# krea-ai/realtime-video

Hardware: AMD Instinct MI355X
Metric: frames/sec at 832x480, 4-step 14B T2V (per-step DiT latency in config) (higher is better)
Workload: dtype bf16

## Files before the change

include/rtv_hip.h:

```cpp
#ifndef RTV_HIP_H
#define RTV_HIP_H

#include <stddef.h>
#include <stdint.h>

#ifdef __cplusplus
extern "C" {
#endif

#define RTV_DTYPE_BF16 0
#define RTV_DTYPE_F16 1

#define RTV_ACT_NONE 0
#define RTV_ACT_GELU_TANH 1
#define RTV_ACT_SILU 2

typedef void* rtv_stream_t;

#define RTV_ABI_VERSION 103
int rtv_version(void);
const char* rtv_last_error(void);

int rtv_prof_enable(int class_mask);
int rtv_prof_read(int cls, double* total_ms, int64_t* launches, double* total_work);
int rtv_prof_reset(void);
int rtv_prof_set_stride(int cls, int stride);
int rtv_prof_read_seen(int cls, int64_t* launches, double* work);
int rtv_prof_bracket_overhead(int n, rtv_stream_t stream, double* avg_ms);

int rtv_dispatch_counts(int64_t* counts, int n);
const char* rtv_dispatch_name(int id);
int rtv_dispatch_reset(void);

int rtv_attn_fwd(const void* q, const void* k, const void* v, void* o,
                 int B, int Lq, int Lkv, int H, int D,
                 int64_t q_batch_stride, int64_t q_row_stride,
                 int64_t k_batch_stride, int64_t k_row_stride,
                 int64_t v_batch_stride, int64_t v_row_stride,
                 int64_t o_batch_stride, int64_t o_row_stride,
                 float scale, int causal_block, int q_offset, int dtype, rtv_stream_t stream);

int rtv_attn_fwd_win(const void* q, const void* k, const void* v, void* o,
                     int B, int Lq, int Lkv0, int Lkv1, int seg1_row, int H, int D,
                     int64_t q_batch_stride, int64_t q_row_stride,
                     int64_t k_batch_stride, int64_t k_row_stride,
                     int64_t v_batch_stride, int64_t v_row_stride,
                     int64_t o_batch_stride, int64_t o_row_stride,
                     float scale, int causal_block, int q_offset, int dtype, rtv_stream_t stream);
int rtv_attn_fwd_dup(const void* q, const void* k, const void* v, void* o,
                     int B, int Lq, int Lkv, int H, int D,
                     int64_t q_batch_stride, int64_t q_row_stride,
                     int64_t k_batch_stride, int64_t k_row_stride,
                     int64_t v_batch_stride, int64_t v_row_stride,
                     int64_t o_batch_stride, int64_t o_row_stride,
                     float scale, int dup_key, int dup_count, int dtype, rtv_stream_t stream);
size_t rtv_attn_split_workspace_bytes(int B, int Lq, int H, int kv_splits);
int rtv_attn_fwd_split(const void* q, const void* k, const void* v, void* o,
                       int B, int Lq, int Lkv0, int Lkv1, int seg1_row, int H, int D,
                       int64_t q_batch_stride, int64_t q_row_stride,
                       int64_t k_batch_stride, int64_t k_row_stride,
                       int64_t v_batch_stride, int64_t v_row_stride,
                       int64_t o_batch_stride, int64_t o_row_stride,
                       float scale, int causal_block, int q_offset,
                       int kv_splits, void* workspace, size_t workspace_bytes, int dtype, rtv_stream_t stream);

int rtv_gemm(const void* A, int lda, const void* W, int ldw, void* C, int ldc,
             int M, int N, int K,
             const void* bias, int act,
             const void* gate, int gate_stride, int rows_per_frame, int row_offset,
             const void* residual, int ldr,
             int dtype, int tile_cfg, rtv_stream_t stream);

size_t rtv_gemm_workspace_bytes(void);
int rtv_gemm_set_workspace(void* ptr, size_t bytes);
int rtv_gemm_set_stream_workspace(rtv_stream_t stream, void* ptr, size_t bytes);

int rtv_layernorm_modulate(const void* x, void* out, int M, int d, float eps,
                           const void* shift, const void* scale, int frame_stride, int rows_per_frame,
                           int row_offset, const void* weight, const void* bias, rtv_stream_t stream);

int rtv_rmsnorm(const void* x, int ldx, void* out, int ldo, int M, int d, float eps,
                const void* weight, rtv_stream_t stream);

int rtv_qk_norm_rope_cache(const void* qkv, void* q_out, void* k_cache, void* v_cache,
                           int64_t cache_row_stride, int cache_row0,
                           int M, int d, int num_heads, float eps,
                           const void* wq, const void* wk, const void* rope_cs,
                           int F, int gh, int gw, int start_frame, int row_offset, rtv_stream_t stream);
int rtv_qk_norm_rope_cache_ring(const void* qkv, void* q_out, void* k_cache, void* v_cache,
                                int64_t cache_row_stride, int cache_row0,
                                int M, int d, int num_heads, float eps,
                                const void* wq, const void* wk, const void* rope_cs,
                                int F, int gh, int gw, int start_frame, int row_offset,
                                int ring_lo, int ring_size, int ring_shift, rtv_stream_t stream);

int rtv_modulation_table(const void* modulation, const void* e0, void* emod,
                         int L, int F, int J, int J0, int d, rtv_stream_t stream);

int rtv_sinusoidal_embedding(const void* t, void* out, int F, int dim, rtv_stream_t stream);

int rtv_patchify(const void* x, void* rows, int C, int F, int gh, int gw, rtv_stream_t stream);
int rtv_unpatchify(const void* rows, void* x, int C, int F, int gh, int gw, rtv_stream_t stream);

int rtv_scheduler_step(const void* flow, int64_t flow_frame_stride, int64_t flow_channel_stride,
                       const void* xt, int64_t xt_frame_stride, int64_t xt_channel_stride,
                       const void* t, const void* t_next, int t_kind,
                       const void* timesteps, const void* sigmas, int n_table,
                       void* x0, const void* noise, void* noisy,
                       int F, int C, int hw, rtv_stream_t stream);

int rtv_silu(const void* x, void* out, int64_t n, rtv_stream_t stream);

typedef struct rtv_dit_config {
  int dim, ffn_dim, num_heads, num_layers;
  int freq_dim, text_dim, text_len;
  int in_dim, out_dim;
  float eps;
  int use_fp8;
  int max_attn_kv_splits;
} rtv_dit_config;

typedef struct rtv_dit_layer_weights {
  const void *qkv_w, *qkv_b;
  const void *norm_q_w, *norm_k_w;
  const void *o_w, *o_b;
  const void *norm3_w, *norm3_b;
  const void *cq_w, *cq_b, *ck_w, *ck_b, *cv_w, *cv_b, *co_w, *co_b;
  const void *cnorm_q_w, *cnorm_k_w;
  const void *ffn0_w, *ffn0_b, *ffn2_w, *ffn2_b;
} rtv_dit_layer_weights;

typedef struct rtv_dit_weights {
  const void *patch_w, *patch_b;
  const void *text0_w, *text0_b, *text2_w, *text2_b;
  const void *time0_w, *time0_b, *time2_w, *time2_b;
  const void *tproj_w, *tproj_b;
  const void *head_w, *head_b;
  const void *modulation;
  const void *head_modulation;
  const void *rope_cs;
  const rtv_dit_layer_weights* layers;
  const float* fp8_scales;
} rtv_dit_weights;

typedef struct rtv_dit_step {
  const void* x;
  const void* t;
  const void* context;
  void* out;
  int F, gh, gw;
  void* const* kv_k;
  void* const* kv_v;
  int64_t kv_row_stride;
  void* const* ca_k;
  void* const* ca_v;
  int compute_cross_kv;
  int cache_row0;
  int kv_lo, kv_hi;
  int start_frame;
  int causal_block;
  int gemm_tile_cfg;
  int row_begin, row_count;
  int ring_lo, ring_size, ring_shift;
  int text_rows;
  int kv_only;
  int attn_kv_splits;
} rtv_dit_step;

size_t rtv_dit_workspace_bytes(const rtv_dit_config* cfg, int F, int gh, int gw);
int rtv_dit_forward(const rtv_dit_config* cfg, const rtv_dit_weights* w, const rtv_dit_step* step,
                    void* workspace, size_t workspace_bytes, rtv_stream_t stream);

int rtv_dit_begin(const rtv_dit_config* cfg, const rtv_dit_weights* w, const rtv_dit_step* step,
                  void* workspace, size_t workspace_bytes, rtv_stream_t stream);
int rtv_dit_layer_qkv(const rtv_dit_config* cfg, const rtv_dit_weights* w, const rtv_dit_step* step, int layer,
                      void* workspace, size_t workspace_bytes, rtv_stream_t stream);
int rtv_dit_layer_rest(const rtv_dit_config* cfg, const rtv_dit_weights* w, const rtv_dit_step* step, int layer,
                       void* workspace, size_t workspace_bytes, rtv_stream_t stream);
enum { RTV_PROJ_LN = 1, RTV_PROJ_Q = 2, RTV_PROJ_KV = 4 };
int rtv_dit_layer_proj(const rtv_dit_config* cfg, const rtv_dit_weights* w, const rtv_dit_step* step, int layer,
                       int parts, int world, void* q_send, void* kv_send,
                       void* workspace, size_t workspace_bytes, rtv_stream_t stream);
int rtv_dit_head(const rtv_dit_config* cfg, const rtv_dit_weights* w, const rtv_dit_step* step, void* head_rows,
                 void* workspace, size_t workspace_bytes, rtv_stream_t stream);
int rtv_dit_finish(const rtv_dit_config* cfg, const rtv_dit_step* step, const void* head_rows, rtv_stream_t stream);

int rtv_dit_layer_qkv_hp(const rtv_dit_config* cfg, const rtv_dit_weights* w, const rtv_dit_step* step, int layer, int world,
                         void* q_send, void* kv_send, void* workspace, size_t workspace_bytes, rtv_stream_t stream);
int rtv_dit_layer_attn_hp(const rtv_dit_config* cfg, const rtv_dit_weights* w, const rtv_dit_step* step, int layer, int world,
                          const void* q_all, void* o_all, void* workspace, size_t workspace_bytes, rtv_stream_t stream);
int rtv_dit_layer_rest_hp(const rtv_dit_config* cfg, const rtv_dit_weights* w, const rtv_dit_step* step, int layer, int world,
                          const void* o_recv, void* workspace, size_t workspace_bytes, rtv_stream_t stream);

int rtv_quantize_fp8(const void* x, int64_t ld, int M, int d, void* q, int64_t ldq, float* scale_out, void* amax_scratch,
                     rtv_stream_t stream);
int rtv_gemm_fp8(const void* A, int lda, const void* W, int ldw, const float* a_scale, float w_scale, void* C, int ldc,
                 int M, int N, int K, const void* bias, int act, const void* gate, int gate_stride, int rows_per_frame,
                 int row_offset, const void* residual, int ldr, rtv_stream_t stream);

enum { RTV_CONV_NONE = 0, RTV_CONV_UPSAMPLE2X = 1, RTV_CONV_DOWN2X = 2, RTV_CONV_TIME_DOWN2X = 3 };
enum { RTV_CONV_GATHER = 16 };
int rtv_conv_cl(const void* in, const void* w, const void* bias, const void* residual, int res_ld,
                void* out, int out_ld, int T, int H, int W, int Cin, int Cout, int kt, int kh, int kw,
                int resample, int n_split, const void* zeros, rtv_stream_t stream);
int rtv_conv_cl_win(const void* in, const void* w, const void* bias, const void* residual, int res_ld,
                    void* out, int out_ld, int T, int H, int W, int Cin, int Cout, int kt, int kh, int kw,
                    int resample, int n_split, const void* zeros, int y_out0, int y_in0, int in_rows, int img_rows,
                    rtv_stream_t stream);
int rtv_conv3_norm_silu_cl(const void* in, const void* w, const void* bias, const void* gamma, void* out, int out_ld,
                           int T, int H, int W, int Cin, int Cout, int flags, const void* zeros, rtv_stream_t stream);
int rtv_rmsnorm_silu_cl(const void* x, void* out, const void* gamma, int C, int64_t npix, int apply_silu,
                        rtv_stream_t stream);
int rtv_softmax_rows(const void* s, int lds, void* p, int ldp, int rows, int n, rtv_stream_t stream);

typedef struct rtv_vae_conv { const void* w; const void* b; } rtv_vae_conv;
typedef struct rtv_vae_res {
  const void* gamma0; rtv_vae_conv conv_a; const void* gamma3; rtv_vae_conv conv_b; rtv_vae_conv shortcut;
} rtv_vae_res;
typedef struct rtv_vae_attn {
  const void* gamma; const void *wq, *bq, *wk, *bk, *wv, *bv, *wproj, *bproj;
} rtv_vae_attn;
typedef struct rtv_vae_weights {
  const void *conv2_w, *conv2_b, *mean, *std;
  rtv_vae_conv conv1;
  rtv_vae_res mid0, mid2, up[12];
  rtv_vae_attn attn;
  rtv_vae_conv time_conv[2], resample[3];
  const void* head_gamma;
  rtv_vae_conv head;
} rtv_vae_weights;

size_t rtv_vae_arena_bytes(int h, int w);
int rtv_vae_cache_slot(int h, int w, int slot, size_t* offset, int* C, int* H, int* W);
int rtv_vae_decode(const rtv_vae_weights* w, const void* z, int T, int h, int wd, int first,
                   void* arena, size_t arena_bytes, void* pixels, rtv_stream_t stream);
int rtv_vae_decode_single(const rtv_vae_weights* w, const void* z, int h, int wd, int is_first_frame,
                          void* arena, size_t arena_bytes, void* pixels, rtv_stream_t stream);
int rtv_pixels_to_rgb8(const void* pixels, void* rgb8, int T, int H, int W, rtv_stream_t stream);
size_t rtv_vae_arena_bytes_rows(int h, int w, int row0, int row1);
int rtv_vae_cache_slot_rows(int h, int w, int row0, int row1, int slot, size_t* offset, int* C, int* H, int* W,
                            int* first_row);
int rtv_vae_decode_rows(const rtv_vae_weights* w, const void* z, int T, int h, int wd, int first, int row0, int row1,
                        void* arena, size_t arena_bytes, void* pixels, rtv_stream_t stream);

typedef struct rtv_vae_enc_weights {
  rtv_vae_conv conv1;
  rtv_vae_res down[8];
  rtv_vae_conv resample[3];
  rtv_vae_conv time_conv[2];
  rtv_vae_res mid0, mid2;
  rtv_vae_attn attn;
  const void* head_gamma;
  rtv_vae_conv head;
  const void *conv1x1_w, *conv1x1_b;
  const void *mean, *std;
} rtv_vae_enc_weights;

size_t rtv_vae_enc_arena_bytes(int H, int W);
int rtv_vae_enc_cache_slot(int H, int W, int slot, size_t* offset, int* C, int* h, int* w, int* nslices);
int rtv_vae_encode(const rtv_vae_enc_weights* w, const void* frames, int Ttot, int t0, int tn, int H, int W, int first,
                   void* arena, size_t arena_bytes, void* mu, int Tout_tot, int tout, rtv_stream_t stream);

size_t rtv_vae_attn_arena_bytes(int h, int w);
int rtv_vae_mid_attention(const rtv_vae_attn* a, const void* x, void* y, int h, int w, void* arena, size_t arena_bytes,
                          rtv_stream_t stream);
int rtv_vae_prep(const void* z, int T, int t, int hw, const void* mean, const void* std, const void* conv2_w,
                 const void* conv2_b, void* out, rtv_stream_t stream);
int rtv_vae_final(const void* in, void* pixels, int T, int64_t hw, int64_t in_hw, int64_t skip_px, rtv_stream_t stream);
int rtv_vae_upsample_cache_t1(void* buf, int64_t slice, rtv_stream_t stream);
int rtv_vae_enc_prep(const void* frames, int Ttot, int t0, int T, int64_t hw, void* out, rtv_stream_t stream);
int rtv_vae_enc_final(const void* in, int T, int64_t hw, const void* conv1x1_w, const void* conv1x1_b, const void* mean,
                      const void* std, void* mu, int Tout_tot, int tout, rtv_stream_t stream);

typedef struct rtv_taehv_weights {
  rtv_vae_conv conv_in;
  rtv_vae_conv mem[9][3];
  const void* up[3];
  rtv_vae_conv head;
} rtv_taehv_weights;

size_t rtv_taehv_arena_bytes(int h, int w, int t_max);
int rtv_taehv_state_slot(int h, int w, int slot, size_t* offset, int* C, int* H, int* W);
int rtv_taehv_decode(const rtv_taehv_weights* w, const void* z, int T, int h, int wd, int first, void* arena,
                     size_t arena_bytes, void* pixels, rtv_stream_t stream);
int rtv_taehv_conv(const void* in, const void* w, const void* bias, const void* residual, void* out, int T, int H, int W,
                   int Cin, int Cout, int kt, int ups, int n_split, int relu, int head, const void* zeros,
                   rtv_stream_t stream);

int rtv_taehv_prep(const void* z, int T, int hw, void* out, rtv_stream_t stream);

typedef struct rtv_taehv_enc_weights {
  rtv_vae_conv conv_in;
  const void* down[3];
  rtv_vae_conv mem[9][3];
  rtv_vae_conv head;
} rtv_taehv_enc_weights;

size_t rtv_taehv_enc_arena_bytes(int H, int W, int t_max);
int rtv_taehv_enc_state_slot(int H, int W, int slot, size_t* offset, int* C, int* h, int* w);
int rtv_taehv_encode(const rtv_taehv_enc_weights* w, const void* frames, int T_total, int t0, int tn, int H, int W, int first,
                     void* arena, size_t arena_bytes, void* latents, int T_out, int j, rtv_stream_t stream);
int rtv_taehv_enc_conv(const void* in, const void* w, const void* bias, void* out, int form, int T, int H, int W, int kt,
                       int n_total, int n0, const void* zeros, rtv_stream_t stream);

int rtv_probe_mfma(const void* A , const void* B , void* D ,
                   rtv_stream_t stream);
int rtv_probe_tr(const void* V , void* out , int kbk, int s,
                 rtv_stream_t stream);

typedef struct {
  int vocab, dim, dim_attn, dim_ffn, num_heads, num_layers;
  float eps;
} rtv_t5_config;
typedef struct {
  const void* norm1_w;
  const void* qk_w;
  const void* v_w;
  const void* o_w;
  const void* norm2_w;
  const void* gate_fc1_w;
  const void* fc2_w;
  const void* pos_bias;
} rtv_t5_layer_weights;
typedef struct {
  const void* token_embedding;
  const void* final_norm_w;
  const rtv_t5_layer_weights* layers;
  int max_len;
} rtv_t5_weights;
size_t rtv_t5_workspace_bytes(const rtv_t5_config* cfg, int seq_len);
int rtv_t5_encode(const rtv_t5_config* cfg, const rtv_t5_weights* w, const int* ids, int seq_len, int out_rows,
                  void* workspace, size_t workspace_bytes, void* out, rtv_stream_t stream);

#ifdef __cplusplus
}
#endif
#endif
```

realtime_video_amd/_lib.py:

```python
import ctypes
import os
import re
import subprocess

_HERE = os.path.dirname(os.path.abspath(__file__))
LIB_PATH = os.environ.get("RTV_LIB_PATH") or os.path.join(_HERE, "librtv_hip.so")
CSRC = os.path.join(_HERE, "csrc")

_INCLUDE = os.path.join(os.path.dirname(_HERE), "include")
HEADERS = ("rtv_hip.h", "rtv_hip_lab.h")

_lib = None

_SCALARS = {"int": ctypes.c_int, "int64_t": ctypes.c_int64, "float": ctypes.c_float, "double": ctypes.c_double,
            "size_t": ctypes.c_size_t}
_RETURNS = {"int": ctypes.c_int, "size_t": ctypes.c_size_t, "const char*": ctypes.c_char_p}
_STARS = r"(\*(?:\s*const\s*\*)?)?"


def _field_type(base, stars, structs):
    value = _SCALARS.get(base) or structs.get(base)
    if not stars:
        return value
    if base == "void":
        return ctypes.c_void_p if stars == "*" else ctypes.POINTER(ctypes.c_void_p)
    return ctypes.POINTER(value) if value and stars == "*" else None


def _param_type(base, stars, structs):
    if not stars:
        return ctypes.c_void_p if base == "rtv_stream_t" else _SCALARS.get(base)
    if base in structs:
        return ctypes.POINTER(structs[base]) if stars == "*" else None
    return ctypes.c_void_p if base == "void" or base in _SCALARS else None


def parse_header(text, structs):
    text = re.sub(r"/\*.*?\*/", "", text, flags=re.S)
    text = re.sub(r"#ifdef __cplusplus.*?#endif", "", text, flags=re.S)
    text = re.sub(r"^[ \t]*#.*$", "", text, flags=re.M)
    text = re.sub(r"\benum\s*\{[^}]*\}\s*;|\btypedef\s+void\s*\*\s*rtv_stream_t\s*;", "", text)

    def struct(m):
        name, fields = m.group(2), []
        for decl in filter(None, (d.strip() for d in m.group(1).split(";"))):
            head = re.match(r"(?:const\s+)?(\w+)\s*", decl)
            for item in decl[head.end():].split(","):
                d = re.fullmatch(_STARS + r"\s*(\w+)((?:\s*\[\d+\])*)", item.strip())
                t = d and _field_type(head.group(1), re.sub(r"\s", "", d.group(1) or ""), structs)
                if not t:
                    raise ValueError(f"{name}: cannot bind field declaration `{decl}`")
                for n in reversed(re.findall(r"\d+", d.group(3))):
                    t = t * int(n)
                fields.append((d.group(2), t))
        structs[name] = type(name, (ctypes.Structure,), {"_fields_": fields})
        return ""

    text = re.sub(r"\btypedef\s+struct\s*\w*\s*\{([^}]*)\}\s*(\w+)\s*;", struct, text)
    protos = {}
    for stmt in filter(None, (" ".join(s.split()) for s in text.split(";"))):
        m = re.fullmatch(r"(.*?)\s*\b(\w+)\s*\((.*)\)", stmt)
        if not m:
            raise ValueError(f"cannot bind declaration `{stmt}`")
        ret, name, params = m.group(1).replace(" *", "*"), m.group(2), m.group(3).strip()
        if ret not in _RETURNS:
            raise ValueError(f"{name}: cannot bind return type `{ret}`")
        argtypes = []
        for param in ([] if params == "void" else params.split(",")):
            d = re.fullmatch(r"(?:const\s+)?(\w+)\s*" + _STARS + r"\s*(\w+)?", param.strip())
            t = d and _param_type(d.group(1), re.sub(r"\s", "", d.group(2) or ""), structs)
            if not t:
                raise ValueError(f"{name}: cannot bind parameter `{param.strip()}`")
            argtypes.append(t)
        protos[name] = (_RETURNS[ret], argtypes)
    return protos


def _read(name):
    with open(os.path.join(_INCLUDE, name)) as f:
        return f.read()


STRUCTS, PROTOTYPES = {}, {}
for _name in HEADERS:
    PROTOTYPES.update(parse_header(_read(_name), STRUCTS))
IO_HEADER = "rtv_hip_io.h"
IO_STRUCTS = dict(STRUCTS)
IO_PROTOTYPES = parse_header(_read(IO_HEADER), IO_STRUCTS)
IO_STRUCTS = {k: v for k, v in IO_STRUCTS.items() if k not in STRUCTS}
JPEG_HEADER = "rtv_hip_jpeg.h"
JPEG_STRUCTS = dict(STRUCTS)
JPEG_PROTOTYPES = parse_header(_read(JPEG_HEADER), JPEG_STRUCTS)
JPEG_STRUCTS = {k: v for k, v in JPEG_STRUCTS.items() if k not in STRUCTS}
JPEGDEC_HEADER = "rtv_hip_jpeg_decode.h"
JPEGDEC_STRUCTS = dict(STRUCTS)
JPEGDEC_PROTOTYPES = parse_header(_read(JPEGDEC_HEADER), JPEGDEC_STRUCTS)
JPEGDEC_STRUCTS = {k: v for k, v in JPEGDEC_STRUCTS.items() if k not in STRUCTS}
LORA_HEADER = "rtv_hip_lora.h"
LORA_STRUCTS = dict(STRUCTS)
LORA_PROTOTYPES = parse_header(_read(LORA_HEADER), LORA_STRUCTS)
LORA_STRUCTS = {k: v for k, v in LORA_STRUCTS.items() if k not in STRUCTS}
LORA_MAX_ADAPTERS, LORA_MAX_RANK = (int(re.search(rf"^#define\s+RTV_LORA_MAX_{n}\s+(\d+)", _read(LORA_HEADER), flags=re.M).group(1))
                                    for n in ("ADAPTERS", "RANK"))
FRAMES_MAX = int(re.search(r"^#define\s+RTV_FRAMES_MAX\s+(\d+)", _read(IO_HEADER), flags=re.M).group(1))
ABI_VERSION = int(re.search(r"^#define\s+RTV_ABI_VERSION\s+(\d+)", _read(HEADERS[0]), flags=re.M).group(1))


def build(verbose=False):
    jobs = os.environ.get("MAX_JOBS") or str(min(16, len(os.sched_getaffinity(0)) if hasattr(os, "sched_getaffinity") else os.cpu_count() or 4))
    cmd = ["make", "-C", CSRC, "-j", jobs]
    res = subprocess.run(cmd, capture_output=True, text=True)
    if verbose or res.returncode != 0:
        print(res.stdout[-4000:])
        print(res.stderr[-4000:])
    if res.returncode != 0:
        raise RuntimeError("building librtv_hip.so failed")
    return LIB_PATH


def declared_symbols(lab=True):
    out = set()
    for name in HEADERS if lab else HEADERS[:1]:
        text = re.sub(r"/\*.*?\*/", "", _read(name), flags=re.S)
        out.update(re.findall(r"\b(rtv_[a-z0-9_]+)\s*\(", text))
    return sorted(out)


def load():
    global _lib
    if _lib is not None:
        return _lib
    if not os.path.exists(LIB_PATH):
        raise RuntimeError(
            f"{LIB_PATH} is missing: run `python -c 'import __graft_entry__ as g; g.build()'` "
            "(or `make -C realtime_video_amd/csrc`). There is no CPU fallback for the HIP path.")
    lib = ctypes.CDLL(LIB_PATH)
    for name, (restype, argtypes) in list(PROTOTYPES.items()) + list(IO_PROTOTYPES.items()) + list(JPEG_PROTOTYPES.items()) + list(JPEGDEC_PROTOTYPES.items()) + list(LORA_PROTOTYPES.items()):
        fn = getattr(lib, name, None)
        if fn is None:
            if os.environ.get("RTV_LIB_PATH"):
                continue
            raise RuntimeError(f"librtv_hip.so does not export {name}")
        fn.restype, fn.argtypes = restype, argtypes
    have = lib.rtv_version()
    if have != ABI_VERSION:
        raise RuntimeError(f"{LIB_PATH} reports ABI revision {have}, include/rtv_hip.h declares RTV_ABI_VERSION {ABI_VERSION}: "
                           "rebuild the library (`make -C realtime_video_amd/csrc`)")
    _lib = lib
    return lib


def check(status, what):
    if status != 0:
        msg = load().rtv_last_error().decode("utf-8", "replace")
        raise RuntimeError(f"{what} failed (status {status}): {msg}")


def call(name, *args):
    check(getattr(load(), name)(*args), name)
```

realtime_video_amd/causal_model.py:

```python
import collections
import ctypes
import types

import torch

from . import _lib, lora, ops
from .rope import rope_cos_sin_table

c_vp = ctypes.c_void_p
_IncompatibleKeys = collections.namedtuple("_IncompatibleKeys", ["missing_keys", "unexpected_keys"])


_Cfg = _lib.STRUCTS["rtv_dit_config"]
_LayerW = _lib.STRUCTS["rtv_dit_layer_weights"]
_Weights = _lib.STRUCTS["rtv_dit_weights"]
_Step = _lib.STRUCTS["rtv_dit_step"]
_LAYER_FIELDS = tuple(n for n, _ in _LayerW._fields_)
_TOP_FIELDS = tuple(n for n, t in _Weights._fields_ if t is c_vp)

_FP8_TOP = ("text0_w", "text2_w", "time0_w", "time2_w", "tproj_w", "head_w")
_FP8_LAYER = ("qkv_w", "o_w", "cq_w", "ck_w", "cv_w", "co_w", "ffn0_w", "ffn2_w")

PROJ_LN, PROJ_Q, PROJ_KV = 1, 2, 4


class BlockCausalMask:

    def __init__(self, num_frames, frame_seqlen, num_frame_per_block, local_attn_size=-1):
        if local_attn_size != -1:
            raise NotImplementedError("local-window block masks are not used by the inference path")
        self.num_frames, self.frame_seqlen = num_frames, frame_seqlen
        self.num_frame_per_block = num_frame_per_block
        self.block_tokens = frame_seqlen * num_frame_per_block

    def __repr__(self):
        return f"BlockCausalMask(frames={self.num_frames}, block_tokens={self.block_tokens})"


class _SelfAttnHandle:

    def __init__(self, local_attn_size, sink_size):
        self.local_attn_size = local_attn_size
        self.sink_size = sink_size
        self.num_frame_per_block = 1
        self.fused_projections = True
        self.max_attention_size = 32760 if local_attn_size == -1 else local_attn_size * 1560

    def fuse_projections(self):
        self.fused_projections = True


def cache_row_map(cache, sink_tokens=None):
    n = int(cache["local_end_index"])
    r = torch.arange(n)
    lo, size, start = (int(cache.get(k, 0)) for k in ("ring_lo", "ring_size", "ring_start"))
    if size > 0:
        r = torch.where(r >= lo, lo + (r - lo + start) % size, r)
    return r


class CausalWanModel:
    def __init__(self, model_type="t2v", patch_size=(1, 2, 2), text_len=512, in_dim=16, dim=2048, ffn_dim=8192,
                 freq_dim=256, text_dim=4096, out_dim=16, num_heads=16, num_layers=32, local_attn_size=-1,
                 sink_size=0, qk_norm=True, cross_attn_norm=True, eps=1e-6, device="cuda"):
        if model_type != "t2v" or tuple(patch_size) != (1, 2, 2) or not qk_norm or not cross_attn_norm:
            raise NotImplementedError("the MI355X hot path implements the t2v causal model (patch 1x2x2, qk_norm, cross_attn_norm)")
        if dim % num_heads or dim // num_heads != 128:
            raise ValueError("head_dim must be 128")
        self.model_type, self.patch_size = model_type, tuple(patch_size)
        self.text_len, self.in_dim, self.dim, self.ffn_dim = text_len, in_dim, dim, ffn_dim
        self.freq_dim, self.text_dim, self.out_dim = freq_dim, text_dim, out_dim
        self.num_heads, self.num_layers, self.eps = num_heads, num_layers, eps
        self.local_attn_size, self.sink_size = local_attn_size, sink_size
        self.device = torch.device(device)
        self.config = types.SimpleNamespace(num_heads=num_heads, dim=dim, num_layers=num_layers, ffn_dim=ffn_dim)
        self.blocks = [types.SimpleNamespace(self_attn=_SelfAttnHandle(local_attn_size, sink_size))
                       for _ in range(num_layers)]
        self.block_mask = None
        self.num_frame_per_block = 1
        self.independent_first_frame = False
        self.gemm_tile_cfg = 0
        self.context_parallel = None
        self._tensors = {}
        self._w = None
        self._ws = {}
        self.fold_text_padding = True
        self.use_hip_graphs = False
        self._graphs = {}
        self._weights_version = 0
        self._cfg = _Cfg(dim, ffn_dim, num_heads, num_layers, freq_dim, text_dim, text_len, in_dim, out_dim, eps, 0, 0)
        self._lora = {}
        self._lora_base = {}
        self.lora_version = 0

    def eval(self):
        return self

    def to(self, *args, **kwargs):
        for a in list(args) + list(kwargs.values()):
            if isinstance(a, torch.dtype) and a != torch.bfloat16:
                raise NotImplementedError(f"the MI355X DiT computes in bf16 (asked for {a})")
            if isinstance(a, (str, torch.device, int)) and not isinstance(a, bool):
                dev = torch.device("cuda", a) if isinstance(a, int) else torch.device(a)
                if dev.type != self.device.type or (dev.index is not None and self.device.index is not None
                                                    and dev.index != self.device.index):
                    raise NotImplementedError(f"weights live on {self.device}; construct the model with device={dev!s} instead")
        return self

    def requires_grad_(self, flag=False):
        return self

    def parameters(self):
        return iter(self._tensors.values())

    def state_dict_shapes(self, fused=False):
        d, f = self.dim, self.ffn_dim
        sh = {"patch_embedding.weight": (d, self.in_dim) + self.patch_size, "patch_embedding.bias": (d,),
              "text_embedding.0.weight": (d, self.text_dim), "text_embedding.0.bias": (d,),
              "text_embedding.2.weight": (d, d), "text_embedding.2.bias": (d,),
              "time_embedding.0.weight": (d, self.freq_dim), "time_embedding.0.bias": (d,),
              "time_embedding.2.weight": (d, d), "time_embedding.2.bias": (d,),
              "time_projection.1.weight": (6 * d, d), "time_projection.1.bias": (6 * d,),
              "head.head.weight": (self.out_dim * 4, d), "head.head.bias": (self.out_dim * 4,), "head.modulation": (1, 2, d)}
        for i in range(self.num_layers):
            p = f"blocks.{i}"
            for a in ("self_attn", "cross_attn"):
                for m in ("q", "k", "v", "o"):
                    sh[f"{p}.{a}.{m}.weight"], sh[f"{p}.{a}.{m}.bias"] = (d, d), (d,)
                sh[f"{p}.{a}.norm_q.weight"], sh[f"{p}.{a}.norm_k.weight"] = (d,), (d,)
            if fused:
                sh[f"{p}.self_attn.to_qkv.weight"], sh[f"{p}.self_attn.to_qkv.bias"] = (3 * d, d), (3 * d,)
            sh[f"{p}.norm3.weight"], sh[f"{p}.norm3.bias"] = (d,), (d,)
            sh[f"{p}.ffn.0.weight"], sh[f"{p}.ffn.0.bias"] = (f, d), (f,)
            sh[f"{p}.ffn.2.weight"], sh[f"{p}.ffn.2.bias"] = (d, f), (d,)
            sh[f"{p}.modulation"] = (1, 6, d)
        return sh

    def load_state_dict(self, sd, strict=True, assign=False):
        dev, bf = self.device, torch.bfloat16
        sd = {(k[len("model."):] if k.startswith("model.") else k): v for k, v in sd.items()}
        want = self.state_dict_shapes(fused=True)
        problems, missing, unexpected = [], [], sorted(k for k in sd if k not in want)
        fused_layers = set()
        for i in range(self.num_layers):
            sa = f"blocks.{i}.self_attn"
            if sa + ".to_qkv.weight" in sd and sa + ".to_qkv.bias" in sd:
                fused_layers.add(i)
        for k, shp in want.items():
            layer_fused = ".self_attn." in k and int(k.split(".")[1]) in fused_layers
            is_qkv = ".self_attn." in k and k.split(".")[3] in ("q", "k", "v")
            is_fused_key = ".to_qkv." in k
            if k not in sd:
                if (is_fused_key and not layer_fused) or (is_qkv and layer_fused):
                    continue
                missing.append(k)
            elif tuple(sd[k].shape) != tuple(shp):
                problems.append(f"size mismatch for {k}: copying a param with shape {tuple(sd[k].shape)} from checkpoint, "
                                f"the shape in current model is {tuple(shp)}.")
        if missing:
            problems.insert(0, "Missing key(s) in state_dict: " + ", ".join(repr(k) for k in missing[:12])
                            + (f" ... ({len(missing)} in total)" if len(missing) > 12 else "") + ".")
        if unexpected and strict:
            problems.insert(1 if missing else 0, "Unexpected key(s) in state_dict: " + ", ".join(repr(k) for k in unexpected[:12])
                            + (f" ... ({len(unexpected)} in total)" if len(unexpected) > 12 else "") + ".")
        if problems and (strict or missing or any(p.startswith("size") for p in problems)):
            raise RuntimeError("Error(s) in loading state_dict for CausalWanModel:\n\t" + "\n\t".join(problems))
        t = {}

        def get(name):
            return sd[name].detach().to(device=dev, dtype=bf).contiguous()

        t["patch_w"] = get("patch_embedding.weight").reshape(self.dim, -1).contiguous()
        t["patch_b"] = get("patch_embedding.bias")
        for dst, src in (("text0", "text_embedding.0"), ("text2", "text_embedding.2"), ("time0", "time_embedding.0"),
                         ("time2", "time_embedding.2"), ("tproj", "time_projection.1"), ("head", "head.head")):
            t[dst + "_w"], t[dst + "_b"] = get(src + ".weight"), get(src + ".bias")
        t["head_modulation"] = get("head.modulation").reshape(2, self.dim).contiguous()
        t["modulation"] = torch.empty((self.num_layers, 6, self.dim), dtype=bf, device=dev)
        for i in range(self.num_layers):
            t["modulation"][i].copy_(sd[f"blocks.{i}.modulation"].detach().reshape(6, self.dim))
        t["rope_cs"] = rope_cos_sin_table(self.dim // self.num_heads).to(dev)
        layers = (_LayerW * self.num_layers)()
        d = self.dim
        for i in range(self.num_layers):
            p, sa, ca = f"blocks.{i}", f"blocks.{i}.self_attn", f"blocks.{i}.cross_attn"
            lt = {}
            if i in fused_layers:
                lt["qkv_w"], lt["qkv_b"] = get(sa + ".to_qkv.weight"), get(sa + ".to_qkv.bias")
            else:
                lt["qkv_w"] = torch.empty((3 * d, d), dtype=bf, device=dev)
                lt["qkv_b"] = torch.empty((3 * d,), dtype=bf, device=dev)
                for j, m in enumerate(("q", "k", "v")):
                    lt["qkv_w"][j * d:(j + 1) * d].copy_(sd[f"{sa}.{m}.weight"].detach())
                    lt["qkv_b"][j * d:(j + 1) * d].copy_(sd[f"{sa}.{m}.bias"].detach())
            lt["norm_q_w"], lt["norm_k_w"] = get(sa + ".norm_q.weight"), get(sa + ".norm_k.weight")
            lt["o_w"], lt["o_b"] = get(sa + ".o.weight"), get(sa + ".o.bias")
            lt["norm3_w"], lt["norm3_b"] = get(p + ".norm3.weight"), get(p + ".norm3.bias")
            for m in ("q", "k", "v", "o"):
                lt[f"c{m}_w"], lt[f"c{m}_b"] = get(f"{ca}.{m}.weight"), get(f"{ca}.{m}.bias")
            lt["cnorm_q_w"], lt["cnorm_k_w"] = get(ca + ".norm_q.weight"), get(ca + ".norm_k.weight")
            lt["ffn0_w"], lt["ffn0_b"] = get(p + ".ffn.0.weight"), get(p + ".ffn.0.bias")
            lt["ffn2_w"], lt["ffn2_b"] = get(p + ".ffn.2.weight"), get(p + ".ffn.2.bias")
            for name in _LAYER_FIELDS:
                setattr(layers[i], name, lt[name].data_ptr())
                t[f"L{i}.{name}"] = lt[name]
        w = _Weights()
        for name in _TOP_FIELDS:
            setattr(w, name, t[name].data_ptr())
        w.layers = ctypes.cast(layers, ctypes.POINTER(_LayerW))
        self._layers_arr = layers
        self._tensors, self._w = t, w
        self._cfg.use_fp8 = 0
        if self._lora or self._lora_base:
            self._lora, self._lora_base = {}, {}
            self.lora_version += 1
        self._graphs.clear()
        self._weights_version += 1
        return _IncompatibleKeys([], [] if strict else unexpected)

    def enable_fp8(self):
        if self._w is None:
            raise RuntimeError("load weights before enable_fp8()")
        if self._cfg.use_fp8:
            return self
        for k in (self.dim, self.ffn_dim, self.text_dim, self.freq_dim):
            if k % 128:
                raise ValueError("enable_fp8: every Linear input width must be a multiple of 128")
        scales = (ctypes.c_float * (len(_FP8_TOP) + len(_FP8_LAYER) * self.num_layers))()

        def quant(key):
            q, s = self._quantize_fp8(self._tensors[key])
            self._tensors[key] = q
            return q, s

        for i, name in enumerate(_FP8_TOP):
            q, scales[i] = quant(name)
            setattr(self._w, name, q.data_ptr())
        for l in range(self.num_layers):
            for j, name in enumerate(_FP8_LAYER):
                q, scales[len(_FP8_TOP) + len(_FP8_LAYER) * l + j] = quant(f"L{l}.{name}")
                setattr(self._layers_arr[l], name, q.data_ptr())
        self._fp8_scales = scales
        self._w.fp8_scales = ctypes.cast(scales, ctypes.POINTER(ctypes.c_float))
        self._cfg.use_fp8 = 1
        self._graphs.clear()
        self._weights_version += 1
        self._ws.clear()
        ops.ensure_gemm_workspace(self.device)
        return self

    @staticmethod
    def _quantize_fp8(w):
        s = w.float().abs().max().clamp(min=1e-12) / 448.0
        q = (w.float() / s).clamp(-448.0, 448.0).to(torch.float8_e4m3fn).contiguous()
        return q, float(s)

    def lora_adapters(self):
        return {name: ad["scale"] for name, ad in self._lora.items()}

    def load_lora(self, sd, scale=1.0, name=None, strict=True):
        targets, _ = lora.parse_lora_state_dict(sd, self.state_dict_shapes(), strict=strict)
        scale = float(scale)
        if scale != scale or scale in (float("inf"), float("-inf")):
            raise ValueError("load_lora: scale must be finite")
        if name is None:
            n = len(self._lora)
            while f"lora{n}" in self._lora:
                n += 1
            name = f"lora{n}"
        if name in self._lora:
            raise ValueError(f"load_lora: an adapter named {name!r} is loaded already")
        if len(self._lora) >= lora.MAX_ADAPTERS:
            raise RuntimeError(f"load_lora: at most {lora.MAX_ADAPTERS} adapters are loaded at once (RTV_LORA_MAX_ADAPTERS)")
        if self.device.type != "cuda":
            raise RuntimeError("load_lora: the merge is a HIP kernel and this model lives on the CPU (no CPU fallback)")
        if self._w is None:
            raise RuntimeError("load weights before load_lora()")
        if self._cfg.use_fp8:
            raise RuntimeError("load_lora after enable_fp8(): the bf16 weights are gone - load adapters first, then enable_fp8()")
        dev, bf = self.device, torch.bfloat16
        on_dev = {t: tg._replace(A=tg.A.detach().to(device=dev, dtype=bf).contiguous(),
                                 B=tg.B.detach().to(device=dev, dtype=bf).contiguous()) for t, tg in targets.items()}
        for tg in on_dev.values():
            if tg.tensor not in self._lora_base:
                self._lora_base[tg.tensor] = self._tensors[tg.tensor].clone()
        self._lora[name] = {"scale": scale, "targets": on_dev}
        self._remerge({tg.tensor for tg in on_dev.values()})
        return name

    def set_lora_scale(self, name, scale):
        if name not in self._lora:
            raise KeyError(f"no LoRA adapter named {name!r} (loaded: {list(self._lora)})")
        scale = float(scale)
        if scale != scale or scale in (float("inf"), float("-inf")):
            raise ValueError("set_lora_scale: scale must be finite")
        self._lora[name]["scale"] = scale
        self._remerge({tg.tensor for tg in self._lora[name]["targets"].values()})

    def unload_lora(self, name=None):
        if name is not None and name not in self._lora:
            raise KeyError(f"no LoRA adapter named {name!r} (loaded: {list(self._lora)})")
        touched = set()
        for n in [name] if name is not None else list(self._lora):
            touched |= {tg.tensor for tg in self._lora.pop(n)["targets"].values()}
        self._remerge(touched)

    def _remerge(self, keys):
        fp8, cross = bool(self._cfg.use_fp8), False
        for key in sorted(keys):
            base = self._lora_base[key]
            live = [(ad["scale"], tg) for ad in self._lora.values() for tg in ad["targets"].values() if tg.tensor == key]
            out = torch.empty_like(base) if fp8 else self._tensors[key]
            blocks = ((0, base.shape[0]),) if not key.endswith(".qkv_w") else tuple((j * self.dim, self.dim) for j in range(3))
            for row0, rows in blocks:
                lora.merge(base[row0:row0 + rows], out[row0:row0 + rows],
                           [(tg.A, tg.B, s * tg.factor) for s, tg in live if (tg.row0, tg.rows) == (row0, rows)])
            if fp8:
                q, s = self._quantize_fp8(out)
                self._tensors[key].copy_(q)
                layer, field = key[1:].split(".")
                self._fp8_scales[len(_FP8_TOP) + len(_FP8_LAYER) * int(layer) + _FP8_LAYER.index(field)] = s
            if not live:
                del self._lora_base[key]
            cross = cross or key.endswith((".ck_w", ".cv_w"))
        if fp8 and keys:
            self._graphs.clear()
            self._weights_version += 1
        if cross:
            self.lora_version += 1

    def init_random_weights(self, seed=0, std=0.02):
        g = torch.Generator(device=self.device).manual_seed(seed)
        d, ffn, bf = self.dim, self.ffn_dim, torch.bfloat16

        def rnd(*shape, s=std):
            return (torch.randn(*shape, generator=g, device=self.device, dtype=torch.float32) * s).to(bf)

        def xav(o, i):
            return rnd(o, i, s=(2.0 / (i + o)) ** 0.5)

        sd = {"patch_embedding.weight": xav(d, self.in_dim * 4).view(d, self.in_dim, 1, 2, 2), "patch_embedding.bias": rnd(d),
              "text_embedding.0.weight": rnd(d, self.text_dim), "text_embedding.0.bias": rnd(d),
              "text_embedding.2.weight": rnd(d, d), "text_embedding.2.bias": rnd(d),
              "time_embedding.0.weight": rnd(d, self.freq_dim), "time_embedding.0.bias": rnd(d),
              "time_embedding.2.weight": rnd(d, d), "time_embedding.2.bias": rnd(d),
              "time_projection.1.weight": xav(6 * d, d), "time_projection.1.bias": rnd(6 * d),
              "head.head.weight": rnd(self.out_dim * 4, d), "head.head.bias": rnd(self.out_dim * 4),
              "head.modulation": rnd(1, 2, d, s=d ** -0.5)}
        for i in range(self.num_layers):
            p = f"blocks.{i}"
            sd[f"{p}.self_attn.to_qkv.weight"], sd[f"{p}.self_attn.to_qkv.bias"] = xav(3 * d, d), rnd(3 * d)
            sd[f"{p}.self_attn.o.weight"], sd[f"{p}.self_attn.o.bias"] = xav(d, d), rnd(d)
            for a in ("self_attn", "cross_attn"):
                sd[f"{p}.{a}.norm_q.weight"] = 1 + rnd(d, s=0.1)
                sd[f"{p}.{a}.norm_k.weight"] = 1 + rnd(d, s=0.1)
            for m in ("q", "k", "v", "o"):
                sd[f"{p}.cross_attn.{m}.weight"], sd[f"{p}.cross_attn.{m}.bias"] = xav(d, d), rnd(d)
            sd[f"{p}.norm3.weight"], sd[f"{p}.norm3.bias"] = 1 + rnd(d, s=0.1), rnd(d, s=0.05)
            sd[f"{p}.ffn.0.weight"], sd[f"{p}.ffn.0.bias"] = xav(ffn, d), rnd(ffn)
            sd[f"{p}.ffn.2.weight"], sd[f"{p}.ffn.2.bias"] = xav(d, ffn), rnd(d)
            sd[f"{p}.modulation"] = rnd(1, 6, d, s=d ** -0.5)
        self.load_state_dict(sd)
        return self

    @staticmethod
    def _prepare_blockwise_causal_attn_mask(device=None, num_frames=21, frame_seqlen=1560, num_frame_per_block=1,
                                            local_attn_size=-1):
        return BlockCausalMask(num_frames, frame_seqlen, num_frame_per_block, local_attn_size)

    def _workspace(self, F, gh, gw, slot=0):
        key = (F, gh, gw, slot)
        ws = self._ws.get(key)
        if ws is None:
            n = _lib.load().rtv_dit_workspace_bytes(ctypes.byref(self._cfg), F, gh, gw)
            ws = torch.empty(n + 256, dtype=torch.uint8, device=self.device)
            self._ws[key] = ws
        return ws

    def kv_cache_heads(self):
        cp = self.context_parallel
        if cp is not None and getattr(cp, "world", 1) > 1 and len(cp.local_ranks()) == 1 and cp.head_exchange(self.num_heads):
            return self.num_heads // cp.world
        return self.num_heads

    def _exchange_buffers(self, M, world, slot, device):
        key = (M, world, slot)
        if not hasattr(self, "_xbufs"):
            self._xbufs = {}
        b = self._xbufs.get(key)
        if b is None:
            rl, hn = M // world, self.num_heads // world
            gc = hn * 128
            e = lambda *shape: torch.empty(shape, dtype=torch.bfloat16, device=device)
            b = {"hn": hn, "q_send": e(world, rl, gc), "kv_send": e(world, rl, 2, gc), "q_all": e(M, gc), "o_all": e(M, gc),
                 "o_recv": e(world, rl, gc)}
            self._xbufs[key] = b
        return b

    def _cache_window(self, kv_cache, num_new, current_start, frame_seqlen, ring=True):
        c0 = kv_cache[0]
        kv_size = c0["k"].shape[1]
        if self.block_mask is not None:
            if num_new > kv_size:
                raise RuntimeError(f"KV cache window [0, {num_new}) outside cache of {kv_size} rows")

            def commit_rc():
                for c in kv_cache:
                    c["global_end_index"] = num_new
                    c["local_end_index"] = num_new
                    c["ring_lo"], c["ring_size"], c["ring_start"] = 0, 0, 0
            return 0, 0, num_new, 0, self.block_mask.block_tokens, (0, 0, 0), commit_rc
        sa = self.blocks[0].self_attn
        g_end, l_end = int(c0["global_end_index"]), int(c0["local_end_index"])
        current_end = current_start + num_new
        sink_tokens = sa.sink_size * frame_seqlen
        ring_lo, ring_size = int(c0.get("ring_lo", 0)), int(c0.get("ring_size", 0))
        ring_start = int(c0.get("ring_start", 0)) if l_end > 0 else 0
        shift_copy = None
        if sa.local_attn_size != -1 and current_end > g_end and num_new + l_end > kv_size:
            evicted = num_new + l_end - kv_size
            rolled = l_end - evicted - sink_tokens
            if ring and rolled <= 0:
                ring_start = 0
            elif ring:
                if ring_size == 0 or ring_start == 0:
                    ring_lo, ring_size = sink_tokens, kv_size - sink_tokens
                elif (ring_lo, ring_size) != (sink_tokens, kv_size - sink_tokens):
                    raise RuntimeError("the attention sink changed under a rotated rolling cache")
                ring_start = (ring_start + evicted) % ring_size
            else:
                shift_copy = (sink_tokens, evicted, rolled)
            local_end = l_end + current_end - g_end - evicted
        else:
            local_end = l_end + current_end - g_end
        if not ring and ring_start:
            raise RuntimeError("this KV cache is rotated (ring_start != 0): reset it before using it under context parallelism")
        local_start = local_end - num_new
        if local_start < 0 or local_end > kv_size:
            raise RuntimeError(f"KV cache window [{local_start}, {local_end}) outside cache of {kv_size} rows")
        lo = max(0, local_end - sa.max_attention_size)
        if ring_start == 0:
            ring_lo = ring_size = 0

        def commit():
            if shift_copy is not None:
                s0, ev, ro = shift_copy
                for c in kv_cache:
                    for n in ("k", "v"):
                        c[n][:, s0:s0 + ro] = c[n][:, s0 + ev:s0 + ev + ro].clone()
            for c in kv_cache:
                c["global_end_index"] = current_end
                c["local_end_index"] = local_end
                c["ring_lo"], c["ring_size"], c["ring_start"] = ring_lo, ring_size, ring_start
        return local_start, lo, local_end, current_start // frame_seqlen, 0, (ring_lo, ring_size, ring_start), commit

    def _forward_inference(self, x, t, context, seq_len=None, clip_fea=None, y=None, kv_cache=None,
                           crossattn_cache=None, current_start=0, cache_start=0, kv_cache_only=False):
        if self._w is None:
            raise RuntimeError("weights not loaded")
        if kv_cache is None or crossattn_cache is None:
            raise NotImplementedError("the hot path is the KV-cached inference forward (causal_model.py:825-954)")
        if clip_fea is not None or y is not None:
            raise NotImplementedError("i2v conditioning is out of scope")
        xs = list(x) if not torch.is_tensor(x) else [x[i] for i in range(x.shape[0])]
        B = len(xs)
        if B != 1:
            raise NotImplementedError("batch size 1 (the streaming server path); run sessions as replicas")
        u = xs[0]
        if not u.is_cuda:
            raise RuntimeError("realtime_video_amd.CausalWanModel needs GPU tensors (no CPU fallback)")
        C, F, Hh, Ww = u.shape
        gh, gw = Hh // 2, Ww // 2
        fs = gh * gw
        M = F * fs
        if seq_len is not None and M > seq_len:
            raise AssertionError("sequence longer than seq_len")
        u = u.to(torch.bfloat16).contiguous()
        tt = t.reshape(-1).to(device=u.device, dtype=torch.float32).contiguous()
        if tt.numel() != F:
            raise ValueError("t must hold one timestep per latent frame")
        need_cross = not all(bool(c["is_init"]) and int(c.get("lora_version", 0)) == self.lora_version for c in crossattn_cache)
        ctx = None
        if need_cross:
            cu = context[0] if not torch.is_tensor(context) else context[0]
            ctx = torch.zeros(self.text_len, self.text_dim, dtype=torch.bfloat16, device=u.device)
            ctx[:cu.shape[0]] = cu.to(torch.bfloat16)
            nz = torch.nonzero(ctx.abs().amax(dim=1) > 0)
            n_real = int(nz[-1]) + 1 if nz.numel() else 0
            for c in crossattn_cache:
                c["text_rows"] = n_real
        cp = self.context_parallel
        use_cp = cp is not None and (cp.world > 1 or getattr(cp, "force_single_rank", False))
        kv_only = bool(kv_cache_only) and not need_cross
        text_rows = int(crossattn_cache[0].get("text_rows", 0)) if getattr(self, "fold_text_padding", True) else 0
        if text_rows <= 0 or any(int(c.get("text_rows", 0)) != text_rows for c in crossattn_cache):
            text_rows = 0
        row0, lo, hi, start_frame, causal_block, (ring_lo, ring_size, ring_shift), commit = \
            self._cache_window(kv_cache, M, current_start, fs, ring=not use_cp)
        L = self.num_layers
        rs = kv_cache[0]["k"].stride(1)
        for c in kv_cache:
            for n in ("k", "v"):
                if c[n].stride(3) != 1 or c[n].stride(2) != c[n].shape[3] or c[n].stride(1) != rs:
                    raise ValueError("KV cache tensors must be [B, kv_size, H, 128] views with dense [H, 128] rows "
                                     "and one common row stride")

        def ptr_array(tensors):
            arr = (c_vp * L)(*[t_.data_ptr() for t_ in tensors])
            return arr, ctypes.cast(arr, ctypes.POINTER(c_vp))

        kk_keep, kk = ptr_array([c["k"] for c in kv_cache])
        kv_keep, kv = ptr_array([c["v"] for c in kv_cache])
        ck_keep, ck = ptr_array([c["k"] for c in crossattn_cache])
        cv_keep, cv = ptr_array([c["v"] for c in crossattn_cache])
        out = (torch.zeros if kv_only else torch.empty)((self.out_dim, F, Hh, Ww), dtype=torch.bfloat16, device=u.device)
        stream = c_vp(torch.cuda.current_stream().cuda_stream)
        cfg_p, w_p = ctypes.byref(self._cfg), ctypes.byref(self._w)

        def make(rank_rows, slot, kk=kk, kv=kv):
            ws = self._workspace(F, gh, gw, slot)
            ws_ptr = (ws.data_ptr() + 255) & ~255
            st = _Step(u.data_ptr(), tt.data_ptr(), ctx.data_ptr() if ctx is not None else None, out.data_ptr(),
                       F, gh, gw, kk, kv, rs, ck, cv, int(need_cross), row0, lo, hi,
                       start_frame, causal_block, int(self.gemm_tile_cfg), rank_rows[0], rank_rows[1],
                       ring_lo, ring_size, ring_shift, int(text_rows), int(kv_only),
                       int(getattr(cp, "attn_kv_splits", 1)) if use_cp else 1)
            return st, (c_vp(ws_ptr), ctypes.c_size_t(ws.numel() - (ws_ptr - ws.data_ptr())), stream)

        splits = int(getattr(cp, "attn_kv_splits", 1)) if use_cp else 1
        if splits > self._cfg.max_attn_kv_splits:
            self._cfg.max_attn_kv_splits = splits
            self._ws.clear()
            self._graphs.clear()
            self._weights_version += 1
        if self.gemm_tile_cfg in (0, 5):
            ops.ensure_gemm_workspace(u.device)
        if use_cp:
            commit()
        if not use_cp:
            graph_key = None
            if self.use_hip_graphs and not need_cross:
                graph_key = (F, gh, gw, row0, lo, hi, start_frame, causal_block, ring_lo, ring_size, ring_shift, kv_only, text_rows,
                             int(self.gemm_tile_cfg), rs, self._weights_version,
                             kv_cache[0]["k"].data_ptr(), kv_cache[-1]["v"].data_ptr(), crossattn_cache[0]["k"].data_ptr())
                ent = self._graphs.get(graph_key)
                if isinstance(ent, dict):
                    ent["u"].copy_(u)
                    ent["t"].copy_(tt)
                    ent["graph"].replay()
                    commit()
                    return ent["out"].clone().unsqueeze(0)
            if graph_key is not None and self._graphs.get(graph_key) == "seen":
                ent = {"u": u.clone(), "t": tt.clone(), "out": out, "keep": (kk_keep, kv_keep, ck_keep, cv_keep)}
                u, tt = ent["u"], ent["t"]
                g = torch.cuda.CUDAGraph()
                if not hasattr(self, "_capture_stream"):
                    self._capture_stream = torch.cuda.Stream(device=u.device)
                ops.ensure_gemm_workspace(u.device, self._capture_stream.cuda_stream)
                with torch.cuda.graph(g, stream=self._capture_stream):
                    stream = c_vp(torch.cuda.current_stream().cuda_stream)
                    st, wsa = make((0, 0), 0)
                    _lib.call("rtv_dit_forward", cfg_p, w_p, ctypes.byref(st), *wsa)
                ent["graph"], ent["step"] = g, st
                self._graphs[graph_key] = ent
                g.replay()
                commit()
                return out.clone().unsqueeze(0)
            if graph_key is not None:
                self._graphs[graph_key] = "seen"
            st, wsa = make((0, 0), 0)
            _lib.call("rtv_dit_forward", cfg_p, w_p, ctypes.byref(st), *wsa)
            commit()
        else:
            graph_key = None
            if self.use_hip_graphs and not need_cross and not getattr(cp, "_gloo", False):
                graph_key = ("cp", id(cp), bool(getattr(cp, "overlap", True)), cp.world, cp.head_exchange(self.num_heads), F, gh, gw, row0, lo, hi, start_frame, causal_block, kv_only,
                             text_rows, int(self.gemm_tile_cfg), rs, self._weights_version, splits,
                             kv_cache[0]["k"].data_ptr(), kv_cache[-1]["v"].data_ptr(), crossattn_cache[0]["k"].data_ptr())
                ent = self._graphs.get(graph_key)
                if isinstance(ent, dict):
                    ent["u"].copy_(u)
                    ent["t"].copy_(tt)
                    ent["graph"].replay()
                    return ent["out"].clone().unsqueeze(0)

            def run_cp():
                self.cp_forwards_issued = getattr(self, "cp_forwards_issued", 0) + 1
                from .parallel import shard_rows, wait_in_order
                W, H = cp.world, self.num_heads
                heads = cp.head_exchange(H)
                keep = []
                if heads:
                    hn = H // W
                    if kv_cache[0]["k"].shape[2] not in (hn, H):
                        raise ValueError(f"KV cache must hold {hn} (this rank's) or {H} heads, not {kv_cache[0]['k'].shape[2]}")
                    parts = []
                    for i, r in enumerate(cp.local_ranks()):
                        h0 = 0 if kv_cache[0]["k"].shape[2] == hn else r * hn
                        ka, kp = ptr_array([c["k"][0, :, h0:h0 + hn] for c in kv_cache])
                        va, vp = ptr_array([c["v"][0, :, h0:h0 + hn] for c in kv_cache])
                        keep.append((ka, va))
                        parts.append(make(shard_rows(M, W, r), i, kp, vp))
                    bufs = [(r, self._exchange_buffers(M, W, i, u.device)) for i, r in enumerate(cp.local_ranks())]
                else:
                    parts = [make(shard_rows(M, W, r), i) for i, r in enumerate(cp.local_ranks())]
                for st, wsa in parts:
                    _lib.call("rtv_dit_begin", cfg_p, w_p, ctypes.byref(st), *wsa)
                null = c_vp(0)
                for l in range(L):
                    last_kv_only = kv_only and l == L - 1
                    if not heads:
                        for st, wsa in parts:
                            _lib.call("rtv_dit_layer_proj", cfg_p, w_p, ctypes.byref(st), l, PROJ_LN | PROJ_KV, 0, null, null, *wsa)
                        pend = cp.gather_kv(kv_cache[l]["k"][0], kv_cache[l]["v"][0], row0, M, async_op=True)
                        if last_kv_only:
                            pend.wait()
                            break
                        for st, wsa in parts:
                            _lib.call("rtv_dit_layer_proj", cfg_p, w_p, ctypes.byref(st), l, PROJ_Q, 0, null, null, *wsa)
                        pend.wait()
                        for st, wsa in parts:
                            _lib.call("rtv_dit_layer_rest", cfg_p, w_p, ctypes.byref(st), l, *wsa)
                        continue
                    if last_kv_only:
                        for (st, wsa), (_, b) in zip(parts, bufs):
                            _lib.call("rtv_dit_layer_proj", cfg_p, w_p, ctypes.byref(st), l, PROJ_LN | PROJ_KV, W, null,
                                      c_vp(b["kv_send"].data_ptr()), *wsa)
                        cp.exchange_kv(bufs, kv_cache[l]["k"][0], kv_cache[l]["v"][0], row0, M)
                        break
                    for (st, wsa), (_, b) in zip(parts, bufs):
                        _lib.call("rtv_dit_layer_proj", cfg_p, w_p, ctypes.byref(st), l, PROJ_LN | PROJ_Q, W,
                                  c_vp(b["q_send"].data_ptr()), null, *wsa)
                    pend_q = cp.exchange_q(bufs, async_op=True)
                    for (st, wsa), (_, b) in zip(parts, bufs):
                        _lib.call("rtv_dit_layer_proj", cfg_p, w_p, ctypes.byref(st), l, PROJ_KV, W, null,
                                  c_vp(b["kv_send"].data_ptr()), *wsa)
                    pend_kv = cp.exchange_kv(bufs, kv_cache[l]["k"][0], kv_cache[l]["v"][0], row0, M, async_op=True)
                    wait_in_order(pend_q, pend_kv)
                    for (st, wsa), (_, b) in zip(parts, bufs):
                        _lib.call("rtv_dit_layer_attn_hp", cfg_p, w_p, ctypes.byref(st), l, W, c_vp(b["q_all"].data_ptr()),
                                  c_vp(b["o_all"].data_ptr()), *wsa)
                    cp.exchange_o(bufs)
                    for (st, wsa), (_, b) in zip(parts, bufs):
                        _lib.call("rtv_dit_layer_rest_hp", cfg_p, w_p, ctypes.byref(st), l, W, c_vp(b["o_recv"].data_ptr()), *wsa)
                if not kv_only:
                    hrow = torch.empty((M, self.out_dim * 4), dtype=torch.bfloat16, device=u.device)
                    for st, wsa in parts:
                        _lib.call("rtv_dit_head", cfg_p, w_p, ctypes.byref(st), c_vp(hrow.data_ptr()), *wsa)
                    cp.all_gather_rows_(hrow, kind="head_rows")
                    _lib.call("rtv_dit_finish", cfg_p, ctypes.byref(parts[0][0]), c_vp(hrow.data_ptr()), stream)

            if graph_key is not None and self._graphs.get(graph_key) == "seen":
                ent = {"u": u.clone(), "t": tt.clone(), "out": out, "keep": (kk_keep, kv_keep, ck_keep, cv_keep)}
                u, tt = ent["u"], ent["t"]
                g = torch.cuda.CUDAGraph()
                if not hasattr(self, "_capture_stream"):
                    self._capture_stream = torch.cuda.Stream(device=u.device)
                ops.ensure_gemm_workspace(u.device, self._capture_stream.cuda_stream)
                with torch.cuda.graph(g, stream=self._capture_stream, capture_error_mode="thread_local"):
                    stream = c_vp(torch.cuda.current_stream().cuda_stream)
                    run_cp()
                ent["graph"] = g
                self._graphs[graph_key] = ent
                g.replay()
                return out.clone().unsqueeze(0)
            if graph_key is not None:
                self._graphs[graph_key] = "seen"
            run_cp()
        if need_cross:
            for c in crossattn_cache:
                c["is_init"] = True
                c["lora_version"] = self.lora_version
        return out.unsqueeze(0)

    def forward(self, *args, **kwargs):
        return self._forward_inference(*args, **kwargs)

    __call__ = forward
```

realtime_video_amd/csrc/attn_fwd.hip:

```cpp
#include "attn_common.h"

namespace rtv {

#ifdef RTV_ATTN_TRACE
__device__ unsigned* g_attn_trace = nullptr;
#define ATT_STAMP(i)                                                                    \
  do {                                                                                  \
    if (tr_on && j >= 20 && j < 24) {                                                   \
      __builtin_amdgcn_sched_barrier(0);                                                \
      const unsigned t_ = (unsigned)__builtin_readcyclecounter();                       \
      if (lane == 0) tr_dst[(j - 20) * 6 + (i)] = t_;                                   \
      __builtin_amdgcn_sched_barrier(0);                                                \
    }                                                                                   \
  } while (0)
#else
#define ATT_STAMP(i)
#endif

template <bool F16>
__global__ __launch_bounds__(256) void attn_combine_kernel(const float* __restrict__ part_o, const float* __restrict__ part_ml,
                                                           uint16_t* __restrict__ o, int S, int B, int H, int Lq, int64_t o_bs,
                                                           int64_t o_rs) {
  const int64_t nrows = (int64_t)B * H * Lq;
  const int64_t row = (int64_t)blockIdx.x * 16 + (threadIdx.x >> 4);
  if (row >= nrows) return;
  const int c8 = (threadIdx.x & 15) * 8;
  float m = -INFINITY;
  for (int s = 0; s < S; ++s) m = fmaxf(m, part_ml[((int64_t)s * nrows + row) * 2]);
  float acc[8] = {0.f, 0.f, 0.f, 0.f, 0.f, 0.f, 0.f, 0.f};
  float l = 0.f;
  for (int s = 0; s < S; ++s) {
    const f32x2 ml = *(const f32x2*)(part_ml + ((int64_t)s * nrows + row) * 2);
    const float w = __builtin_amdgcn_exp2f(ml[0] - m);
    l += w * ml[1];
    const float* po = part_o + ((int64_t)s * nrows + row) * ATT_D + c8;
    const f32x4 a = *(const f32x4*)po, b2 = *(const f32x4*)(po + 4);
#pragma unroll
    for (int i = 0; i < 4; ++i) {
      acc[i] += w * a[i];
      acc[4 + i] += w * b2[i];
    }
  }
  const float inv = 1.0f / l;
  const int bh = (int)(row / Lq), q = (int)(row - (int64_t)bh * Lq);
  const int b = bh / H, h = bh - b * H;
  u32x4 out;
#pragma unroll
  for (int i = 0; i < 4; ++i) out[i] = pack2<F16>(acc[2 * i] * inv, acc[2 * i + 1] * inv);
  *(u32x4*)(o + (size_t)b * o_bs + (size_t)q * o_rs + (size_t)h * ATT_D + c8) = out;
}

template <bool F16, int NW>
__global__ __launch_bounds__(NW * 64, 2) void attn_fwd_kernel(AttnParams p) {
  constexpr int ATT_QT = ATT_QW * NW;
  constexpr int ATT_THREADS = NW * 64;
  constexpr int ATT_LD_PER_THREAD = ATT_KT * 16 / ATT_THREADS;
  constexpr int ATT_RSTEP = ATT_THREADS / 16;
  extern __shared__ __attribute__((aligned(16))) char smem[];
  char* const sK = smem;
  char* const sV = smem + 2 * ATT_TILE_BYTES;

  const int tid = threadIdx.x;
  const int lane = tid & 63;
  const int wave = __builtin_amdgcn_readfirstlane(tid >> 6);
  const int l31 = lane & 31, g = lane >> 5;

  int bh, qt;
  {
    const int nbh = p.B * p.H;
    const int bid = blockIdx.x;
    if (nbh % 8 == 0) {
      int xcd = bid & 7, slot = bid >> 3;
      bh = xcd + 8 * (slot / p.n_qtiles);
      qt = slot % p.n_qtiles;
    } else {
      bh = bid / p.n_qtiles;
      qt = bid % p.n_qtiles;
    }
  }
  const int b = bh / p.H, h = bh % p.H;
  const int q0 = qt * ATT_QT;

  const uint16_t* qb = p.q + (size_t)b * p.q_bs + (size_t)h * ATT_D;
  const uint16_t* kb = p.k + (size_t)b * p.k_bs + (size_t)h * ATT_D;
  const uint16_t* vb = p.v + (size_t)b * p.v_bs + (size_t)h * ATT_D;
  uint16_t* ob = p.o + (size_t)b * p.o_bs + (size_t)h * ATT_D;

  const int q_row = q0 + wave * ATT_QW + l31;
  const int q_row_c = min(q_row, p.Lq - 1);
  u32x4 qf[8];
  {
    const uint16_t* qp = qb + (size_t)q_row_c * p.q_rs + g * 8;
#pragma unroll
    for (int dc = 0; dc < 8; ++dc) qf[dc] = *(const u32x4*)(qp + dc * 16);
  }

  int kv_lim = p.Lkv;
  int wave_min_lim = p.Lkv;
  int wg_max_lim = p.Lkv;
  if (p.causal_block > 0) {
    const int cb = p.causal_block;
    kv_lim = min(p.Lkv, ((p.q_offset + q_row_c) / cb + 1) * cb);
    int first = min(q0 + wave * ATT_QW, p.Lq - 1);
    wave_min_lim = min(p.Lkv, ((p.q_offset + first) / cb + 1) * cb);
    int last = min(q0 + ATT_QT - 1, p.Lq - 1);
    wg_max_lim = min(p.Lkv, ((p.q_offset + last) / cb + 1) * cb);
  }
  const int ntiles = (wg_max_lim + ATT_KT - 1) / ATT_KT;
  int t_lo, t_hi;
  split_tile_range(p, ntiles, &t_lo, &t_hi);

  u32x4 kreg[ATT_LD_PER_THREAD], vreg[ATT_LD_PER_THREAD];
  const int st_r = tid >> 4, st_c = tid & 15;
  const uint32_t k_goff = (uint32_t)(st_r * (int)p.k_rs + st_c * 8) * 2u;
  const uint32_t v_goff = (uint32_t)(st_r * (int)p.v_rs + st_c * 8) * 2u;
  auto load_tile = [&](int j) {
    const int row0 = j * ATT_KT;
    const bool in0 = row0 + ATT_KT <= p.n0;
    if (in0 || (row0 >= p.n0 && row0 + ATT_KT <= p.Lkv)) {
      const int64_t prow = in0 ? row0 : row0 + p.delta;
      const char* kj = (const char*)(kb + prow * p.k_rs);
      const char* vj = (const char*)(vb + prow * p.v_rs);
#pragma unroll
      for (int i = 0; i < ATT_LD_PER_THREAD; ++i) {
        kreg[i] = *(const u32x4*)(kj + (size_t)(i * ATT_RSTEP) * p.k_rs * 2 + k_goff);
        vreg[i] = *(const u32x4*)(vj + (size_t)(i * ATT_RSTEP) * p.v_rs * 2 + v_goff);
      }
    } else {
#pragma unroll
      for (int i = 0; i < ATT_LD_PER_THREAD; ++i) {
        int kv = min(row0 + st_r + i * ATT_RSTEP, p.Lkv - 1);
        if (kv >= p.n0) kv += p.delta;
        kreg[i] = *(const u32x4*)(kb + (int64_t)kv * p.k_rs + st_c * 8);
        vreg[i] = *(const u32x4*)(vb + (int64_t)kv * p.v_rs + st_c * 8);
      }
    }
  };
  char* const k_wr = sK + st_r * 256 + ((st_c ^ (st_r & 15)) << 4);
  char* const v_wr = sV + st_r * 256 + ((st_c << 4) ^ ((st_r & 3) << 6));
  auto write_tile = [&](int buf) {
#pragma unroll
    for (int i = 0; i < ATT_LD_PER_THREAD; ++i) {
      *(u32x4*)(k_wr + buf * ATT_TILE_BYTES + i * ATT_RSTEP * 256) = kreg[i];
      *(u32x4*)(v_wr + buf * ATT_TILE_BYTES + i * ATT_RSTEP * 256) = vreg[i];
    }
  };

  const char* k_rd[8];
#pragma unroll
  for (int dc = 0; dc < 8; ++dc) k_rd[dc] = sK + l31 * 256 + (((dc * 2 + g) ^ (l31 & 15)) << 4);
  const int i16 = lane & 15, h16 = (lane >> 4) & 1;
  const char* v_rd[4];
#pragma unroll
  for (int db = 0; db < 4; ++db)
    v_rd[db] = sV + (4 * g + (i16 >> 2)) * 256 + h16 * 32 + (i16 & 3) * 8 + ((db ^ (i16 >> 2)) << 6);

  f32x16 oacc[4];
#pragma unroll
  for (int db = 0; db < 4; ++db)
#pragma unroll
    for (int r = 0; r < 16; ++r) oacc[db][r] = 0.f;
  float m_run = -1e30f;
  float l_run = 0.f;
  const float c = p.scale_log2e;
  const f32x2 c2 = {c, c};
  constexpr float RESCALE_SLACK = 8.f;

#ifdef RTV_ATTN_TRACE
  const bool tr_on = g_attn_trace != nullptr && (wave == 0 || wave == NW - 1) && blockIdx.x < 512;
  unsigned* const tr_dst = g_attn_trace + ((size_t)(blockIdx.x & 511) * 2 + (wave == 0 ? 0 : 1)) * 24;
#endif
  auto tile = [&](const int j, auto bufc) {
    constexpr int buf = decltype(bufc)::value;
    const bool has_next = (j + 1 < t_hi);
    ATT_STAMP(0);
    if (has_next) load_tile(j + 1);

    f32x16 sacc[2];
#pragma unroll
    for (int kbk = 0; kbk < 2; ++kbk)
#pragma unroll
      for (int r = 0; r < 16; ++r) sacc[kbk][r] = 0.f;
#pragma unroll
    for (int dc = 0; dc < 8; ++dc)
#pragma unroll
      for (int kbk = 0; kbk < 2; ++kbk) {
        u32x4 kf = *(const u32x4*)(k_rd[dc] + buf * ATT_TILE_BYTES + kbk * 32 * 256);
        sacc[kbk] = mfma32<F16>(kf, qf[dc], sacc[kbk]);
      }

    ATT_STAMP(1);
    if (p.dup_key >= 0 && (unsigned)(p.dup_key - j * ATT_KT) < (unsigned)ATT_KT) {
      const int local = p.dup_key - j * ATT_KT;
#pragma unroll
      for (int kbk = 0; kbk < 2; ++kbk)
#pragma unroll
        for (int r = 0; r < 16; ++r)
          if (kbk * 32 + (r & 3) + 8 * (r >> 2) + 4 * g == local) sacc[kbk][r] += p.dup_bias;
    }
    if ((j + 1) * ATT_KT > wave_min_lim) {
#pragma unroll
      for (int kbk = 0; kbk < 2; ++kbk)
#pragma unroll
        for (int r = 0; r < 16; ++r) {
          int kv = j * ATT_KT + kbk * 32 + (r & 3) + 8 * (r >> 2) + 4 * g;
          if (kv >= kv_lim) sacc[kbk][r] = -INFINITY;
        }
    }

    float mx = sacc[0][0];
#pragma unroll
    for (int r = 1; r < 16; ++r) mx = fmaxf(mx, sacc[0][r]);
#pragma unroll
    for (int r = 0; r < 16; ++r) mx = fmaxf(mx, sacc[1][r]);
    mx = fmaxf(mx, __shfl_xor(mx, 32, 64));
    const float m_cand = fmaxf(m_run, mx * c);
    const bool need = m_cand - m_run > RESCALE_SLACK;
    if (__builtin_amdgcn_ballot_w64(need) != 0) {
      const float m_new = need ? m_cand : m_run;
      const float alpha = __builtin_amdgcn_exp2f(m_run - m_new);
      m_run = m_new;
      l_run *= alpha;
#pragma unroll
      for (int db = 0; db < 4; ++db)
#pragma unroll
        for (int r = 0; r < 16; ++r) oacc[db][r] *= alpha;
    }
    const f32x2 nm2 = {-m_run, -m_run};
    f32x2 ps2 = {0.f, 0.f};
    u32x4 pf[2][2];
#pragma unroll
    for (int kbk = 0; kbk < 2; ++kbk)
#pragma unroll
      for (int t = 0; t < 8; ++t) {
        f32x2 x = {sacc[kbk][2 * t], sacc[kbk][2 * t + 1]};
        x = __builtin_elementwise_fma(x, c2, nm2);
        f32x2 e = {__builtin_amdgcn_exp2f(x[0]), __builtin_amdgcn_exp2f(x[1])};
        ps2 += e;
        pf[kbk][t >> 2][t & 3] = pack2<F16>(e[0], e[1]);
      }
    l_run += ps2[0] + ps2[1];

    ATT_STAMP(2);
#pragma unroll
    for (int kbk = 0; kbk < 2; ++kbk)
#pragma unroll
      for (int s = 0; s < 2; ++s) {
#pragma unroll
        for (int db = 0; db < 4; ++db) {
          const char* vp = v_rd[db] + buf * ATT_TILE_BYTES + (kbk * 32 + s * 16) * 256;
          u32x2 lo = lds_tr_read(vp);
          u32x2 hi = lds_tr_read(vp + 8 * 256);
          u32x4 vf = {lo[0], lo[1], hi[0], hi[1]};
          oacc[db] = mfma32<F16>(vf, pf[kbk][s], oacc[db]);
        }
      }

    ATT_STAMP(3);
    if (has_next) write_tile(buf ^ 1);
    ATT_STAMP(4);
    __syncthreads();
    ATT_STAMP(5);
  };

  load_tile(t_lo);
  write_tile(0);
  __syncthreads();
  for (int j = t_lo; j < t_hi; j += 2) {
    tile(j, IntC<0>{});
    if (j + 1 < t_hi) tile(j + 1, IntC<1>{});
  }

  const float l_tot = l_run + __shfl_xor(l_run, 32, 64);
  if (p.kv_splits > 1) {
    store_partial(p, bh, q_row, g, oacc, m_run, l_tot);
    return;
  }
  const float inv = 1.0f / l_tot;
  if (q_row < p.Lq) {
    uint16_t* op = ob + (size_t)q_row * p.o_rs + 4 * g;
#pragma unroll
    for (int db = 0; db < 4; ++db)
#pragma unroll
      for (int i = 0; i < 4; ++i) {
        u32x2 w;
        w[0] = pack2<F16>(oacc[db][4 * i + 0] * inv, oacc[db][4 * i + 1] * inv);
        w[1] = pack2<F16>(oacc[db][4 * i + 2] * inv, oacc[db][4 * i + 3] * inv);
        *(u32x2*)(op + db * 32 + i * 8) = w;
      }
  }
}


constexpr int ATT_NB = 3;

#ifdef RTV_ATTN_TRACE
#define ATT_STAMP8(i)                                                                   \
  do {                                                                                  \
    if (tr_on && j >= 20 && j < 24) {                                                   \
      __builtin_amdgcn_sched_barrier(0);                                                \
      const unsigned t_ = (unsigned)__builtin_readcyclecounter();                       \
      if (lane == 0) tr_lds[(j - 20) * 8 + (i)] = t_;    \
      __builtin_amdgcn_sched_barrier(0);                                                \
    }                                                                                   \
  } while (0)
#else
#define ATT_STAMP8(i)
#endif

template <bool F16>
__global__ __launch_bounds__(512, 2) void attn_fwd_pp_kernel(AttnParams p) {
  constexpr int ATT_QT = 256;
  extern __shared__ __attribute__((aligned(16))) char smem[];
  char* const sK = smem;
  char* const sV = smem + ATT_NB * ATT_TILE_BYTES;

  const int tid = threadIdx.x;
  const int lane = tid & 63;
  const int wave = __builtin_amdgcn_readfirstlane(tid >> 6);
  const int grp = wave >> 2;
  const int l31 = lane & 31, g = lane >> 5;

  int bh, qt;
  {
    const int nbh = p.B * p.H;
    const int bid = blockIdx.x;
    if (nbh % 8 == 0) {
      int xcd = bid & 7, slot = bid >> 3;
      bh = xcd + 8 * (slot / p.n_qtiles);
      qt = slot % p.n_qtiles;
    } else {
      bh = bid / p.n_qtiles;
      qt = bid % p.n_qtiles;
    }
  }
  const int b = bh / p.H, h = bh % p.H;
  const int q0 = qt * ATT_QT;
  const uint16_t* qb = p.q + (size_t)b * p.q_bs + (size_t)h * ATT_D;
  const uint16_t* kb = p.k + (size_t)b * p.k_bs + (size_t)h * ATT_D;
  const uint16_t* vb = p.v + (size_t)b * p.v_bs + (size_t)h * ATT_D;
  uint16_t* ob = p.o + (size_t)b * p.o_bs + (size_t)h * ATT_D;

  const int q_row = q0 + wave * ATT_QW + l31;
  const int q_row_c = min(q_row, p.Lq - 1);
  int kv_lim = p.Lkv, wave_min_lim = p.Lkv, wg_max_lim = p.Lkv;
  if (p.causal_block > 0) {
    const int cb = p.causal_block;
    kv_lim = min(p.Lkv, ((p.q_offset + q_row_c) / cb + 1) * cb);
    int first = min(q0 + wave * ATT_QW, p.Lq - 1);
    wave_min_lim = min(p.Lkv, ((p.q_offset + first) / cb + 1) * cb);
    int last = min(q0 + ATT_QT - 1, p.Lq - 1);
    wg_max_lim = min(p.Lkv, ((p.q_offset + last) / cb + 1) * cb);
  }
  const int ntiles = (wg_max_lim + ATT_KT - 1) / ATT_KT;
  int t_lo, t_hi;
  split_tile_range(p, ntiles, &t_lo, &t_hi);

  const __amdgpu_buffer_rsrc_t rsrcK = __builtin_amdgcn_make_buffer_rsrc((void*)kb, 0, 0x7fffffff, 0x00020000);
  const __amdgpu_buffer_rsrc_t rsrcV = __builtin_amdgcn_make_buffer_rsrc((void*)vb, 0, 0x7fffffff, 0x00020000);
  const int st_row = wave * 8 + (lane >> 4);
  const int st_cp = lane & 15;
  const int k_rs = (int)p.k_rs, v_rs = (int)p.v_rs;
  const int w_off0 = __builtin_amdgcn_readfirstlane(p.off0), w_delta = __builtin_amdgcn_readfirstlane(p.delta);
  const int w_n0 = __builtin_amdgcn_readfirstlane(p.n0), w_lkv = __builtin_amdgcn_readfirstlane(p.Lkv);
  int k_ch[2], v_ch[2];
  uint32_t k_fast[2], v_fast[2];
#pragma unroll
  for (int i = 0; i < 2; ++i) {
    const int r = st_row + 4 * i;
    k_ch[i] = (st_cp ^ (r & 15)) * 8;
    v_ch[i] = (st_cp ^ ((r & 3) << 2)) * 8;
    k_fast[i] = (uint32_t)(r * k_rs + k_ch[i]) * 2u;
    v_fast[i] = (uint32_t)(r * v_rs + v_ch[i]) * 2u;
  }
  auto stage = [&](const __amdgpu_buffer_rsrc_t& rsrc, char* ring, int j, int rs, const uint32_t (&fast)[2],
                   const int (&ch)[2]) {
    const int row0 = j * ATT_KT;
    char* const dst = ring + (j % ATT_NB) * ATT_TILE_BYTES + wave * (8 * 256);
    const bool in0 = row0 + ATT_KT <= w_n0;
    if (in0 || (row0 >= w_n0 && row0 + ATT_KT <= w_lkv)) {
      const uint32_t so = (uint32_t)((row0 + (in0 ? w_off0 : w_delta)) * rs) * 2u;
#pragma unroll
      for (int i = 0; i < 2; ++i)
        __builtin_amdgcn_raw_ptr_buffer_load_lds(rsrc, (RTV_LDS void*)(dst + i * 1024), 16, fast[i], so, 0, 0);
    } else {
#pragma unroll
      for (int i = 0; i < 2; ++i) {
        int kv = min(row0 + st_row + 4 * i, w_lkv - 1);
        kv += kv >= w_n0 ? w_delta : w_off0;
        __builtin_amdgcn_raw_ptr_buffer_load_lds(rsrc, (RTV_LDS void*)(dst + i * 1024), 16,
                                                 (uint32_t)(kv * rs + ch[i]) * 2u, 0, 0, 0);
      }
    }
  };
  auto stage_k = [&](int j) { stage(rsrcK, sK, j, k_rs, k_fast, k_ch); };
  auto stage_v = [&](int j) { stage(rsrcV, sV, j, v_rs, v_fast, v_ch); };

  stage_k(t_lo);
  stage_v(t_lo);
  stage_k(t_lo + 1);
  stage_v(t_lo + 1);
  u32x4 qf[8];
  {
    const uint16_t* qp = qb + (size_t)q_row_c * p.q_rs + g * 8;
#pragma unroll
    for (int dc = 0; dc < 8; ++dc) qf[dc] = *(const u32x4*)(qp + dc * 16);
  }

  uint32_t k_rd32[8];
#pragma unroll
  for (int dc = 0; dc < 8; ++dc)
    k_rd32[dc] = (uint32_t)(uintptr_t)(RTV_LDS const char*)(sK + l31 * 256 + (((dc * 2 + g) ^ (l31 & 15)) << 4));
  const int i16 = lane & 15, h16 = (lane >> 4) & 1;
  uint32_t v_rd32[4];
#pragma unroll
  for (int db = 0; db < 4; ++db)
    v_rd32[db] = (uint32_t)(uintptr_t)(RTV_LDS const char*)(sV + (4 * g + (i16 >> 2)) * 256 + h16 * 32 + (i16 & 3) * 8 +
                                                            ((db ^ (i16 >> 2)) << 6));

  f32x16 oacc[4];
#pragma unroll
  for (int db = 0; db < 4; ++db)
#pragma unroll
    for (int r = 0; r < 16; ++r) oacc[db][r] = 0.f;
  float m_run = -1e30f;
  float l_run = 0.f;
  const float c = p.scale_log2e;
  const f32x2 c2 = {c, c};
  constexpr float RESCALE_SLACK = 8.f;

  f32x16 sacc[2];
  u32x4 pf[2][2];
  u32x4 frag[16];
  f32x2 ps2 = {0.f, 0.f};
  auto exp_step = [&](auto kc, auto tc) {
    constexpr int kbk = decltype(kc)::value, t = decltype(tc)::value;
    const f32x2 nm2 = {-m_run, -m_run};
    f32x2 x = {sacc[kbk][2 * t], sacc[kbk][2 * t + 1]};
    x = __builtin_elementwise_fma(x, c2, nm2);
#ifdef ATT_LAB_T3
    f32x2 e = x;
#else
    f32x2 e = {__builtin_amdgcn_exp2f(x[0]), __builtin_amdgcn_exp2f(x[1])};
#endif
    ps2 += e;
    pf[kbk][t >> 2][t & 3] = pack2<F16>(e[0], e[1]);
  };

#ifdef RTV_ATTN_TRACE
  const bool tr_on = g_attn_trace != nullptr && (wave == 0 || wave == 7) && blockIdx.x < 512;
  unsigned* const tr_dst = g_attn_trace + ((size_t)(blockIdx.x & 511) * 2 + (wave == 0 ? 0 : 1)) * 32;
  unsigned* const tr_lds = (unsigned*)(smem + 2 * ATT_NB * ATT_TILE_BYTES) + (wave == 0 ? 0 : 32);
#endif
#define PP_BARRIER()                        \
  do {                                      \
    __builtin_amdgcn_sched_barrier(0);      \
    __builtin_amdgcn_s_barrier();           \
    __builtin_amdgcn_sched_barrier(0);      \
  } while (0)

  asm volatile("s_waitcnt vmcnt(0)" ::: "memory");
  __syncthreads();
  if (grp) PP_BARRIER();

  const bool idle_rows = p.skip_idle && q0 + wave * ATT_QW >= p.Lq;
  if (idle_rows) {
    for (int j = t_lo; j < t_hi; ++j) {
      stage_k(j + 2);
      asm volatile("s_waitcnt vmcnt(4)" ::: "memory");
      PP_BARRIER();
      PP_BARRIER();
      stage_v(j + 2);
      asm volatile("s_waitcnt vmcnt(4)" ::: "memory");
      PP_BARRIER();
      PP_BARRIER();
    }
    if (!grp) PP_BARRIER();
    return;
  }
  for (int j = t_lo; j < t_hi; ++j) {
    const int slot_off = (j % ATT_NB) * ATT_TILE_BYTES;
    ATT_STAMP8(0);
#ifndef ATT_LAB_T6
    stage_k(j + 2);
#endif
    static_for<0, 16>([&](auto ic) {
      constexpr int n = decltype(ic)::value;
      frag[n] = lds_read128_at<(n & 1) * 32 * 256>(k_rd32[n >> 1] + (uint32_t)slot_off);
    });
    asm volatile("s_waitcnt vmcnt(4)" ::: "memory");
    ATT_STAMP8(1);
    PP_BARRIER();
    ATT_STAMP8(2);
    lds_wait_frags(frag);
    uint32_t va[4];
#pragma unroll
    for (int db = 0; db < 4; ++db) va[db] = v_rd32[db] + (uint32_t)slot_off;
    auto rd_v = [&](auto ic) {
#ifndef ATT_LAB_T4
      constexpr int idx = decltype(ic)::value;
      constexpr int off = ((idx >> 3) * 32 + ((idx >> 2) & 1) * 16) * 256;
      const u32x2 lo = lds_tr_read_at<off>(va[idx & 3]);
      const u32x2 hi = lds_tr_read_at<off + 8 * 256>(va[idx & 3]);
      frag[idx] = u32x4{lo[0], lo[1], hi[0], hi[1]};
#endif
    };
    static_for<0, 8>([&](auto ic) {
      constexpr int dc = decltype(ic)::value;
      if constexpr (dc == 0) {
        f32x16 z;
#pragma unroll
        for (int r = 0; r < 16; ++r) z[r] = 0.f;
        sacc[0] = mfma32<F16>(frag[0], qf[0], z);
        sacc[1] = mfma32<F16>(frag[1], qf[0], z);
      } else {
        sacc[0] = mfma32<F16>(frag[2 * dc], qf[dc], sacc[0]);
        sacc[1] = mfma32<F16>(frag[2 * dc + 1], qf[dc], sacc[1]);
      }
      __builtin_amdgcn_sched_barrier(0);
      rd_v(IntC<2 * dc>{});
      rd_v(IntC<2 * dc + 1>{});
      __builtin_amdgcn_sched_barrier(0);
    });
    ATT_STAMP8(3);
    PP_BARRIER();
    ATT_STAMP8(4);
#ifndef ATT_LAB_T6
    stage_v(j + 2);
#endif
    if ((j + 1) * ATT_KT > wave_min_lim) {
#pragma unroll
      for (int kbk = 0; kbk < 2; ++kbk)
#pragma unroll
        for (int r = 0; r < 16; ++r) {
          int kv = j * ATT_KT + kbk * 32 + (r & 3) + 8 * (r >> 2) + 4 * g;
          if (kv >= kv_lim) sacc[kbk][r] = -INFINITY;
        }
    }
    {
      float mx = sacc[0][0];
#pragma unroll
      for (int r = 1; r < 16; ++r) mx = fmaxf(mx, sacc[0][r]);
#pragma unroll
      for (int r = 0; r < 16; ++r) mx = fmaxf(mx, sacc[1][r]);
      mx = xor32_max(mx);
      const float m_cand = fmaxf(m_run, mx * c);
      const bool need = m_cand - m_run > RESCALE_SLACK;
      if (__builtin_amdgcn_ballot_w64(need) != 0) {
        const float m_new = need ? m_cand : m_run;
        const float alpha = __builtin_amdgcn_exp2f(m_run - m_new);
        m_run = m_new;
        l_run *= alpha;
#pragma unroll
        for (int db = 0; db < 4; ++db)
#pragma unroll
          for (int r = 0; r < 16; ++r) oacc[db][r] *= alpha;
      }
      static_for<0, 4>([&](auto ic) { exp_step(IntC<0>{}, ic); });
    }
    asm volatile("" : "+v"(pf[0][0]), "+v"(ps2));
    asm volatile("s_waitcnt vmcnt(4)" ::: "memory");
    ATT_STAMP8(5);
    PP_BARRIER();
    ATT_STAMP8(6);
    lds_wait_frags(frag);
    static_for<0, 16>([&](auto ic) {
      constexpr int i = decltype(ic)::value, kbk = i >> 3, s_ = (i >> 2) & 1, db = i & 3;
      oacc[db] = mfma32<F16>(frag[(kbk * 2 + s_) * 4 + db], pf[kbk][s_], oacc[db]);
      if constexpr (i < 12) {
        constexpr int f = i + 4;
        exp_step(IntC<(f >> 3)>{}, IntC<(f & 7)>{});
      }
      __builtin_amdgcn_sched_barrier(0);
    });
    l_run += ps2[0] + ps2[1];
    ps2 = f32x2{0.f, 0.f};
    asm volatile("" : "+v"(l_run));
    ATT_STAMP8(7);
    PP_BARRIER();
  }
  if (!grp) PP_BARRIER();
#undef PP_BARRIER

#ifdef RTV_ATTN_TRACE
  if (tr_on && lane < 32 && ntiles >= 24) tr_dst[lane] = tr_lds[lane];
#endif
  const float l_tot = l_run + __shfl_xor(l_run, 32, 64);
  if (p.kv_splits > 1) {
    store_partial(p, bh, q_row, g, oacc, m_run, l_tot);
    return;
  }
  const float inv = 1.0f / l_tot;
  if (q_row < p.Lq) {
    uint16_t* op = ob + (size_t)q_row * p.o_rs + 4 * g;
#pragma unroll
    for (int db = 0; db < 4; ++db)
#pragma unroll
      for (int i = 0; i < 4; ++i) {
        u32x2 w;
        w[0] = pack2<F16>(oacc[db][4 * i + 0] * inv, oacc[db][4 * i + 1] * inv);
        w[1] = pack2<F16>(oacc[db][4 * i + 2] * inv, oacc[db][4 * i + 3] * inv);
        *(u32x2*)(op + db * 32 + i * 8) = w;
      }
  }
}

}

using namespace rtv;

#ifdef RTV_ATTN_TRACE
extern "C" int rtv_attn_debug_trace(unsigned* buf) {
  return hipMemcpyToSymbol(HIP_SYMBOL(rtv::g_attn_trace), &buf, sizeof(buf)) == hipSuccess ? 0 : -1;
}
#endif

static std::atomic<int> g_attn_waves{0};
static std::atomic<bool> g_attn_lockstep{false};
static std::atomic<bool> g_attn_force_pp{false};
static std::atomic<bool> g_attn_skip_idle{true};
static std::atomic<int> g_attn_w4{-2};
constexpr int W4_DEFAULT = 600;
namespace rtv {
int launch_attn_w4(const AttnParams& p, bool f16, int variant, dim3 grid, hipStream_t stream);
}

extern "C" int rtv_attn_set_skip_idle(int on) {
  g_attn_skip_idle = on != 0;
  return 0;
}

extern "C" int rtv_attn_set_waves(int waves) {
  if (waves != 0 && waves != 4 && waves != 8 && waves != 81 && waves != 82 && !(waves >= 840 && waves <= 1639))
    return set_error(-1, "attn_set_waves: 0 (auto), 4, 8, 81 (256 rows, lockstep schedule), 82 (256 rows, four-phase schedule) or "
                         "840 + v (256 rows, one wave per SIMD, kernel variant v: attn_w4.hip)");
  g_attn_lockstep = waves == 81;
  g_attn_force_pp = waves == 82;
  g_attn_w4 = waves >= 840 ? waves - 840 : (waves == 81 || waves == 82 ? -1 : -2);
  g_attn_waves = waves > 8 ? 8 : waves;
  return 0;
}

extern "C" int rtv_attn_fwd(const void* q, const void* k, const void* v, void* o, int B, int Lq, int Lkv,
                            int H, int D, int64_t q_batch_stride, int64_t q_row_stride,
                            int64_t k_batch_stride, int64_t k_row_stride, int64_t v_batch_stride,
                            int64_t v_row_stride, int64_t o_batch_stride, int64_t o_row_stride, float scale,
                            int causal_block, int q_offset, int dtype, rtv_stream_t stream) {
  return rtv_attn_fwd_win(q, k, v, o, B, Lq, Lkv, 0, 0, H, D, q_batch_stride, q_row_stride, k_batch_stride, k_row_stride,
                          v_batch_stride, v_row_stride, o_batch_stride, o_row_stride, scale, causal_block, q_offset, dtype,
                          stream);
}

static int attn_fwd_impl(const void* q, const void* k, const void* v, void* o, int B, int Lq, int Lkv0, int Lkv1,
                         int seg1_row, int H, int D, int64_t q_batch_stride, int64_t q_row_stride,
                         int64_t k_batch_stride, int64_t k_row_stride, int64_t v_batch_stride,
                         int64_t v_row_stride, int64_t o_batch_stride, int64_t o_row_stride, float scale,
                         int causal_block, int q_offset, int dtype, rtv_stream_t stream, int dup_key, int dup_count,
                         int kv_splits = 1, void* split_ws = nullptr, size_t split_ws_bytes = 0);

extern "C" int rtv_attn_fwd_win(const void* q, const void* k, const void* v, void* o, int B, int Lq, int Lkv0, int Lkv1,
                                int seg1_row, int H, int D, int64_t q_batch_stride, int64_t q_row_stride,
                                int64_t k_batch_stride, int64_t k_row_stride, int64_t v_batch_stride,
                                int64_t v_row_stride, int64_t o_batch_stride, int64_t o_row_stride, float scale,
                                int causal_block, int q_offset, int dtype, rtv_stream_t stream) {
  return attn_fwd_impl(q, k, v, o, B, Lq, Lkv0, Lkv1, seg1_row, H, D, q_batch_stride, q_row_stride, k_batch_stride, k_row_stride,
                       v_batch_stride, v_row_stride, o_batch_stride, o_row_stride, scale, causal_block, q_offset, dtype, stream,
                       -1, 0);
}

extern "C" int rtv_attn_fwd_dup(const void* q, const void* k, const void* v, void* o, int B, int Lq, int Lkv, int H, int D,
                                int64_t q_batch_stride, int64_t q_row_stride, int64_t k_batch_stride, int64_t k_row_stride,
                                int64_t v_batch_stride, int64_t v_row_stride, int64_t o_batch_stride, int64_t o_row_stride,
                                float scale, int dup_key, int dup_count, int dtype, rtv_stream_t stream) {
  if (dup_key < 0 || dup_key >= Lkv || dup_count < 1) return set_error(-1, "attn_fwd_dup: dup_key must be a key of the window, dup_count >= 1");
  return attn_fwd_impl(q, k, v, o, B, Lq, Lkv, 0, 0, H, D, q_batch_stride, q_row_stride, k_batch_stride, k_row_stride,
                       v_batch_stride, v_row_stride, o_batch_stride, o_row_stride, scale, 0, 0, dtype, stream,
                       dup_count > 1 ? dup_key : -1, dup_count);
}

extern "C" size_t rtv_attn_split_workspace_bytes(int B, int Lq, int H, int kv_splits) {
  if (B <= 0 || Lq <= 0 || H <= 0 || kv_splits < 2) return 0;
  return (size_t)kv_splits * B * H * Lq * (ATT_D + 2) * sizeof(float);
}

extern "C" int rtv_attn_fwd_split(const void* q, const void* k, const void* v, void* o, int B, int Lq, int Lkv0, int Lkv1,
                                  int seg1_row, int H, int D, int64_t q_batch_stride, int64_t q_row_stride,
                                  int64_t k_batch_stride, int64_t k_row_stride, int64_t v_batch_stride,
                                  int64_t v_row_stride, int64_t o_batch_stride, int64_t o_row_stride, float scale,
                                  int causal_block, int q_offset, int kv_splits, void* workspace, size_t workspace_bytes,
                                  int dtype, rtv_stream_t stream) {
  if (kv_splits < 1 || kv_splits > 16) return set_error(-1, "attn_fwd_split: kv_splits must be 1..16");
  return attn_fwd_impl(q, k, v, o, B, Lq, Lkv0, Lkv1, seg1_row, H, D, q_batch_stride, q_row_stride, k_batch_stride, k_row_stride,
                       v_batch_stride, v_row_stride, o_batch_stride, o_row_stride, scale, causal_block, q_offset, dtype, stream, -1,
                       0, kv_splits, workspace, workspace_bytes);
}

static int attn_fwd_impl(const void* q, const void* k, const void* v, void* o, int B, int Lq, int Lkv0, int Lkv1,
                         int seg1_row, int H, int D, int64_t q_batch_stride, int64_t q_row_stride,
                         int64_t k_batch_stride, int64_t k_row_stride, int64_t v_batch_stride,
                         int64_t v_row_stride, int64_t o_batch_stride, int64_t o_row_stride, float scale,
                         int causal_block, int q_offset, int dtype, rtv_stream_t stream, int dup_key, int dup_count,
                         int kv_splits, void* split_ws, size_t split_ws_bytes) {
  if (Lkv0 < 0 || Lkv1 < 0) return set_error(-1, "attn_fwd: negative segment length");
  if (Lkv1 > 0 && causal_block > 0) return set_error(-1, "attn_fwd: the block-causal mask needs a one-segment window");
  const int Lkv = Lkv0 + Lkv1;
  if (D != ATT_D) return set_error(-1, "attn_fwd: head_dim must be 128");
  if (B <= 0 || H <= 0 || Lq <= 0) return 0;
  if (Lkv <= 0) return set_error(-1, "attn_fwd: Lkv must be positive");
  if ((q_row_stride | k_row_stride | v_row_stride | o_row_stride | q_batch_stride | k_batch_stride |
       v_batch_stride | o_batch_stride) & 7)
    return set_error(-1, "attn_fwd: strides must be multiples of 8 elements (16-byte rows)");
  if (((uintptr_t)q | (uintptr_t)k | (uintptr_t)v | (uintptr_t)o) & 15)
    return set_error(-1, "attn_fwd: base pointers must be 16-byte aligned");
  if (causal_block < 0 || q_offset < 0) return set_error(-1, "attn_fwd: negative mask parameters");
  if (dtype != RTV_DTYPE_BF16 && dtype != RTV_DTYPE_F16) return set_error(-1, "attn_fwd: dtype");
  AttnParams p;
  p.q = (const uint16_t*)q;
  p.k = (const uint16_t*)k;
  p.v = (const uint16_t*)v;
  p.o = (uint16_t*)o;
  p.B = B;
  p.Lq = Lq;
  p.Lkv = Lkv;
  p.H = H;
  p.q_bs = q_batch_stride;
  p.q_rs = q_row_stride;
  p.k_bs = k_batch_stride;
  p.k_rs = k_row_stride;
  p.v_bs = v_batch_stride;
  p.v_rs = v_row_stride;
  p.o_bs = o_batch_stride;
  p.o_rs = o_row_stride;
  p.scale_log2e = scale * 1.4426950408889634f;
  p.dup_key = dup_key;
  p.dup_bias = dup_key >= 0 ? log2f((float)dup_count) / p.scale_log2e : 0.f;
  if (kv_splits > (Lkv + ATT_KT - 1) / ATT_KT) kv_splits = (Lkv + ATT_KT - 1) / ATT_KT;
  if (kv_splits < 1) kv_splits = 1;
  p.kv_splits = kv_splits;
  p.part_o = nullptr;
  p.part_ml = nullptr;
  if (kv_splits > 1) {
    if (dup_key >= 0) return set_error(-1, "attn_fwd: no KV split of a window with a counted key");
    const size_t rows = (size_t)kv_splits * B * H * Lq;
    if (!split_ws || ((uintptr_t)split_ws & 15) || split_ws_bytes < rows * (ATT_D + 2) * sizeof(float))
      return set_error(-1, "attn_fwd: split workspace missing, misaligned or too small (rtv_attn_split_workspace_bytes)");
    p.part_o = (float*)split_ws;
    p.part_ml = p.part_o + rows * ATT_D;
  }
  p.causal_block = causal_block;
  p.q_offset = q_offset;
  p.n0 = Lkv1 > 0 ? Lkv0 : Lkv;
  p.delta = Lkv1 > 0 ? seg1_row - Lkv0 : 0;
  int waves = g_attn_waves;
  const int cus = device_num_cus() > 0 ? device_num_cus() : 256;
  if (waves == 0) waves = ((int64_t)B * H * ((Lq + 255) / 256) * kv_splits < (int64_t)cus * 5 / 8 || Lkv <= 512) ? 4 : 8;
  const int qt_rows = ATT_QW * waves;
  p.n_qtiles = (Lq + qt_rows - 1) / qt_rows;
  const int lds = 4 * ATT_TILE_BYTES;
  const bool f16 = dtype == RTV_DTYPE_F16;
  const void* kerns[4] = {(const void*)attn_fwd_kernel<false, 8>, (const void*)attn_fwd_kernel<true, 8>,
                          (const void*)attn_fwd_kernel<false, 4>, (const void*)attn_fwd_kernel<true, 4>};
  static LdsAttr lds_attr[4];
  const int ki = (waves == 4 ? 2 : 0) + (f16 ? 1 : 0);
  if (int st = ensure_dynamic_lds(kerns[ki], lds, &lds_attr[ki], "attn_fwd")) return st;
  const int grid = B * H * p.n_qtiles;
  double kv_avg = Lkv;
  if (causal_block > 0 && Lq > 0) {
    double keys = 0;
    for (int64_t r0 = 0; r0 < Lq;) {
      const int64_t blk = (r0 + q_offset) / causal_block;
      int64_t r1 = (blk + 1) * (int64_t)causal_block - q_offset;
      if (r1 > Lq) r1 = Lq;
      const int64_t lim = (blk + 1) * (int64_t)causal_block;
      keys += (double)(r1 - r0) * (double)(lim < Lkv ? lim : Lkv);
      r0 = r1;
    }
    kv_avg = keys / Lq;
  }
  ProfScope prof(PROF_ATTN, (hipStream_t)stream, 4.0 * B * H * (double)Lq * kv_avg * ATT_D);
  const dim3 g(grid, kv_splits), t(waves * 64);
  auto combine = [&]() -> int {
    if (int st = check_launch("attn_fwd")) return st;
    const int64_t nrows = (int64_t)B * H * Lq;
    const dim3 cg((unsigned)((nrows + 15) / 16)), ct(256);
    note_kernel(DK_ATTN_SPLIT_COMBINE);
    if (f16) hipLaunchKernelGGL((attn_combine_kernel<true>), cg, ct, 0, (hipStream_t)stream, p.part_o, p.part_ml, p.o, kv_splits, B, H, Lq, p.o_bs, p.o_rs);
    else hipLaunchKernelGGL((attn_combine_kernel<false>), cg, ct, 0, (hipStream_t)stream, p.part_o, p.part_ml, p.o, kv_splits, B, H, Lq, p.o_bs, p.o_rs);
    return check_launch("attn_combine");
  };
  p.off0 = 0;
  p.skip_idle = g_attn_skip_idle ? 1 : 0;
  const int base_shift = (Lkv1 > 0 && seg1_row < 0) ? seg1_row : 0;
  const int64_t top0 = (int64_t)p.n0 - base_shift, top1 = (int64_t)Lkv + p.delta - base_shift;
  const int64_t rs_max = k_row_stride > v_row_stride ? k_row_stride : v_row_stride;
  const bool offsets_fit = k_row_stride > 0 && v_row_stride > 0 &&
                           ((top0 > top1 ? top0 : top1) + ATT_KT) * rs_max * 2 < 0x7fffffffLL;
  int w4v = g_attn_w4;
  if (w4v == -2) w4v = Lkv >= 1024 ? W4_DEFAULT : -1;
  if (waves == 8 && w4v >= 0 && !f16 && Lkv1 == 0 && dup_key < 0 && offsets_fit) {
    if (int st = launch_attn_w4(p, f16, w4v, g, (hipStream_t)stream)) return st;
    note_kernel(DK_ATTN_W4);
    if (kv_splits > 1) return combine();
    return check_launch("attn_w4");
  }
  if (waves == 8 && !g_attn_lockstep && offsets_fit && dup_key < 0 && (Lkv >= 1024 || g_attn_force_pp)) {
    p.k += (int64_t)base_shift * k_row_stride;
    p.v += (int64_t)base_shift * v_row_stride;
    p.off0 = -base_shift;
    p.delta -= base_shift;
#ifdef RTV_ATTN_TRACE
    const int lds_pp = 2 * ATT_NB * ATT_TILE_BYTES + 256;
#else
    const int lds_pp = 2 * ATT_NB * ATT_TILE_BYTES;
#endif
    static LdsAttr pp_attr[2];
    const void* kp = f16 ? (const void*)attn_fwd_pp_kernel<true> : (const void*)attn_fwd_pp_kernel<false>;
    if (int st = ensure_dynamic_lds(kp, lds_pp, &pp_attr[f16], "attn_fwd")) return st;
    note_kernel(DK_ATTN_FOUR_PHASE);
    if (f16) hipLaunchKernelGGL((attn_fwd_pp_kernel<true>), g, t, lds_pp, (hipStream_t)stream, p);
    else hipLaunchKernelGGL((attn_fwd_pp_kernel<false>), g, t, lds_pp, (hipStream_t)stream, p);
    if (kv_splits > 1) return combine();
    return check_launch("attn_fwd");
  }
  note_kernel(waves == 4 ? DK_ATTN_LOCKSTEP_128ROW : DK_ATTN_LOCKSTEP_256ROW);
  if (waves == 4) {
    if (f16) hipLaunchKernelGGL((attn_fwd_kernel<true, 4>), g, t, lds, (hipStream_t)stream, p);
    else hipLaunchKernelGGL((attn_fwd_kernel<false, 4>), g, t, lds, (hipStream_t)stream, p);
  } else {
    if (f16) hipLaunchKernelGGL((attn_fwd_kernel<true, 8>), g, t, lds, (hipStream_t)stream, p);
    else hipLaunchKernelGGL((attn_fwd_kernel<false, 8>), g, t, lds, (hipStream_t)stream, p);
  }
  if (kv_splits > 1) return combine();
  return check_launch("attn_fwd");
}
```

realtime_video_amd/csrc/dit_forward.hip:

```cpp
#include <atomic>

#include "rtv_common.h"
#include "rtv_internal.h"

namespace rtv {

__global__ void silu_kernel(const bf16_t* __restrict__ x, bf16_t* __restrict__ out, int64_t n) {
  for (int64_t i = (int64_t)blockIdx.x * blockDim.x + threadIdx.x; i < n; i += (int64_t)gridDim.x * blockDim.x)
    out[i] = f32_to_bf16(silu(bf16_to_f32(x[i])));
}

struct Workspace {
  char* base;
  size_t off, cap;
  bool ok;
  void* take(size_t bytes) {
    size_t a = (off + 255) & ~(size_t)255;
    if (base && a + bytes > cap) ok = false;
    off = a + bytes;
    return base ? base + a : nullptr;
  }
};

struct DitBuffers {
  uint16_t *x, *xn, *qkv, *q, *ao, *h, *prow, *hrow;
  uint16_t *sinus, *te1, *e, *se, *e0, *emod, *ehead, *ctx1, *ctx, *ktmp;
  uint8_t* q8;
  float* fscale;
  float* attn_part;
  size_t attn_part_bytes;
};

static size_t carve(const rtv_dit_config* c, int F, int gh, int gw, char* base, size_t cap, DitBuffers* b,
                    bool* ok) {
  Workspace ws{base, 0, cap, true};
  const size_t M = (size_t)F * gh * gw, d = c->dim, e = 2;
  DitBuffers t;
  t.x = (uint16_t*)ws.take(M * d * e);
  t.xn = (uint16_t*)ws.take(M * d * e);
  t.qkv = (uint16_t*)ws.take(M * 3 * d * e);
  t.q = (uint16_t*)ws.take(M * d * e);
  t.ao = (uint16_t*)ws.take(M * d * e);
  t.h = (uint16_t*)ws.take(M * (size_t)c->ffn_dim * e);
  t.prow = (uint16_t*)ws.take(M * (size_t)c->in_dim * 4 * e);
  t.hrow = (uint16_t*)ws.take(M * (size_t)c->out_dim * 4 * e);
  t.sinus = (uint16_t*)ws.take((size_t)F * c->freq_dim * e);
  t.te1 = (uint16_t*)ws.take((size_t)F * d * e);
  t.e = (uint16_t*)ws.take((size_t)F * d * e);
  t.se = (uint16_t*)ws.take((size_t)F * d * e);
  t.e0 = (uint16_t*)ws.take((size_t)F * 6 * d * e);
  t.emod = (uint16_t*)ws.take((size_t)c->num_layers * F * 6 * d * e);
  t.ehead = (uint16_t*)ws.take((size_t)F * 2 * d * e);
  t.ctx1 = (uint16_t*)ws.take((size_t)c->text_len * d * e);
  t.ctx = (uint16_t*)ws.take((size_t)c->text_len * d * e);
  t.ktmp = (uint16_t*)ws.take((size_t)c->text_len * d * e);
  {
    size_t rows = M > (size_t)c->text_len ? M : (size_t)c->text_len, k = d;
    if ((size_t)c->ffn_dim > k) k = c->ffn_dim;
    if ((size_t)c->text_dim > k) k = c->text_dim;
    if ((size_t)c->freq_dim > k) k = c->freq_dim;
    t.q8 = (uint8_t*)ws.take(c->use_fp8 ? rows * k : 0);
    t.fscale = (float*)ws.take(256);
  }
  t.attn_part_bytes = c->max_attn_kv_splits > 1 ? M * (size_t)c->num_heads * (128 + 2) * sizeof(float) : 0;
  t.attn_part = (float*)ws.take(t.attn_part_bytes);
  if (b) *b = t;
  if (ok) *ok = ws.ok;
  return ws.off;
}

struct Ctx {
  const rtv_dit_config* cfg;
  const rtv_dit_weights* w;
  const rtv_dit_step* st;
  DitBuffers b;
  rtv_stream_t stream;
  int d, H, L, ffn, hd, F, gh, gw, fs, M, r0, rc, tc;
};

static int make_ctx(const rtv_dit_config* cfg, const rtv_dit_weights* w, const rtv_dit_step* st, void* workspace,
                    size_t workspace_bytes, rtv_stream_t stream, Ctx* c) {
  if (!cfg || !w || !st || !workspace) return set_error(-1, "dit: null argument");
  c->cfg = cfg;
  c->w = w;
  c->st = st;
  c->stream = stream;
  c->d = cfg->dim;
  c->H = cfg->num_heads;
  c->L = cfg->num_layers;
  c->ffn = cfg->ffn_dim;
  if (c->H <= 0 || c->d % c->H || c->d / c->H != 128) return set_error(-1, "dit: head_dim must be 128");
  c->hd = 128;
  c->F = st->F;
  c->gh = st->gh;
  c->gw = st->gw;
  c->fs = st->gh * st->gw;
  c->M = st->F * c->fs;
  if (c->M <= 0) return set_error(-1, "dit: empty token grid");
  c->r0 = st->row_begin;
  c->rc = st->row_count > 0 ? st->row_count : c->M - st->row_begin;
  if (c->r0 < 0 || c->rc <= 0 || c->r0 + c->rc > c->M) return set_error(-1, "dit: local row range outside the token grid");
  if (st->kv_lo < 0 || st->kv_hi <= st->kv_lo) return set_error(-1, "dit: empty attention window");
  if (st->cache_row0 < 0 || st->cache_row0 + c->M > st->kv_hi)
    return set_error(-1, "dit: the rows written by this call must lie inside the attention window");
  if (st->ring_size < 0 || st->ring_lo < 0 || st->ring_shift < 0 || (st->ring_size > 0 && st->ring_shift >= st->ring_size) ||
      (st->ring_size > 0 && st->kv_hi > st->ring_lo + st->ring_size))
    return set_error(-1, "dit: bad ring window (0 <= ring_shift < ring_size, kv_hi <= ring_lo + ring_size)");
  if (st->ring_size > 0 && st->ring_shift > 0 && st->causal_block > 0)
    return set_error(-1, "dit: the block-causal recompute pass writes an unrotated cache (ring_shift must be 0)");
  if (((uintptr_t)workspace) & 255) return set_error(-1, "dit: workspace must be 256-byte aligned");
  bool ok = true;
  carve(cfg, c->F, c->gh, c->gw, (char*)workspace, workspace_bytes, &c->b, &ok);
  if (!ok) return set_error(-1, "dit: workspace too small (see rtv_dit_workspace_bytes)");
  c->tc = st->gemm_tile_cfg;
  return 0;
}

}

using namespace rtv;

#define RTV_TRY(expr)        \
  do {                       \
    int _s = (expr);         \
    if (_s != 0) return _s;  \
  } while (0)

extern "C" int rtv_silu(const void* x, void* out, int64_t n, rtv_stream_t stream) {
  if (n <= 0) return 0;
  int blocks = (int)((n + 255) / 256);
  if (blocks > 2048) blocks = 2048;
  hipLaunchKernelGGL(silu_kernel, dim3(blocks), dim3(256), 0, (hipStream_t)stream, (const bf16_t*)x,
                     (bf16_t*)out, n);
  return check_launch("silu");
}

extern "C" size_t rtv_dit_workspace_bytes(const rtv_dit_config* cfg, int F, int gh, int gw) {
  if (!cfg || F <= 0 || gh <= 0 || gw <= 0) return 0;
  return carve(cfg, F, gh, gw, nullptr, 0, nullptr, nullptr) + 256;
}

enum { S_TEXT0 = 0, S_TEXT2, S_TIME0, S_TIME2, S_TPROJ, S_HEAD, S_LAYER0 };
enum { S_QKV = 0, S_O, S_CQ, S_CK, S_CV, S_CO, S_FFN0, S_FFN2, S_PER_LAYER };
static int linear(Ctx& c, int sidx, const void* a, int K, const void* w, const void* bias, void* out, int M, int N, int act,
                  const void* gate, int gate_stride, int rpf, int row_off, const void* res, int cfg, rtv_stream_t s) {
  if (!c.cfg->use_fp8 || sidx < 0)
    return rtv_gemm(a, K, w, K, out, N, M, N, K, bias, act, gate, gate_stride, rpf, row_off, res, N, RTV_DTYPE_BF16, cfg, s);
  if (!c.w->fp8_scales) return set_error(-1, "dit: use_fp8 needs rtv_dit_weights.fp8_scales");
  if (rtv_quantize_fp8(a, K, M, K, c.b.q8, K, c.b.fscale, c.b.fscale + 1, s)) return -1;
  return rtv_gemm_fp8(c.b.q8, K, w, K, c.b.fscale, c.w->fp8_scales[sidx], out, N, M, N, K, bias, act, gate, gate_stride, rpf,
                      row_off, res, N, s);
}

static int dit_begin(Ctx& c) {
  const rtv_dit_config* cfg = c.cfg;
  const rtv_dit_weights* w = c.w;
  const rtv_dit_step* st = c.st;
  DitBuffers& b = c.b;
  const int d = c.d, F = c.F, L = c.L, tc = c.tc;
  rtv_stream_t stream = c.stream;
  const int pk = cfg->in_dim * 4;
  RTV_TRY(rtv_patchify(st->x, b.prow, cfg->in_dim, F, c.gh, c.gw, stream));
  RTV_TRY(linear(c, -1, b.prow + (size_t)c.r0 * pk, pk, w->patch_w, w->patch_b, b.x, c.rc, d, 0, nullptr, 0, 0, 0, nullptr, tc, stream));
  RTV_TRY(rtv_sinusoidal_embedding(st->t, b.sinus, F, cfg->freq_dim, stream));
  RTV_TRY(linear(c, S_TIME0, b.sinus, cfg->freq_dim, w->time0_w, w->time0_b, b.te1, F, d, RTV_ACT_SILU, nullptr, 0, 0, 0, nullptr, tc, stream));
  RTV_TRY(linear(c, S_TIME2, b.te1, d, w->time2_w, w->time2_b, b.e, F, d, 0, nullptr, 0, 0, 0, nullptr, tc, stream));
  RTV_TRY(rtv_silu(b.e, b.se, (int64_t)F * d, stream));
  RTV_TRY(linear(c, S_TPROJ, b.se, d, w->tproj_w, w->tproj_b, b.e0, F, 6 * d, 0, nullptr, 0, 0, 0, nullptr, tc, stream));
  RTV_TRY(rtv_modulation_table(w->modulation, b.e0, b.emod, L, F, 6, 6, d, stream));
  RTV_TRY(rtv_modulation_table(w->head_modulation, b.e, b.ehead, 1, F, 2, 1, d, stream));
  if (st->compute_cross_kv) {
    if (!st->context) return set_error(-1, "dit: context required to initialise the cross-attention cache");
    const int T = cfg->text_len;
    RTV_TRY(linear(c, S_TEXT0, st->context, cfg->text_dim, w->text0_w, w->text0_b, b.ctx1, T, d, RTV_ACT_GELU_TANH, nullptr, 0, 0, 0, nullptr, tc, stream));
    RTV_TRY(linear(c, S_TEXT2, b.ctx1, d, w->text2_w, w->text2_b, b.ctx, T, d, 0, nullptr, 0, 0, 0, nullptr, tc, stream));
    for (int l = 0; l < L; ++l) {
      const rtv_dit_layer_weights& lw = w->layers[l];
      RTV_TRY(linear(c, S_LAYER0 + S_PER_LAYER * l + S_CK, b.ctx, d, lw.ck_w, lw.ck_b, b.ktmp, T, d, 0, nullptr, 0, 0, 0, nullptr, tc, stream));
      RTV_TRY(rtv_rmsnorm(b.ktmp, d, st->ca_k[l], d, T, d, cfg->eps, lw.cnorm_k_w, stream));
      RTV_TRY(linear(c, S_LAYER0 + S_PER_LAYER * l + S_CV, b.ctx, d, lw.cv_w, lw.cv_b, st->ca_v[l], T, d, 0, nullptr, 0, 0, 0, nullptr, tc, stream));
    }
  }
  return 0;
}

static int hp_check(Ctx& c, int world);

static std::atomic<int> g_direct_v{1};
static int dit_layer_proj(Ctx& c, int l, int parts, int world, void* q_send, void* kv_send) {
  const rtv_dit_layer_weights& lw = c.w->layers[l];
  const rtv_dit_step* st = c.st;
  DitBuffers& b = c.b;
  const int d = c.d;
  if (!(parts & (RTV_PROJ_LN | RTV_PROJ_Q | RTV_PROJ_KV))) return set_error(-1, "dit: empty projection phase");
  const uint16_t* em = b.emod + (size_t)l * c.F * 6 * d;
  if (parts & RTV_PROJ_LN)
    RTV_TRY(rtv_layernorm_modulate(b.x, b.xn, c.rc, d, c.cfg->eps, em + 0 * d, em + 1 * d, 6 * d, c.fs, c.r0, nullptr, nullptr, c.stream));
  const bool q = parts & RTV_PROJ_Q, kv = parts & RTV_PROJ_KV;
  if (!q && !kv) return 0;
  const int n0 = q ? 0 : d, nn = (q ? d : 0) + (kv ? 2 * d : 0);
  const uint16_t* wq = (const uint16_t*)lw.qkv_w;
  const uint16_t* bq = (const uint16_t*)lw.qkv_b;
  const size_t welt = c.cfg->use_fp8 ? 1 : 2;
  bool v_in_place = false;
  {
    const void* wp = (const char*)lw.qkv_w + (size_t)n0 * d * welt;
    (void)wq;
    void* v_dst = nullptr;
    if (kv && !kv_send && g_direct_v.load(std::memory_order_relaxed) && st->kv_v[l] && !(st->kv_row_stride & 7)) {
      int r0 = st->cache_row0 + c.r0;
      const int S = st->ring_lo, R = st->ring_size;
      bool one_range = true;
      if (R > 0 && r0 + c.rc > S) {
        if (r0 < S) one_range = false;
        else {
          r0 = S + (r0 - S + st->ring_shift) % R;
          one_range = r0 + c.rc <= S + R;
        }
      }
      uint16_t* dst = (uint16_t*)st->kv_v[l] + (size_t)r0 * st->kv_row_stride;
      if (one_range && !((uintptr_t)dst & 15)) v_dst = dst;
    }
    const void* wv = (const char*)lw.qkv_w + (size_t)2 * d * d * welt;
    {
      const int rp = (q ? 1 : 0) | (kv ? 2 : 0) | (v_dst ? 4 : 0);
      if (q_send || kv_send) {
        RTV_TRY(hp_check(c, world));
        const int gc = d / world;
        if ((q && !q_send) || (kv && !kv_send)) return set_error(-1, "dit: exchange buffers required");
        RTV_TRY(qk_norm_rope_check(2 * gc, 0, c.rc, d, c.H, c.F, c.gh, c.gw, st->start_frame, c.r0, gc, (int64_t)c.rc * gc,
                                   (int64_t)c.rc * 2 * gc, 0, 0, 0, rp));
      } else {
        RTV_TRY(qk_norm_rope_check(st->kv_row_stride, st->cache_row0, c.rc, d, c.H, c.F, c.gh, c.gw, st->start_frame, c.r0, 0, 0, 0,
                                   st->ring_lo, st->ring_size, st->ring_shift, rp));
      }
    }
    if (!c.cfg->use_fp8) {
      if (v_dst) {
        if (2 * d > n0)
          RTV_TRY(rtv_gemm(b.xn, d, wp, d, b.qkv + n0, 3 * d, c.rc, 2 * d - n0, d, bq + n0, 0, nullptr, 0, 0, 0, nullptr, 0, RTV_DTYPE_BF16,
                           c.tc, c.stream));
        RTV_TRY(rtv_gemm(b.xn, d, wv, d, v_dst, (int)st->kv_row_stride, c.rc, d, d, bq + 2 * d, 0, nullptr, 0, 0, 0, nullptr, 0,
                         RTV_DTYPE_BF16, c.tc, c.stream));
        v_in_place = true;
      } else {
        RTV_TRY(rtv_gemm(b.xn, d, wp, d, b.qkv + n0, 3 * d, c.rc, nn, d, bq + n0, 0, nullptr, 0, 0, 0, nullptr, 0, RTV_DTYPE_BF16, c.tc,
                         c.stream));
      }
    } else {
      if (!c.w->fp8_scales) return set_error(-1, "dit: use_fp8 needs rtv_dit_weights.fp8_scales");
      if (rtv_quantize_fp8(b.xn, d, c.rc, d, b.q8, d, b.fscale, b.fscale + 1, c.stream)) return -1;
      const float ws = c.w->fp8_scales[S_LAYER0 + S_PER_LAYER * l + S_QKV];
      if (v_dst) {
        if (2 * d > n0)
          RTV_TRY(rtv_gemm_fp8(b.q8, d, wp, d, b.fscale, ws, b.qkv + n0, 3 * d, c.rc, 2 * d - n0, d, bq + n0, 0, nullptr, 0, 0, 0, nullptr, 0,
                               c.stream));
        RTV_TRY(rtv_gemm_fp8(b.q8, d, wv, d, b.fscale, ws, v_dst, (int)st->kv_row_stride, c.rc, d, d, bq + 2 * d, 0, nullptr, 0, 0, 0, nullptr,
                             0, c.stream));
        v_in_place = true;
      } else {
        RTV_TRY(rtv_gemm_fp8(b.q8, d, wp, d, b.fscale, ws, b.qkv + n0, 3 * d, c.rc, nn, d, bq + n0, 0, nullptr, 0, 0, 0, nullptr, 0, c.stream));
      }
    }
  }
  const int rope_parts = (q ? 1 : 0) | (kv ? 2 : 0) | (v_in_place ? 4 : 0);
  if (q_send || kv_send) {
    RTV_TRY(hp_check(c, world));
    const int gc = d / world;
    if ((q && !q_send) || (kv && !kv_send)) return set_error(-1, "dit: exchange buffers required");
    return qk_norm_rope_launch(b.qkv, q_send, kv_send, kv_send ? (void*)((uint16_t*)kv_send + gc) : nullptr, 2 * gc, 0, c.rc, d, c.H,
                               c.cfg->eps, lw.norm_q_w, lw.norm_k_w, c.w->rope_cs, c.F, c.gh, c.gw, st->start_frame, c.r0, gc,
                               (int64_t)c.rc * gc, (int64_t)c.rc * 2 * gc, 0, 0, 0, rope_parts, c.stream);
  }
  return qk_norm_rope_launch(b.qkv, b.q, st->kv_k[l], st->kv_v[l], st->kv_row_stride, st->cache_row0, c.rc, d, c.H, c.cfg->eps,
                             lw.norm_q_w, lw.norm_k_w, c.w->rope_cs, c.F, c.gh, c.gw, st->start_frame, c.r0, 0, 0, 0, st->ring_lo,
                             st->ring_size, st->ring_shift, rope_parts, c.stream);
}

static int dit_layer_qkv(Ctx& c, int l) { return dit_layer_proj(c, l, RTV_PROJ_LN | RTV_PROJ_Q | RTV_PROJ_KV, 0, nullptr, nullptr); }

static int dit_after_attn(Ctx& c, int l);

struct KeyWindow {
  int row0, n0, row1, n1;
};
static KeyWindow key_window(const rtv_dit_step* st) {
  const int lo = st->kv_lo, hi = st->kv_hi, S = st->ring_lo, R = st->ring_size;
  if (R <= 0 || hi <= S) return KeyWindow{lo, hi - lo, 0, 0};
  const int rl = lo > S ? lo : S;
  const int n = hi - rl;
  const int p0 = S + (rl - S + st->ring_shift) % R;
  const int first = (p0 + n <= S + R) ? n : S + R - p0;
  const int sink = lo < S ? S - lo : 0;
  if (first == n) {
    if (sink == 0) return KeyWindow{p0, n, 0, 0};
    if (p0 == S) return KeyWindow{lo, sink + n, 0, 0};
    return KeyWindow{lo, sink, p0, n};
  }
  return KeyWindow{sink ? lo : S, sink + n - first, p0, first};
}

static int sharded_self_attn(Ctx& c, const void* q, const void* k, const void* v, void* o, int rows, int n0, int n1, int seg1_row,
                             int heads, int64_t q_rs, int64_t kv_rs, int64_t o_rs, int q_offset) {
  const rtv_dit_step* st = c.st;
  const float scale = 1.0f / sqrtf((float)c.hd);
  const int S = st->attn_kv_splits;
  const int qo = st->causal_block > 0 ? q_offset : 0;
  if (S > 1 && (S > c.cfg->max_attn_kv_splits || rtv_attn_split_workspace_bytes(1, rows, heads, S) > c.b.attn_part_bytes))
    return set_error(-1, "dit: attn_kv_splits exceeds rtv_dit_config.max_attn_kv_splits / the partials do not fit the workspace "
                         "(splits <= number of shards)");
  if (S > 1)
    return rtv_attn_fwd_split(q, k, v, o, 1, rows, n0, n1, seg1_row, heads, c.hd, 0, q_rs, 0, kv_rs, 0, kv_rs, 0, o_rs, scale,
                              st->causal_block, qo, S, c.b.attn_part, c.b.attn_part_bytes, RTV_DTYPE_BF16, c.stream);
  return rtv_attn_fwd_win(q, k, v, o, 1, rows, n0, n1, seg1_row, heads, c.hd, 0, q_rs, 0, kv_rs, 0, kv_rs, 0, o_rs, scale,
                          st->causal_block, qo, RTV_DTYPE_BF16, c.stream);
}

static int dit_layer_rest(Ctx& c, int l) {
  const rtv_dit_step* st = c.st;
  DitBuffers& b = c.b;
  const int d = c.d, H = c.H, hd = c.hd, rc = c.rc, r0 = c.r0;
  rtv_stream_t stream = c.stream;
  const float scale = 1.0f / sqrtf((float)hd);
  const int64_t rs = st->kv_row_stride;
  const int Lkv = st->kv_hi - st->kv_lo;
  const int q_offset = st->cache_row0 - st->kv_lo + r0;
  uint16_t* kc = (uint16_t*)st->kv_k[l];
  uint16_t* vc = (uint16_t*)st->kv_v[l];
  KeyWindow kw = key_window(st);
  if (rc < c.M) {
    RTV_TRY(sharded_self_attn(c, b.q, kc + (size_t)kw.row0 * rs, vc + (size_t)kw.row0 * rs, b.ao, rc, kw.n0, kw.n1,
                              kw.row1 - kw.row0, H, d, rs, d, q_offset));
  } else {
    RTV_TRY(rtv_attn_fwd_win(b.q, kc + (size_t)kw.row0 * rs, vc + (size_t)kw.row0 * rs, b.ao, 1, rc, kw.n0, kw.n1,
                             kw.row1 - kw.row0, H, hd, 0, d, 0, rs, 0, rs, 0, d, scale, st->causal_block,
                             st->causal_block > 0 ? q_offset : 0, RTV_DTYPE_BF16, stream));
  }
  (void)Lkv;
  return dit_after_attn(c, l);
}

static int dit_after_attn(Ctx& c, int l) {
  const rtv_dit_layer_weights& lw = c.w->layers[l];
  const rtv_dit_step* st = c.st;
  DitBuffers& b = c.b;
  const int d = c.d, H = c.H, hd = c.hd, fs = c.fs, tc = c.tc, rc = c.rc, r0 = c.r0;
  rtv_stream_t stream = c.stream;
  const float eps = c.cfg->eps;
  const uint16_t* em = b.emod + (size_t)l * c.F * 6 * d;
  const float scale = 1.0f / sqrtf((float)hd);
  RTV_TRY(linear(c, S_LAYER0 + S_PER_LAYER * l + S_O, b.ao, d, lw.o_w, lw.o_b, b.x, rc, d, 0, em + 2 * d, 6 * d, fs, r0, b.x, tc, stream));
  RTV_TRY(rtv_layernorm_modulate(b.x, b.xn, rc, d, eps, nullptr, nullptr, 0, 0, 0, lw.norm3_w, lw.norm3_b, stream));
  RTV_TRY(linear(c, S_LAYER0 + S_PER_LAYER * l + S_CQ, b.xn, d, lw.cq_w, lw.cq_b, b.qkv, rc, d, 0, nullptr, 0, 0, 0, nullptr, tc, stream));
  RTV_TRY(rtv_rmsnorm(b.qkv, d, b.q, d, rc, d, eps, lw.cnorm_q_w, stream));
  if (st->text_rows > 0 && st->text_rows + 1 < c.cfg->text_len)
    RTV_TRY(rtv_attn_fwd_dup(b.q, st->ca_k[l], st->ca_v[l], b.ao, 1, rc, st->text_rows + 1, H, hd, 0, d, 0, d, 0, d, 0, d, scale,
                             st->text_rows, c.cfg->text_len - st->text_rows, RTV_DTYPE_BF16, stream));
  else
    RTV_TRY(rtv_attn_fwd(b.q, st->ca_k[l], st->ca_v[l], b.ao, 1, rc, c.cfg->text_len, H, hd, 0, d, 0, d, 0, d, 0, d,
                         scale, 0, 0, RTV_DTYPE_BF16, stream));
  RTV_TRY(linear(c, S_LAYER0 + S_PER_LAYER * l + S_CO, b.ao, d, lw.co_w, lw.co_b, b.x, rc, d, 0, nullptr, 0, 0, 0, b.x, tc, stream));
  RTV_TRY(rtv_layernorm_modulate(b.x, b.xn, rc, d, eps, em + 3 * d, em + 4 * d, 6 * d, fs, r0, nullptr, nullptr, stream));
  RTV_TRY(linear(c, S_LAYER0 + S_PER_LAYER * l + S_FFN0, b.xn, d, lw.ffn0_w, lw.ffn0_b, b.h, rc, c.ffn, RTV_ACT_GELU_TANH, nullptr, 0, 0, 0, nullptr, tc, stream));
  RTV_TRY(linear(c, S_LAYER0 + S_PER_LAYER * l + S_FFN2, b.h, c.ffn, lw.ffn2_w, lw.ffn2_b, b.x, rc, d, 0, em + 5 * d, 6 * d, fs, r0, b.x, tc, stream));
  return 0;
}

static int hp_check(Ctx& c, int world) {
  if (world < 1 || c.H % world) return set_error(-1, "dit: head-parallel exchange needs num_heads % world == 0");
  if (c.M % world || c.rc != c.M / world || c.r0 % c.rc)
    return set_error(-1, "dit: head-parallel exchange needs equal token shards (M % world == 0)");
  return 0;
}

static int dit_layer_qkv_hp(Ctx& c, int l, int world, void* q_send, void* kv_send) {
  return dit_layer_proj(c, l, RTV_PROJ_LN | RTV_PROJ_Q | RTV_PROJ_KV, world, q_send, kv_send);
}

static int dit_layer_attn_hp(Ctx& c, int l, int world, const void* q_all, void* o_all) {
  RTV_TRY(hp_check(c, world));
  const rtv_dit_step* st = c.st;
  const int gc = c.d / world, hn = c.H / world;
  const int64_t rs = st->kv_row_stride;
  const int Lkv = st->kv_hi - st->kv_lo;
  const int q_offset = st->cache_row0 - st->kv_lo;
  const uint16_t* kc = (const uint16_t*)st->kv_k[l];
  const uint16_t* vc = (const uint16_t*)st->kv_v[l];
  KeyWindow kw = key_window(st);
  (void)Lkv;
  return sharded_self_attn(c, q_all, kc + (size_t)kw.row0 * rs, vc + (size_t)kw.row0 * rs, o_all, c.M, kw.n0, kw.n1,
                           kw.row1 - kw.row0, hn, gc, rs, gc, q_offset);
}

static int dit_layer_rest_hp(Ctx& c, int l, int world, const void* o_recv) {
  RTV_TRY(hp_check(c, world));
  RTV_TRY(regroup_heads(o_recv, c.b.ao, c.rc, world, c.d / world, c.stream));
  return dit_after_attn(c, l);
}

static int dit_head(Ctx& c, void* head_rows) {
  DitBuffers& b = c.b;
  const int d = c.d, n = c.cfg->out_dim * 4;
  RTV_TRY(rtv_layernorm_modulate(b.x, b.xn, c.rc, d, c.cfg->eps, b.ehead + 0 * d, b.ehead + 1 * d, 2 * d, c.fs, c.r0, nullptr, nullptr, c.stream));
  RTV_TRY(linear(c, S_HEAD, b.xn, d, c.w->head_w, c.w->head_b, (uint16_t*)head_rows + (size_t)c.r0 * n, c.rc, n, 0, nullptr, 0, 0, 0, nullptr, c.tc, c.stream));
  return 0;
}

extern "C" int rtv_dit_begin(const rtv_dit_config* cfg, const rtv_dit_weights* w, const rtv_dit_step* st, void* ws,
                             size_t ws_bytes, rtv_stream_t stream) {
  Ctx c;
  RTV_TRY(make_ctx(cfg, w, st, ws, ws_bytes, stream, &c));
  return dit_begin(c);
}

extern "C" int rtv_dit_layer_qkv(const rtv_dit_config* cfg, const rtv_dit_weights* w, const rtv_dit_step* st, int layer,
                                 void* ws, size_t ws_bytes, rtv_stream_t stream) {
  Ctx c;
  RTV_TRY(make_ctx(cfg, w, st, ws, ws_bytes, stream, &c));
  if (layer < 0 || layer >= c.L) return set_error(-1, "dit: layer out of range");
  return dit_layer_qkv(c, layer);
}

extern "C" int rtv_dit_layer_proj(const rtv_dit_config* cfg, const rtv_dit_weights* w, const rtv_dit_step* st, int layer,
                                  int parts, int world, void* q_send, void* kv_send, void* ws, size_t ws_bytes,
                                  rtv_stream_t stream) {
  Ctx c;
  RTV_TRY(make_ctx(cfg, w, st, ws, ws_bytes, stream, &c));
  if (layer < 0 || layer >= c.L) return set_error(-1, "dit: layer out of range");
  return dit_layer_proj(c, layer, parts, world, q_send, kv_send);
}

extern "C" int rtv_dit_layer_rest(const rtv_dit_config* cfg, const rtv_dit_weights* w, const rtv_dit_step* st, int layer,
                                  void* ws, size_t ws_bytes, rtv_stream_t stream) {
  Ctx c;
  RTV_TRY(make_ctx(cfg, w, st, ws, ws_bytes, stream, &c));
  if (layer < 0 || layer >= c.L) return set_error(-1, "dit: layer out of range");
  return dit_layer_rest(c, layer);
}

extern "C" int rtv_dit_layer_qkv_hp(const rtv_dit_config* cfg, const rtv_dit_weights* w, const rtv_dit_step* st, int layer,
                                    int world, void* q_send, void* kv_send, void* ws, size_t ws_bytes, rtv_stream_t stream) {
  Ctx c;
  RTV_TRY(make_ctx(cfg, w, st, ws, ws_bytes, stream, &c));
  if (layer < 0 || layer >= c.L) return set_error(-1, "dit: layer out of range");
  if (!q_send || !kv_send) return set_error(-1, "dit: exchange buffers required");
  return dit_layer_qkv_hp(c, layer, world, q_send, kv_send);
}

extern "C" int rtv_dit_layer_attn_hp(const rtv_dit_config* cfg, const rtv_dit_weights* w, const rtv_dit_step* st, int layer,
                                     int world, const void* q_all, void* o_all, void* ws, size_t ws_bytes,
                                     rtv_stream_t stream) {
  Ctx c;
  RTV_TRY(make_ctx(cfg, w, st, ws, ws_bytes, stream, &c));
  if (layer < 0 || layer >= c.L) return set_error(-1, "dit: layer out of range");
  if (!q_all || !o_all) return set_error(-1, "dit: exchange buffers required");
  return dit_layer_attn_hp(c, layer, world, q_all, o_all);
}

extern "C" int rtv_dit_layer_rest_hp(const rtv_dit_config* cfg, const rtv_dit_weights* w, const rtv_dit_step* st, int layer,
                                     int world, const void* o_recv, void* ws, size_t ws_bytes, rtv_stream_t stream) {
  Ctx c;
  RTV_TRY(make_ctx(cfg, w, st, ws, ws_bytes, stream, &c));
  if (layer < 0 || layer >= c.L) return set_error(-1, "dit: layer out of range");
  if (!o_recv) return set_error(-1, "dit: exchange buffers required");
  return dit_layer_rest_hp(c, layer, world, o_recv);
}

extern "C" int rtv_dit_head(const rtv_dit_config* cfg, const rtv_dit_weights* w, const rtv_dit_step* st, void* head_rows,
                            void* ws, size_t ws_bytes, rtv_stream_t stream) {
  Ctx c;
  RTV_TRY(make_ctx(cfg, w, st, ws, ws_bytes, stream, &c));
  if (!head_rows) return set_error(-1, "dit: head_rows required");
  return dit_head(c, head_rows);
}

extern "C" int rtv_dit_finish(const rtv_dit_config* cfg, const rtv_dit_step* st, const void* head_rows,
                              rtv_stream_t stream) {
  if (!cfg || !st || !head_rows || !st->out) return set_error(-1, "dit: null argument");
  return rtv_unpatchify(head_rows, st->out, cfg->out_dim, st->F, st->gh, st->gw, stream);
}

extern "C" int rtv_dit_forward(const rtv_dit_config* cfg, const rtv_dit_weights* w, const rtv_dit_step* st,
                               void* workspace, size_t workspace_bytes, rtv_stream_t stream) {
  Ctx c;
  RTV_TRY(make_ctx(cfg, w, st, workspace, workspace_bytes, stream, &c));
  if (c.r0 != 0 || c.rc != c.M)
    return set_error(-1, "dit_forward: sharded row ranges need the phase API (rtv_dit_begin/layer_qkv/layer_rest/head/finish)");
  RTV_TRY(dit_begin(c));
  for (int l = 0; l < c.L; ++l) {
    if (st->kv_only && l == c.L - 1)
      return dit_layer_proj(c, l, RTV_PROJ_LN | RTV_PROJ_KV, 0, nullptr, nullptr);
    RTV_TRY(dit_layer_qkv(c, l));
    RTV_TRY(dit_layer_rest(c, l));
  }
  RTV_TRY(dit_head(c, c.b.hrow));
  return rtv_unpatchify(c.b.hrow, st->out, cfg->out_dim, c.F, c.gh, c.gw, stream);
}

extern "C" int rtv_dit_set_direct_v(int on) {
  g_direct_v = on ? 1 : 0;
  return 0;
}
```

realtime_video_amd/csrc/rtv_internal.h:

```cpp
#pragma once
#include <hip/hip_runtime.h>

#include <atomic>

#include "../../include/rtv_hip.h"
#include "../../include/rtv_hip_lab.h"

namespace rtv {

int set_error(int code, const char* msg);
int check_launch(const char* what);

struct LdsAttr {
  std::atomic<uint64_t> done{0};
};
int ensure_dynamic_lds(const void* kernel, int bytes, LdsAttr* state, const char* what);

int device_num_cus();

enum ProfClass { PROF_GEMM = 0, PROF_ATTN, PROF_LN, PROF_ROPE, PROF_CONV, PROF_MISC, PROF_NCLASS };

struct ProfScope {
  ProfScope(int cls, hipStream_t stream, double work);
  ~ProfScope();
  int slot;
  hipStream_t stream;
};

enum DispatchKernel {
  DK_GEMM_128x128 = 0, DK_GEMM_OTHER_CFG, DK_GEMM8_256x256, DK_GEMM8M_128x256, DK_GEMM5_160x256, DK_GEMM_FP8_256x256,
  DK_ATTN_W4, DK_ATTN_FOUR_PHASE, DK_ATTN_LOCKSTEP_256ROW, DK_ATTN_LOCKSTEP_128ROW, DK_ATTN_SPLIT_COMBINE,
  DK_CONV_HALO4P, DK_CONV_HALO4, DK_CONV_HALO, DK_CONV_IGEMM, DK_COUNT
};
void note_kernel(int id);

struct GemmParams;
int launch_gemm(const GemmParams& p, int dtype, int tile_cfg, hipStream_t stream);
int launch_gemm8(const GemmParams& p, bool f16, bool split_k, hipStream_t stream);
int launch_gemm4(const GemmParams& p, bool f16, hipStream_t stream, int lab = 0);
int launch_gemm8m(const GemmParams& p, bool f16, bool split_k, hipStream_t stream);
int launch_gemm5(const GemmParams& p, bool f16, bool split_k, hipStream_t stream);
int launch_quantize_fp8(const uint16_t* x, int64_t ld, int M, int d, uint8_t* q, int64_t ldq, float* scale_out,
                        unsigned* amax_scratch, hipStream_t stream);
int launch_gemm_fp8(GemmParams p, const uint8_t* A, int lda, const uint8_t* W, int ldw, const float* a_scale, float w_scale,
                    hipStream_t stream);

int qk_norm_rope_check(int64_t cache_row_stride, int cache_row0, int M, int d, int num_heads, int F, int gh, int gw, int start_frame,
                       int row_offset, int group_cols, int64_t q_group_stride, int64_t kv_group_stride, int ring_lo, int ring_size,
                       int ring_shift, int parts);
int qk_norm_rope_launch(const void* qkv, void* q_out, void* k_cache, void* v_cache, int64_t cache_row_stride,
                        int cache_row0, int M, int d, int num_heads, float eps, const void* wq, const void* wk,
                        const void* rope_cs, int F, int gh, int gw, int start_frame, int row_offset, int group_cols,
                        int64_t q_group_stride, int64_t kv_group_stride, int ring_lo, int ring_size, int ring_shift,
                        int parts , rtv_stream_t stream);
int regroup_heads(const void* in, void* out, int rows, int G, int group_cols, rtv_stream_t stream);

int conv3_last_tap(const void* frame, const void* w3, const void* bias, const void* gamma, const void* residual, int res_ld, void* out,
                   int out_ld, int H, int W, int Cin, int Cout, int flags, const void* zeros, hipStream_t stream);

}
```

realtime_video_amd/csrc/runtime.hip:

```cpp
#include <mutex>
#include <string>
#include <vector>

#include "gemm_core.h"
#include "rtv_internal.h"

namespace rtv {

static thread_local std::string g_err;

int set_error(int code, const char* msg) {
  g_err = msg ? msg : "unknown error";
  if (code > 0) {
    g_err += ": ";
    g_err += hipGetErrorString((hipError_t)code);
  }
  return code == 0 ? -1 : code;
}

int ensure_dynamic_lds(const void* kernel, int bytes, LdsAttr* state, const char* what) {
  int dev = 0;
  if (hipGetDevice(&dev) != hipSuccess || dev < 0 || dev >= 64) return set_error(-1, "cannot query the current device");
  const uint64_t bit = 1ull << dev;
  if (state->done.load(std::memory_order_acquire) & bit) return 0;
  hipError_t e = hipFuncSetAttribute(kernel, hipFuncAttributeMaxDynamicSharedMemorySize, bytes);
  if (e != hipSuccess) return set_error((int)e, what);
  state->done.fetch_or(bit, std::memory_order_release);
  return 0;
}

int device_num_cus() {
  static std::atomic<int> cus[64];
  int dev = 0;
  if (hipGetDevice(&dev) != hipSuccess || dev < 0 || dev >= 64) return 0;
  int n = cus[dev].load(std::memory_order_relaxed);
  if (n == 0) {
    hipDeviceProp_t prop;
    if (hipGetDeviceProperties(&prop, dev) != hipSuccess) return 0;
    n = prop.multiProcessorCount;
    cus[dev].store(n, std::memory_order_relaxed);
  }
  return n;
}

static std::atomic<int64_t> g_dispatch[DK_COUNT];
static const char* const g_dispatch_names[DK_COUNT] = {
    "gemm_kernel<128x128>", "gemm_kernel<other tile config>", "gemm8_kernel<256x256 ping-pong>", "gemm8m_kernel<128x256 ping-pong>",
    "gemm5_kernel<160x256 one wave per SIMD>", "gemm_fp8_kernel<256x256>",
    "attn_fwd_w4_kernel<one wave per SIMD>", "attn_fwd_pp_kernel<four-phase>", "attn_fwd_kernel<lockstep, 256 rows>",
    "attn_fwd_kernel<lockstep, 128 rows>", "attn_combine_kernel<kv split>",
    "conv_halo4p_kernel<persistent>", "conv_halo4_kernel", "conv_halo_kernel", "conv_igemm_kernel"};
void note_kernel(int id) {
  if (id >= 0 && id < DK_COUNT) g_dispatch[id].fetch_add(1, std::memory_order_relaxed);
}

int check_launch(const char* what) {
  hipError_t e = hipGetLastError();
  if (e != hipSuccess) return set_error((int)e, what);
  return 0;
}

struct ProfRec {
  int cls;
  hipEvent_t start, stop;
  double work;
};
static unsigned g_prof_mask = 0;
static int g_prof_stride[PROF_NCLASS] = {1, 1, 1, 1, 1, 1};
static int64_t g_prof_seen[PROF_NCLASS] = {0};
static double g_prof_seen_work[PROF_NCLASS] = {0};
static std::mutex g_prof_mu;
static std::vector<ProfRec> g_prof;
static std::vector<hipEvent_t> g_event_pool;

static hipEvent_t get_event() {
  if (!g_event_pool.empty()) {
    hipEvent_t e = g_event_pool.back();
    g_event_pool.pop_back();
    return e;
  }
  hipEvent_t e;
  hipEventCreate(&e);
  return e;
}

ProfScope::ProfScope(int cls, hipStream_t s, double work) : slot(-1), stream(s) {
  if (!((g_prof_mask >> cls) & 1u)) return;
  std::lock_guard<std::mutex> lk(g_prof_mu);
  g_prof_seen_work[cls] += work;
  if (g_prof_seen[cls]++ % g_prof_stride[cls]) return;
  ProfRec r;
  r.cls = cls;
  r.work = work;
  r.start = get_event();
  r.stop = get_event();
  hipEventRecord(r.start, s);
  g_prof.push_back(r);
  slot = (int)g_prof.size() - 1;
}
ProfScope::~ProfScope() {
  if (slot < 0) return;
  std::lock_guard<std::mutex> lk(g_prof_mu);
  hipEventRecord(g_prof[slot].stop, stream);
}

}

using namespace rtv;

extern "C" {

int rtv_version(void) { return RTV_ABI_VERSION; }

const char* rtv_last_error(void) { return g_err.c_str(); }

int rtv_lab_build(void) {
#ifdef RTV_LAB
  return 1;
#else
  return 0;
#endif
}

int rtv_dispatch_counts(int64_t* counts, int n) {
  for (int i = 0; counts && i < n && i < DK_COUNT; ++i) counts[i] = g_dispatch[i].load(std::memory_order_relaxed);
  return DK_COUNT;
}

const char* rtv_dispatch_name(int id) { return id >= 0 && id < DK_COUNT ? g_dispatch_names[id] : ""; }

int rtv_dispatch_reset(void) {
  for (auto& c : g_dispatch) c.store(0, std::memory_order_relaxed);
  return 0;
}

int rtv_prof_enable(int class_mask) {
  g_prof_mask = (unsigned)class_mask;
  return 0;
}

int rtv_prof_reset(void) {
  std::lock_guard<std::mutex> lk(g_prof_mu);
  for (auto& r : g_prof) {
    g_event_pool.push_back(r.start);
    g_event_pool.push_back(r.stop);
  }
  g_prof.clear();
  for (int c = 0; c < PROF_NCLASS; ++c) {
    g_prof_seen[c] = 0;
    g_prof_seen_work[c] = 0;
  }
  return 0;
}

int rtv_prof_set_stride(int cls, int stride) {
  if (cls < 0 || cls >= PROF_NCLASS || stride < 1) return set_error(-1, "prof_set_stride: class 0..5, stride >= 1");
  std::lock_guard<std::mutex> lk(g_prof_mu);
  g_prof_stride[cls] = stride;
  return 0;
}

int rtv_prof_bracket_overhead(int n, rtv_stream_t stream_, double* avg_ms) {
  if (n < 1 || n > 4096 || !avg_ms) return set_error(-1, "prof_bracket_overhead: 1 <= n <= 4096, avg_ms != null");
  hipStream_t stream = (hipStream_t)stream_;
  std::vector<hipEvent_t> ev;
  ev.reserve(2 * (size_t)n);
  auto fail = [&](const char* what) {
    for (auto& e : ev) (void)hipEventDestroy(e);
    return set_error(-1, what);
  };
  for (int i = 0; i < 2 * n; ++i) {
    hipEvent_t e;
    if (hipEventCreate(&e) != hipSuccess) return fail("prof_bracket_overhead: hipEventCreate");
    ev.push_back(e);
  }
  for (int i = 0; i < n; ++i) {
    if (hipEventRecord(ev[2 * i], stream) != hipSuccess || hipEventRecord(ev[2 * i + 1], stream) != hipSuccess)
      return fail("prof_bracket_overhead: hipEventRecord");
  }
  if (hipStreamSynchronize(stream) != hipSuccess) return fail("prof_bracket_overhead: hipStreamSynchronize");
  double tot = 0;
  for (int i = 0; i < n; ++i) {
    float t = 0;
    if (hipEventElapsedTime(&t, ev[2 * i], ev[2 * i + 1]) != hipSuccess) return fail("prof_bracket_overhead: hipEventElapsedTime");
    tot += t;
  }
  for (auto& e : ev) (void)hipEventDestroy(e);
  *avg_ms = tot / n;
  return 0;
}

int rtv_prof_read_seen(int cls, int64_t* launches, double* work) {
  if (cls < 0 || cls >= PROF_NCLASS) return set_error(-1, "prof_read_seen: class 0..5");
  std::lock_guard<std::mutex> lk(g_prof_mu);
  if (launches) *launches = g_prof_seen[cls];
  if (work) *work = g_prof_seen_work[cls];
  return 0;
}

int rtv_prof_read(int cls, double* total_ms, int64_t* launches, double* total_work) {
  std::lock_guard<std::mutex> lk(g_prof_mu);
  double ms = 0, work = 0;
  int64_t n = 0;
  for (auto& r : g_prof) {
    if (r.cls != cls) continue;
    hipError_t e = hipEventSynchronize(r.stop);
    if (e != hipSuccess) return set_error((int)e, "prof_read: hipEventSynchronize");
    float t = 0;
    e = hipEventElapsedTime(&t, r.start, r.stop);
    if (e != hipSuccess) return set_error((int)e, "prof_read: hipEventElapsedTime");
    ms += t;
    work += r.work;
    ++n;
  }
  if (total_ms) *total_ms = ms;
  if (launches) *launches = n;
  if (total_work) *total_work = work;
  return 0;
}

int rtv_gemm(const void* A, int lda, const void* W, int ldw, void* C, int ldc, int M, int N, int K,
             const void* bias, int act, const void* gate, int gate_stride, int rows_per_frame, int row_offset,
             const void* residual, int ldr, int dtype, int tile_cfg, rtv_stream_t stream) {
  if (!A || !W || !C) return set_error(-1, "gemm: null operand");
  if (((uintptr_t)A | (uintptr_t)W) & 15) return set_error(-1, "gemm: A/W must be 16-byte aligned");
  if (((uintptr_t)C | (uintptr_t)bias | (uintptr_t)gate | (uintptr_t)residual) & 7)
    return set_error(-1, "gemm: C/bias/gate/residual must be 8-byte aligned");
  if (gate && (gate_stride % 4)) return set_error(-1, "gemm: gate_stride must be a multiple of 4");
  if (act < 0 || act > 2) return set_error(-1, "gemm: unknown activation");
  GemmParams p;
  p.A = (const uint16_t*)A;
  p.W = (const uint16_t*)W;
  p.C = (uint16_t*)C;
  p.lda = lda;
  p.ldw = ldw;
  p.ldc = ldc;
  p.M = M;
  p.N = N;
  p.K = K;
  p.bias = (const uint16_t*)bias;
  p.act = act;
  p.gate = (const uint16_t*)gate;
  p.gate_stride = gate_stride;
  p.rows_per_frame = rows_per_frame;
  p.row_offset = row_offset;
  p.residual = (const uint16_t*)residual;
  p.ldr = ldr;
  p.tiles_m = p.tiles_n = 0;
  return launch_gemm(p, dtype, tile_cfg, (hipStream_t)stream);
}

}
```

realtime_video_amd/ops.py:

```python
import ctypes
import math

import torch

from . import _lib

ACT_NONE, ACT_GELU_TANH, ACT_SILU = 0, 1, 2
DT_BF16, DT_F16 = 0, 1
PROF_CLASSES = {"gemm": 0, "attn": 1, "layernorm": 2, "rope": 3, "conv": 4, "misc": 5}


def _ptr(t):
    return ctypes.c_void_p(t.data_ptr()) if t is not None else ctypes.c_void_p(0)


def _stream():
    return ctypes.c_void_p(torch.cuda.current_stream().cuda_stream)


def _dt(t):
    if t.dtype == torch.bfloat16:
        return DT_BF16
    if t.dtype == torch.float16:
        return DT_F16
    raise TypeError(f"expected bfloat16 or float16 tensor, got {t.dtype}")


def _gpu(*ts):
    for t in ts:
        if t is not None and not t.is_cuda:
            raise RuntimeError("realtime_video_amd kernels need GPU tensors (no CPU fallback)")


def prof_enable(on=True, classes=None):
    mask = 0
    if on:
        mask = 0x3F if classes is None else sum(1 << PROF_CLASSES[c] for c in classes)
    _lib.call("rtv_prof_enable", int(mask))


def prof_reset():
    _lib.call("rtv_prof_reset")


def prof_set_stride(cls, stride):
    _lib.call("rtv_prof_set_stride", PROF_CLASSES[cls] if isinstance(cls, str) else int(cls), int(stride))


def prof_bracket_overhead(n=256):
    ms = ctypes.c_double(0)
    _lib.call("rtv_prof_bracket_overhead", int(n), ctypes.c_void_p(torch.cuda.current_stream().cuda_stream), ctypes.byref(ms))
    return ms.value


def dispatch_counts(reset=False):
    lib = _lib.load()
    n = lib.rtv_dispatch_counts(None, 0)
    buf = (ctypes.c_int64 * n)()
    lib.rtv_dispatch_counts(buf, n)
    out = {lib.rtv_dispatch_name(i).decode(): int(buf[i]) for i in range(n) if buf[i]}
    if reset:
        lib.rtv_dispatch_reset()
    return out


def prof_read(cls):
    c = PROF_CLASSES[cls] if isinstance(cls, str) else int(cls)
    ms, n, work = ctypes.c_double(0), ctypes.c_int64(0), ctypes.c_double(0)
    _lib.call("rtv_prof_read", c, ctypes.byref(ms), ctypes.byref(n), ctypes.byref(work))
    sn, swork = ctypes.c_int64(0), ctypes.c_double(0)
    _lib.call("rtv_prof_read_seen", c, ctypes.byref(sn), ctypes.byref(swork))
    scale = swork.value / work.value if work.value > 0 else 1.0
    return {"ms": ms.value, "launches": n.value, "work": work.value, "seen_launches": sn.value, "seen_work": swork.value,
            "ms_class": ms.value * scale}


def attn_set_waves(waves=0):
    _lib.call("rtv_attn_set_waves", int(waves))


def attn_fwd(q, k, v, out=None, scale=None, causal_block=0, q_offset=0):
    _gpu(q, k, v)
    B, Lq, H, D = q.shape
    Lkv = k.shape[1]
    if k.shape != v.shape or k.shape[0] != B or k.shape[2] != H or k.shape[3] != D:
        raise ValueError(f"attention shape mismatch q{tuple(q.shape)} k{tuple(k.shape)} v{tuple(v.shape)}")
    if not (q.dtype == k.dtype == v.dtype):
        raise TypeError("q, k, v must share a dtype")
    for t in (q, k, v):
        if t.stride(3) != 1 or t.stride(2) != D:
            raise ValueError("attention operands need dense [H, D] inner dims (BLHD layout)")
    if out is None:
        out = torch.empty((B, Lq, H, D), dtype=q.dtype, device=q.device)
    if scale is None:
        scale = 1.0 / math.sqrt(D)
    _lib.call("rtv_attn_fwd", _ptr(q), _ptr(k), _ptr(v), _ptr(out), B, Lq, Lkv, H, D,
              q.stride(0), q.stride(1), k.stride(0), k.stride(1), v.stride(0), v.stride(1),
              out.stride(0), out.stride(1), float(scale), int(causal_block), int(q_offset), _dt(q), _stream())
    return out


def attn_fwd_dup(q, k, v, dup_key, dup_count, out=None, scale=None):
    _gpu(q, k, v)
    B, Lq, H, D = q.shape
    Lkv = k.shape[1]
    if k.shape != v.shape or k.shape[0] != B or k.shape[2] != H or k.shape[3] != D:
        raise ValueError(f"attention shape mismatch q{tuple(q.shape)} k{tuple(k.shape)} v{tuple(v.shape)}")
    for t in (q, k, v):
        if t.stride(3) != 1 or t.stride(2) != D:
            raise ValueError("attention operands need dense [H, D] inner dims (BLHD layout)")
    if out is None:
        out = torch.empty((B, Lq, H, D), dtype=q.dtype, device=q.device)
    if scale is None:
        scale = 1.0 / math.sqrt(D)
    _lib.call("rtv_attn_fwd_dup", _ptr(q), _ptr(k), _ptr(v), _ptr(out), B, Lq, Lkv, H, D,
              q.stride(0), q.stride(1), k.stride(0), k.stride(1), v.stride(0), v.stride(1),
              out.stride(0), out.stride(1), float(scale), int(dup_key), int(dup_count), _dt(q), _stream())
    return out


def attn_fwd_win(q, k_cache, v_cache, seg0, seg1=(0, 0), out=None, scale=None):
    _gpu(q, k_cache, v_cache)
    B, Lq, H, D = q.shape
    (r0, n0), (r1, n1) = seg0, seg1
    rows = k_cache.shape[1]
    if min(r0, n0, r1, n1) < 0 or r0 + n0 > rows or (n1 and r1 + n1 > rows):
        raise ValueError("attn_fwd_win: segment outside the cache")
    for t in (q, k_cache, v_cache):
        if t.stride(3) != 1 or t.stride(2) != D:
            raise ValueError("attention operands need dense [H, D] inner dims (BLHD layout)")
    if out is None:
        out = torch.empty((B, Lq, H, D), dtype=q.dtype, device=q.device)
    if scale is None:
        scale = 1.0 / math.sqrt(D)
    k, v = k_cache[:, r0:], v_cache[:, r0:]
    _lib.call("rtv_attn_fwd_win", _ptr(q), _ptr(k), _ptr(v), _ptr(out), B, Lq, n0, n1,
              (r1 - r0) if n1 else 0, H, D, q.stride(0), q.stride(1), k.stride(0), k.stride(1), v.stride(0), v.stride(1),
              out.stride(0), out.stride(1), float(scale), 0, 0, _dt(q), _stream())
    return out


def attn_fwd_split(q, k_cache, v_cache, seg0, seg1=(0, 0), kv_splits=2, out=None, scale=None, workspace=None, causal_block=0,
                   q_offset=0):
    _gpu(q, k_cache, v_cache)
    B, Lq, H, D = q.shape
    (r0, n0), (r1, n1) = seg0, seg1
    rows = k_cache.shape[1]
    if min(r0, n0, r1, n1) < 0 or r0 + n0 > rows or (n1 and r1 + n1 > rows):
        raise ValueError("attn_fwd_split: segment outside the cache")
    for t in (q, k_cache, v_cache):
        if t.stride(3) != 1 or t.stride(2) != D:
            raise ValueError("attention operands need dense [H, D] inner dims (BLHD layout)")
    if out is None:
        out = torch.empty((B, Lq, H, D), dtype=q.dtype, device=q.device)
    if scale is None:
        scale = 1.0 / math.sqrt(D)
    if workspace is None:
        need = _lib.load().rtv_attn_split_workspace_bytes(B, Lq, H, int(kv_splits))
        workspace = torch.empty(max(need, 16) // 4, dtype=torch.float32, device=q.device)
    k, v = k_cache[:, r0:], v_cache[:, r0:]
    _lib.call("rtv_attn_fwd_split", _ptr(q), _ptr(k), _ptr(v), _ptr(out), B, Lq, n0, n1,
              (r1 - r0) if n1 else 0, H, D, q.stride(0), q.stride(1), k.stride(0), k.stride(1), v.stride(0), v.stride(1),
              out.stride(0), out.stride(1), float(scale), int(causal_block), int(q_offset), int(kv_splits), _ptr(workspace),
              workspace.numel() * workspace.element_size(), _dt(q), _stream())
    return out


_gemm_ws = {}


def ensure_gemm_workspace(device, stream=None):
    dev = torch.device(device)
    idx = dev.index if dev.index is not None else torch.cuda.current_device()
    if stream is None:
        stream = torch.cuda.current_stream(idx).cuda_stream
    key = (idx, int(stream))
    if key in _gemm_ws:
        return
    n = _lib.load().rtv_gemm_workspace_bytes()
    with torch.cuda.device(idx):
        ws = torch.zeros(n + 256, dtype=torch.uint8, device=torch.device("cuda", idx))
        off = (-ws.data_ptr()) % 256
        try:
            _lib.call("rtv_gemm_set_stream_workspace", ctypes.c_void_p(int(stream)), ctypes.c_void_p(ws.data_ptr() + off),
                      ctypes.c_size_t(n))
        except RuntimeError as e:
            if "too many workspaces" not in str(e):
                raise
            import warnings
            warnings.warn("rtv: split-K workspace table full; GEMMs on this stream run unsplit "
                          "(release_gemm_workspace() frees the entry of a stream that is no longer used)")
            ws = None
    _gemm_ws[key] = ws


def release_gemm_workspace(device, stream):
    dev = torch.device(device)
    idx = dev.index if dev.index is not None else torch.cuda.current_device()
    handle = int(stream.cuda_stream if hasattr(stream, "cuda_stream") else stream)
    ws = _gemm_ws.pop((idx, handle), None)
    if ws is None:
        return
    with torch.cuda.device(idx):
        if hasattr(stream, "synchronize"):
            stream.synchronize()
        else:
            torch.cuda.synchronize(idx)
        _lib.call("rtv_gemm_set_stream_workspace", ctypes.c_void_p(handle), ctypes.c_void_p(0), ctypes.c_size_t(0))


def gemm(a, w, bias=None, act=ACT_NONE, gate=None, gate_stride=0, rows_per_frame=0, residual=None,
         out=None, tile_cfg=0, row_offset=0):
    _gpu(a, w, bias, gate, residual, out)
    if a.dim() != 2 or w.dim() != 2 or a.shape[1] != w.shape[1]:
        raise ValueError(f"gemm shape mismatch a{tuple(a.shape)} w{tuple(w.shape)}")
    if a.stride(1) != 1 or w.stride(1) != 1:
        raise ValueError("gemm operands must be K-contiguous")
    M, K = a.shape
    N = w.shape[0]
    if out is None:
        out = torch.empty((M, N), dtype=a.dtype, device=a.device)
    if tile_cfg in (0, 5, 7, 50):
        ensure_gemm_workspace(a.device)
    _lib.call("rtv_gemm", _ptr(a), a.stride(0), _ptr(w), w.stride(0), _ptr(out), out.stride(0), M, N, K,
              _ptr(bias), int(act), _ptr(gate), int(gate_stride), int(rows_per_frame), int(row_offset),
              _ptr(residual), residual.stride(0) if residual is not None else 0,
              _dt(a), int(tile_cfg), _stream())
    return out


def quantize_fp8(x, out=None):
    _gpu(x)
    if x.dtype != torch.bfloat16 or x.dim() != 2 or x.stride(1) != 1:
        raise TypeError("quantize_fp8 expects a K-contiguous bf16 matrix")
    M, d = x.shape
    if out is None:
        out = torch.empty((M, d), dtype=torch.float8_e4m3fn, device=x.device)
    scale = torch.empty(1, dtype=torch.float32, device=x.device)
    scratch = torch.empty(1, dtype=torch.int32, device=x.device)
    _lib.call("rtv_quantize_fp8", _ptr(x), ctypes.c_int64(x.stride(0)), M, d, _ptr(out), ctypes.c_int64(out.stride(0)),
              _ptr(scale), _ptr(scratch), _stream())
    return out, scale


def gemm_fp8(a_q, a_scale, w_q, w_scale, bias=None, act=ACT_NONE, gate=None, gate_stride=0, rows_per_frame=0,
             residual=None, out=None, row_offset=0):
    _gpu(a_q, w_q, a_scale, bias, gate, residual, out)
    if a_q.dtype != torch.float8_e4m3fn or w_q.dtype != torch.float8_e4m3fn:
        raise TypeError("gemm_fp8 expects float8_e4m3fn operands")
    M, K = a_q.shape
    N = w_q.shape[0]
    if w_q.shape[1] != K or a_q.stride(1) != 1 or w_q.stride(1) != 1:
        raise ValueError("gemm_fp8 shape / stride mismatch")
    if out is None:
        out = torch.empty((M, N), dtype=torch.bfloat16, device=a_q.device)
    ensure_gemm_workspace(a_q.device)
    _lib.call("rtv_gemm_fp8", _ptr(a_q), a_q.stride(0), _ptr(w_q), w_q.stride(0), _ptr(a_scale), ctypes.c_float(float(w_scale)),
              _ptr(out), out.stride(0), M, N, K, _ptr(bias), int(act), _ptr(gate), int(gate_stride), int(rows_per_frame),
              int(row_offset), _ptr(residual), residual.stride(0) if residual is not None else 0, _stream())
    return out


def layernorm_modulate(x, eps=1e-6, shift=None, scale=None, frame_stride=0, rows_per_frame=0,
                       weight=None, bias=None, out=None, row_offset=0):
    _gpu(x, shift, scale, weight, bias)
    M, d = x.shape
    if out is None:
        out = torch.empty_like(x)
    _lib.call("rtv_layernorm_modulate", _ptr(x), _ptr(out), M, d, float(eps), _ptr(shift), _ptr(scale),
              int(frame_stride), int(rows_per_frame), int(row_offset), _ptr(weight), _ptr(bias), _stream())
    return out


def rmsnorm(x, weight, eps=1e-6, out=None):
    _gpu(x, weight)
    M, d = x.shape
    if out is None:
        out = torch.empty((M, d), dtype=x.dtype, device=x.device)
    _lib.call("rtv_rmsnorm", _ptr(x), x.stride(0), _ptr(out), out.stride(0), M, d, float(eps), _ptr(weight),
              _stream())
    return out


def qk_norm_rope_cache(qkv, k_cache, v_cache, cache_row0, num_heads, wq, wk, rope_cs, grid, start_frame,
                       eps=1e-6, q_out=None, row_offset=0, ring=(0, 0, 0)):
    _gpu(qkv, k_cache, v_cache, wq, wk, rope_cs)
    M, d3 = qkv.shape
    d = d3 // 3
    F, gh, gw = grid
    if q_out is None:
        q_out = torch.empty((M, d), dtype=qkv.dtype, device=qkv.device)
    if cache_row0 + row_offset + M > k_cache.shape[0]:
        raise ValueError("KV-cache write out of range")
    _lib.call("rtv_qk_norm_rope_cache_ring", _ptr(qkv), _ptr(q_out), _ptr(k_cache), _ptr(v_cache),
              k_cache.stride(0), int(cache_row0), M, d, int(num_heads), float(eps), _ptr(wq), _ptr(wk),
              _ptr(rope_cs), int(F), int(gh), int(gw), int(start_frame), int(row_offset),
              int(ring[0]), int(ring[1]), int(ring[2]), _stream())
    return q_out


def modulation_table(modulation, e0, out=None):
    _gpu(modulation, e0)
    L, J, d = modulation.shape
    F, J0, _ = e0.shape
    if out is None:
        out = torch.empty((L, F, J, d), dtype=modulation.dtype, device=modulation.device)
    _lib.call("rtv_modulation_table", _ptr(modulation), _ptr(e0), _ptr(out), L, F, J, J0, d, _stream())
    return out


def sinusoidal_embedding(t, dim):
    _gpu(t)
    t = t.to(torch.float32).contiguous()
    out = torch.empty((t.numel(), dim), dtype=torch.bfloat16, device=t.device)
    _lib.call("rtv_sinusoidal_embedding", _ptr(t), _ptr(out), t.numel(), int(dim), _stream())
    return out


def patchify(x, gh, gw):
    _gpu(x)
    C, F = x.shape[0], x.shape[1]
    x = x.contiguous()
    out = torch.empty((F * gh * gw, C * 4), dtype=x.dtype, device=x.device)
    _lib.call("rtv_patchify", _ptr(x), _ptr(out), C, F, gh, gw, _stream())
    return out


def unpatchify(rows, C, F, gh, gw):
    _gpu(rows)
    rows = rows.contiguous()
    out = torch.empty((C, F, 2 * gh, 2 * gw), dtype=rows.dtype, device=rows.device)
    _lib.call("rtv_unpatchify", _ptr(rows), _ptr(out), C, F, gh, gw, _stream())
    return out


_T_KIND = {torch.float32: 0, torch.float64: 1, torch.int64: 2}


def _frame_view(x, what):
    if x.dtype != torch.bfloat16:
        raise NotImplementedError(f"scheduler_step: {what} must be bf16 (the reference's inference dtype), got {x.dtype}")
    F, C, h, w = x.shape
    if w > 1 and x.stride(3) != 1 or h > 1 and x.stride(2) != w:
        x = x.contiguous()
    return x, x.stride(0), x.stride(1)


def scheduler_step(timesteps, sigmas, flow=None, xt=None, t=None, x0=None, noise=None, t_next=None):
    src = flow if flow is not None else x0
    _gpu(src, timesteps, sigmas)
    F, C, h, w = src.shape
    if timesteps.dtype != torch.float32 or sigmas.dtype != torch.float32 or timesteps.numel() != sigmas.numel():
        raise ValueError("scheduler_step: timesteps / sigmas must be float32 tables of one length")
    tk = None
    for tt in (t, t_next):
        if tt is not None:
            _gpu(tt)
            if tt.dtype not in _T_KIND or tt.numel() != F or not tt.is_contiguous():
                raise ValueError(f"scheduler_step: timestep must be a contiguous [F] float32/float64/int64 tensor, got "
                                 f"{tt.dtype} {tuple(tt.shape)}")
            if tk is not None and tk != _T_KIND[tt.dtype]:
                raise ValueError("scheduler_step: t and t_next must share a dtype")
            tk = _T_KIND[tt.dtype]
    fs = fc = xs = xc = 0
    if flow is not None:
        _gpu(xt)
        if xt.shape != flow.shape:
            raise ValueError(f"scheduler_step: flow {tuple(flow.shape)} vs xt {tuple(xt.shape)}")
        flow, fs, fc = _frame_view(flow, "flow")
        xt, xs, xc = _frame_view(xt, "xt")
        x0 = torch.empty((F, C, h, w), dtype=torch.bfloat16, device=src.device)
    else:
        if x0.dtype != torch.bfloat16:
            raise NotImplementedError("scheduler_step: x0 must be bf16")
        x0 = x0.contiguous()
    noisy = None
    if t_next is not None:
        _gpu(noise)
        if noise.dtype != torch.bfloat16 or noise.shape != x0.shape:
            raise ValueError("scheduler_step: noise must be bf16 of the latent shape")
        noise = noise.contiguous()
        noisy = torch.empty_like(x0)
    _lib.call("rtv_scheduler_step", _ptr(flow) if flow is not None else None, fs, fc,
              _ptr(xt) if flow is not None else None, xs, xc, _ptr(t) if t is not None else None,
              _ptr(t_next) if t_next is not None else None, tk if tk is not None else 0,
              _ptr(timesteps), _ptr(sigmas), timesteps.numel(), _ptr(x0),
              _ptr(noise) if noise is not None else None, _ptr(noisy) if noisy is not None else None,
              F, C, h * w, _stream())
    return x0, noisy


def pixels_to_rgb8(pixels, out=None):
    _gpu(pixels)
    if pixels.dtype != torch.float32 or pixels.shape[-3] != 3 or not pixels.is_contiguous():
        raise ValueError("pixels_to_rgb8 expects contiguous float32 [..., 3, H, W]")
    H, W = pixels.shape[-2:]
    T = pixels.numel() // (3 * H * W)
    shape = tuple(pixels.shape[:-3]) + (H, W, 3)
    if out is None:
        out = torch.empty(shape, dtype=torch.uint8, device=pixels.device)
    elif out.shape != shape or out.dtype != torch.uint8 or not out.is_contiguous():
        raise ValueError("pixels_to_rgb8: out must be contiguous uint8 [..., H, W, 3]")
    _lib.call("rtv_pixels_to_rgb8", _ptr(pixels), _ptr(out), T, H, W, _stream())
    return out


def frames_from_rgb8(rgb8, size, out=None, slots=None):
    _gpu(rgb8)
    if rgb8.dtype != torch.uint8 or rgb8.dim() != 4 or rgb8.shape[-1] != 3 or not rgb8.is_contiguous():
        raise ValueError("frames_from_rgb8 expects contiguous uint8 [T, Hin, Win, 3]")
    N, Hin, Win = rgb8.shape[:3]
    h, w = int(size[0]), int(size[1])
    slots = list(range(N)) if slots is None else [int(i) for i in slots]
    if any(not 0 <= i < N for i in slots):
        raise IndexError(f"frames_from_rgb8: slot outside the {N} frames")
    T = len(slots)
    if out is None:
        out = torch.empty((3, T, h, w), dtype=torch.float16, device=rgb8.device)
    elif out.shape != (3, T, h, w) or out.dtype != torch.float16 or not out.is_contiguous() or out.device != rgb8.device:
        raise ValueError("frames_from_rgb8: out must be contiguous float16 [3, T, h, w] on the frames' device")
    for t0 in range(0, T, _lib.FRAMES_MAX):
        part = slots[t0:t0 + _lib.FRAMES_MAX]
        _lib.call("rtv_frames_from_rgb8", _ptr(rgb8), (ctypes.c_int * len(part))(*part), Hin * Win * 3, len(part), Hin, Win,
                  _ptr(out), T, t0, h, w, _stream())
    return out


def jpeg_header(quality, H, W):
    buf = ctypes.create_string_buffer(1024)
    n = _lib.load().rtv_jpeg_header(int(quality), int(H), int(W), buf, len(buf))
    if n == 0:
        _lib.check(-1, "rtv_jpeg_header")
    return buf.raw[:n]


def _jpeg_input(x, what):
    _gpu(x)
    if x.dtype == torch.float32 and x.dim() >= 3 and x.shape[-3] == 3 and x.is_contiguous():
        H, W = x.shape[-2:]
        return x, 0, x.numel() // (3 * H * W), H, W
    if x.dtype == torch.uint8 and x.dim() >= 3 and x.shape[-1] == 3 and x.is_contiguous():
        H, W = x.shape[-3:-1]
        return x, 1, x.numel() // (3 * H * W), H, W
    raise ValueError(f"{what} expects contiguous float32 [..., 3, H, W] in [-1, 1] or uint8 [..., H, W, 3]")


def _jpeg_arena(T, H, W, device, arena):
    need = jpeg_arena_bytes(T, H, W)
    if arena is None:
        arena = torch.empty(max(need, 16), dtype=torch.uint8, device=device)
    elif arena.dtype != torch.uint8 or not arena.is_contiguous() or arena.device != device:
        raise ValueError("arena must be a contiguous uint8 tensor on the pixels' device")
    return arena


def jpeg_arena_bytes(T, H, W):
    return _lib.load().rtv_jpeg_arena_bytes(int(T), int(H), int(W))


def jpeg_out_bound(T, H, W):
    return _lib.load().rtv_jpeg_out_bound(int(T), int(H), int(W))


def jpeg_encode(pixels, quality=90, out=None, offsets=None, arena=None):
    pixels, rgb8, T, H, W = _jpeg_input(pixels, "jpeg_encode")
    dev = pixels.device
    arena = _jpeg_arena(T, H, W, dev, arena)
    if offsets is None:
        offsets = torch.zeros(T + 1, dtype=torch.int64, device=dev)
    elif offsets.dtype != torch.int64 or offsets.numel() != T + 1 or not offsets.is_contiguous() or offsets.device != dev:
        raise ValueError("jpeg_encode: offsets must be contiguous int64 [T + 1] on the pixels' device")
    if out is not None and (out.dtype != torch.uint8 or not out.is_contiguous() or out.device != dev):
        raise ValueError("jpeg_encode: out must be a contiguous uint8 tensor on the pixels' device")

    def run(buf):
        _lib.call("rtv_jpeg_encode", _ptr(pixels), rgb8, T, H, W, int(quality), _ptr(arena), arena.numel(), _ptr(buf), buf.numel(),
                  _ptr(offsets), _stream())
    if out is not None:
        run(out)
        return out, offsets
    out = torch.empty(T * (H * W + 1024), dtype=torch.uint8, device=dev)
    run(out)
    total = int(offsets[-1]) if T else 0
    if total > out.numel():
        out = torch.empty(total, dtype=torch.uint8, device=dev)
        run(out)
    return out[:total], offsets


def jpeg_coefficients(pixels, quality=90, arena=None):
    pixels, rgb8, T, H, W = _jpeg_input(pixels, "jpeg_coefficients")
    arena = _jpeg_arena(T, H, W, pixels.device, arena)
    out = torch.empty((T, (H + 15) // 16, (W + 15) // 16, 6, 64), dtype=torch.int16, device=pixels.device)
    _lib.call("rtv_jpeg_coefficients", _ptr(pixels), rgb8, T, H, W, int(quality), _ptr(arena), arena.numel(), _ptr(out), _stream())
    return out


JPEG_DESC_BYTES = ctypes.sizeof(_lib.JPEGDEC_STRUCTS["rtv_jpeg_desc"])


class JpegInfo:

    def __init__(self, desc):
        self.desc = desc
        self.H, self.W, self.components = desc.height, desc.width, desc.components
        self.sampling = (desc.hsamp, desc.vsamp)
        self.restart_interval, self.file_bytes = desc.restart_interval, desc.file_bytes

    def packed(self):
        return ctypes.string_at(ctypes.byref(self.desc), JPEG_DESC_BYTES)


def _jpeg_bytes(data, what):
    if isinstance(data, (bytearray, memoryview)):
        data = bytes(data)
    if not isinstance(data, bytes):
        raise TypeError(f"{what} expects a JPEG file as bytes, bytearray or memoryview, not {type(data).__name__}")
    return data


def jpeg_parse(data):
    data = _jpeg_bytes(data, "jpeg_parse")
    lib = _lib.load()
    desc = _lib.JPEGDEC_STRUCTS["rtv_jpeg_desc"]()
    if lib.rtv_jpeg_parse(data, len(data), ctypes.byref(desc)) != 0:
        raise ValueError(lib.rtv_last_error().decode("utf-8", "replace"))
    return JpegInfo(desc)


def jpeg_decode_arena_bytes(infos):
    descs = (_lib.JPEGDEC_STRUCTS["rtv_jpeg_desc"] * max(len(infos), 1))(*[i.desc for i in infos])
    return _lib.load().rtv_jpeg_decode_arena_bytes(descs, len(infos))


def jpeg_decode_frames(infos, frames, outs, status, arena, rounds=None, subseq_bits=0):
    T = len(infos)
    if not (len(frames) == len(outs) == T) or T > _lib.FRAMES_MAX:
        raise ValueError(f"jpeg_decode: as many frames as outputs, at most {_lib.FRAMES_MAX} per call")
    _gpu(status, arena, rounds, *frames, *outs)
    for info, f, o in zip(infos, frames, outs):
        if f.dtype != torch.uint8 or not f.is_contiguous() or f.numel() < JPEG_DESC_BYTES + info.file_bytes:
            raise ValueError("jpeg_decode: a frame must be a contiguous uint8 tensor of descriptor plus file")
        if o.dtype != torch.uint8 or tuple(o.shape) != (info.H, info.W, 3) or not o.is_contiguous():
            raise ValueError("jpeg_decode: an output must be contiguous uint8 [H, W, 3] of the file's size")
    if status.dtype != torch.int32 or status.numel() < T or not status.is_contiguous():
        raise ValueError("jpeg_decode: status must be contiguous int32 [T]")
    if rounds is not None and (rounds.dtype != torch.int32 or rounds.numel() < T or not rounds.is_contiguous()):
        raise ValueError("jpeg_decode: rounds must be contiguous int32 [T]")
    if arena.dtype != torch.uint8 or not arena.is_contiguous():
        raise ValueError("jpeg_decode: arena must be a contiguous uint8 tensor")
    descs = (_lib.JPEGDEC_STRUCTS["rtv_jpeg_desc"] * T)(*[i.desc for i in infos])
    fp = (ctypes.c_void_p * T)(*[f.data_ptr() for f in frames])
    op = (ctypes.c_void_p * T)(*[o.data_ptr() for o in outs])
    _lib.call("rtv_jpeg_decode", descs, fp, op, T, int(subseq_bits), _ptr(arena), arena.numel(), _ptr(status), _ptr(rounds), _stream())


def _jpeg_upload(file, device, what):
    if torch.is_tensor(file):
        _gpu(file)
        raise TypeError(f"{what} expects JPEG files as bytes-like objects")
    data = _jpeg_bytes(file, what)
    info = jpeg_parse(data)
    host = torch.frombuffer(bytearray(info.packed() + data), dtype=torch.uint8)
    return info, host.to(device)


def jpeg_decode(files, out=None, status=None, arena=None, subseq_bits=0, device="cuda"):
    files = list(files)
    pairs = [_jpeg_upload(f, device, "jpeg_decode") for f in files]
    infos, frames = [p[0] for p in pairs], [p[1] for p in pairs]
    dev = frames[0].device if frames else torch.device(device)
    if out is None:
        out = [torch.empty((i.H, i.W, 3), dtype=torch.uint8, device=dev) for i in infos]
    if status is None:
        status = torch.zeros(len(files), dtype=torch.int32, device=dev)
    for t0 in range(0, len(files), _lib.FRAMES_MAX):
        part = slice(t0, t0 + _lib.FRAMES_MAX)
        need = jpeg_decode_arena_bytes(infos[part])
        a = arena if arena is not None else torch.empty(max(need, 16), dtype=torch.uint8, device=dev)
        jpeg_decode_frames(infos[part], frames[part], out[part], status[part], a, subseq_bits=subseq_bits)
    return out, status


def jpeg_decode_coefficients(file, subseq_bits=0, device="cuda"):
    info, frame = _jpeg_upload(file, device, "jpeg_decode_coefficients")
    need = jpeg_decode_arena_bytes([info])
    d = info.desc
    shapes = [(d.mcu_rows * (d.vsamp if c == 0 else 1), d.mcu_cols * (d.hsamp if c == 0 else 1), 64) for c in range(d.components)]
    n = sum(s[0] * s[1] * 64 for s in shapes)
    arena = torch.empty(max(need, 16), dtype=torch.uint8, device=frame.device)
    flat = torch.empty(n, dtype=torch.int16, device=frame.device)
    status = torch.zeros(1, dtype=torch.int32, device=frame.device)
    rounds = torch.zeros(1, dtype=torch.int32, device=frame.device)
    _lib.call("rtv_jpeg_decode_coefficients", ctypes.byref(d), _ptr(frame), int(subseq_bits), _ptr(arena), arena.numel(), _ptr(flat),
              _ptr(status), _ptr(rounds), _stream())
    out, at = [], 0
    for s in shapes:
        out.append(flat[at:at + s[0] * s[1] * 64].view(s))
        at += s[0] * s[1] * 64
    return out, status, rounds
```

Baseline: 18.73.

## Fold cross-attention V and output projection into a per-head precomputed weight

```diff
diff --git a/include/rtv_hip.h b/include/rtv_hip.h
--- a/include/rtv_hip.h
+++ b/include/rtv_hip.h
@@ -17,7 +17,7 @@
 
 typedef void* rtv_stream_t;
 
-#define RTV_ABI_VERSION 103
+#define RTV_ABI_VERSION 104
 int rtv_version(void);
 const char* rtv_last_error(void);
 
@@ -165,6 +165,7 @@
   int text_rows;
   int kv_only;
   int attn_kv_splits;
+  int ca_vo_ld;
 } rtv_dit_step;
 
 size_t rtv_dit_workspace_bytes(const rtv_dit_config* cfg, int F, int gh, int gw);
diff --git a/include/rtv_hip_cross_fold.h b/include/rtv_hip_cross_fold.h
--- /dev/null
+++ b/include/rtv_hip_cross_fold.h
@@ -0,0 +1,21 @@
+#ifndef RTV_HIP_CROSS_FOLD_H
+#define RTV_HIP_CROSS_FOLD_H
+#include "rtv_hip.h"
+
+#ifdef __cplusplus
+extern "C" {
+#endif
+
+int rtv_attn_probs_dup(const void* q, const void* k, void* p, int Lq, int Lkv, int H, int D,
+                       int64_t q_row_stride, int64_t k_row_stride, int64_t p_row_stride, int kh, int p_cols,
+                       float scale, int dup_key, int dup_count, rtv_stream_t stream);
+
+#define RTV_CROSS_FOLD_KH_MAX 120
+int rtv_cross_fold_dims(int num_heads, int text_rows, int* kh, int* k_fold);
+int rtv_cross_fold_weight(const void* co_w, int64_t ldw, const void* v, int64_t ldv, void* vo, int64_t ldvo,
+                          int num_heads, int rows, int kh, int k_fold, rtv_stream_t stream);
+
+#ifdef __cplusplus
+}
+#endif
+#endif
diff --git a/realtime_video_amd/_lib.py b/realtime_video_amd/_lib.py
--- a/realtime_video_amd/_lib.py
+++ b/realtime_video_amd/_lib.py
@@ -100,6 +100,9 @@
 LORA_STRUCTS = dict(STRUCTS)
 LORA_PROTOTYPES = parse_header(_read(LORA_HEADER), LORA_STRUCTS)
 LORA_STRUCTS = {k: v for k, v in LORA_STRUCTS.items() if k not in STRUCTS}
+CROSS_FOLD_HEADER = "rtv_hip_cross_fold.h"
+CROSS_FOLD_STRUCTS = dict(STRUCTS)
+CROSS_FOLD_PROTOTYPES = parse_header(_read(CROSS_FOLD_HEADER), CROSS_FOLD_STRUCTS)
 LORA_MAX_ADAPTERS, LORA_MAX_RANK = (int(re.search(rf"^#define\s+RTV_LORA_MAX_{n}\s+(\d+)", _read(LORA_HEADER), flags=re.M).group(1))
                                     for n in ("ADAPTERS", "RANK"))
 FRAMES_MAX = int(re.search(r"^#define\s+RTV_FRAMES_MAX\s+(\d+)", _read(IO_HEADER), flags=re.M).group(1))
@@ -135,7 +138,7 @@
             f"{LIB_PATH} is missing: run `python -c 'import __graft_entry__ as g; g.build()'` "
             "(or `make -C realtime_video_amd/csrc`). There is no CPU fallback for the HIP path.")
     lib = ctypes.CDLL(LIB_PATH)
-    for name, (restype, argtypes) in list(PROTOTYPES.items()) + list(IO_PROTOTYPES.items()) + list(JPEG_PROTOTYPES.items()) + list(JPEGDEC_PROTOTYPES.items()) + list(LORA_PROTOTYPES.items()):
+    for name, (restype, argtypes) in list(PROTOTYPES.items()) + list(IO_PROTOTYPES.items()) + list(JPEG_PROTOTYPES.items()) + list(JPEGDEC_PROTOTYPES.items()) + list(LORA_PROTOTYPES.items()) + list(CROSS_FOLD_PROTOTYPES.items()):
         fn = getattr(lib, name, None)
         if fn is None:
             if os.environ.get("RTV_LIB_PATH"):
diff --git a/realtime_video_amd/causal_model.py b/realtime_video_amd/causal_model.py
--- a/realtime_video_amd/causal_model.py
+++ b/realtime_video_amd/causal_model.py
@@ -1,5 +1,6 @@
 import collections
 import ctypes
+import os
 import types
 
 import torch
@@ -22,6 +23,15 @@
 _FP8_LAYER = ("qkv_w", "o_w", "cq_w", "ck_w", "cv_w", "co_w", "ffn0_w", "ffn2_w")
 
 PROJ_LN, PROJ_Q, PROJ_KV = 1, 2, 4
+
+
+def _cross_fold_max_cols(num_heads):
+    lib, kh, kf = _lib.load(), ctypes.c_int(0), ctypes.c_int(0)
+    rows = 1
+    while lib.rtv_cross_fold_dims(int(num_heads), rows + 8, ctypes.byref(kh), ctypes.byref(kf)):
+        rows += 8
+    lib.rtv_cross_fold_dims(int(num_heads), rows, ctypes.byref(kh), ctypes.byref(kf))
+    return kf.value
 
 
 class BlockCausalMask:
@@ -85,6 +95,7 @@
         self._w = None
         self._ws = {}
         self.fold_text_padding = True
+        self.fold_cross_v = os.environ.get("RTV_FOLD_CROSS_V", "1") != "0"
         self.use_hip_graphs = False
         self._graphs = {}
         self._weights_version = 0
@@ -322,7 +333,7 @@
                 self._fp8_scales[len(_FP8_TOP) + len(_FP8_LAYER) * int(layer) + _FP8_LAYER.index(field)] = s
             if not live:
                 del self._lora_base[key]
-            cross = cross or key.endswith((".ck_w", ".cv_w"))
+            cross = cross or key.endswith((".ck_w", ".cv_w", ".co_w"))
         if fp8 and keys:
             self._graphs.clear()
             self._weights_version += 1
@@ -495,6 +506,17 @@
         text_rows = int(crossattn_cache[0].get("text_rows", 0)) if getattr(self, "fold_text_padding", True) else 0
         if text_rows <= 0 or any(int(c.get("text_rows", 0)) != text_rows for c in crossattn_cache):
             text_rows = 0
+        fold_k = 0
+        if 0 < text_rows < self.text_len - 1 and getattr(self, "fold_cross_v", True) and not self._cfg.use_fp8:
+            kh_, kf_ = ctypes.c_int(0), ctypes.c_int(0)
+            if _lib.load().rtv_cross_fold_dims(self.num_heads, text_rows, ctypes.byref(kh_), ctypes.byref(kf_)):
+                fold_k = kf_.value
+            if fold_k and not need_cross and any(c.get("vo_for") != (text_rows, self.lora_version) for c in crossattn_cache):
+                fold_k = 0
+        if fold_k:
+            for c in crossattn_cache:
+                if "vo" not in c:
+                    c["vo"] = torch.zeros(self.dim * _cross_fold_max_cols(self.num_heads), dtype=torch.bfloat16, device=u.device)
         row0, lo, hi, start_frame, causal_block, (ring_lo, ring_size, ring_shift), commit = \
             self._cache_window(kv_cache, M, current_start, fs, ring=not use_cp)
         L = self.num_layers
@@ -512,7 +534,9 @@
         kk_keep, kk = ptr_array([c["k"] for c in kv_cache])
         kv_keep, kv = ptr_array([c["v"] for c in kv_cache])
         ck_keep, ck = ptr_array([c["k"] for c in crossattn_cache])
-        cv_keep, cv = ptr_array([c["v"] for c in crossattn_cache])
+        cv_list = [c["v"] for c in crossattn_cache] + ([c["vo"] for c in crossattn_cache] if fold_k else [])
+        cv_keep = (c_vp * len(cv_list))(*[t_.data_ptr() for t_ in cv_list])
+        cv = ctypes.cast(cv_keep, ctypes.POINTER(c_vp))
         out = (torch.zeros if kv_only else torch.empty)((self.out_dim, F, Hh, Ww), dtype=torch.bfloat16, device=u.device)
         stream = c_vp(torch.cuda.current_stream().cuda_stream)
         cfg_p, w_p = ctypes.byref(self._cfg), ctypes.byref(self._w)
@@ -524,7 +548,7 @@
                        F, gh, gw, kk, kv, rs, ck, cv, int(need_cross), row0, lo, hi,
                        start_frame, causal_block, int(self.gemm_tile_cfg), rank_rows[0], rank_rows[1],
                        ring_lo, ring_size, ring_shift, int(text_rows), int(kv_only),
-                       int(getattr(cp, "attn_kv_splits", 1)) if use_cp else 1)
+                       int(getattr(cp, "attn_kv_splits", 1)) if use_cp else 1, fold_k)
             return st, (c_vp(ws_ptr), ctypes.c_size_t(ws.numel() - (ws_ptr - ws.data_ptr())), stream)
 
         splits = int(getattr(cp, "attn_kv_splits", 1)) if use_cp else 1
@@ -540,7 +564,7 @@
         if not use_cp:
             graph_key = None
             if self.use_hip_graphs and not need_cross:
-                graph_key = (F, gh, gw, row0, lo, hi, start_frame, causal_block, ring_lo, ring_size, ring_shift, kv_only, text_rows,
+                graph_key = (F, gh, gw, row0, lo, hi, start_frame, causal_block, ring_lo, ring_size, ring_shift, kv_only, text_rows, fold_k,
                              int(self.gemm_tile_cfg), rs, self._weights_version,
                              kv_cache[0]["k"].data_ptr(), kv_cache[-1]["v"].data_ptr(), crossattn_cache[0]["k"].data_ptr())
                 ent = self._graphs.get(graph_key)
@@ -575,7 +599,7 @@
             graph_key = None
             if self.use_hip_graphs and not need_cross and not getattr(cp, "_gloo", False):
                 graph_key = ("cp", id(cp), bool(getattr(cp, "overlap", True)), cp.world, cp.head_exchange(self.num_heads), F, gh, gw, row0, lo, hi, start_frame, causal_block, kv_only,
-                             text_rows, int(self.gemm_tile_cfg), rs, self._weights_version, splits,
+                             text_rows, fold_k, int(self.gemm_tile_cfg), rs, self._weights_version, splits,
                              kv_cache[0]["k"].data_ptr(), kv_cache[-1]["v"].data_ptr(), crossattn_cache[0]["k"].data_ptr())
                 ent = self._graphs.get(graph_key)
                 if isinstance(ent, dict):
@@ -671,6 +695,7 @@
             for c in crossattn_cache:
                 c["is_init"] = True
                 c["lora_version"] = self.lora_version
+                c["vo_for"] = (text_rows, self.lora_version) if fold_k else None
         return out.unsqueeze(0)
 
     def forward(self, *args, **kwargs):
diff --git a/realtime_video_amd/csrc/attn_fwd.hip b/realtime_video_amd/csrc/attn_fwd.hip
--- a/realtime_video_amd/csrc/attn_fwd.hip
+++ b/realtime_video_amd/csrc/attn_fwd.hip
@@ -605,6 +605,124 @@
   }
 }
 
+struct ProbsParams {
+  const uint16_t* q;
+  const uint16_t* k;
+  uint16_t* p;
+  int Lq, Lkv, H;
+  int64_t q_rs, k_rs, p_rs;
+  int kh, p_cols;
+  float scale_log2e;
+  int dup_key;
+  float dup_log2;
+  int tiles_per_wg;
+};
+constexpr int PROBS_NW = 4;
+constexpr int PROBS_ROWS = PROBS_NW * ATT_QW;
+
+template <int NKB>
+__global__ __launch_bounds__(PROBS_NW * 64) void attn_probs_kernel(ProbsParams p) {
+  constexpr int KEYS = NKB * 32;
+  constexpr int SLAB_LD = KEYS * 2 + 16;
+  extern __shared__ __attribute__((aligned(16))) char smem[];
+  char* const sK = smem;
+  const int tid = threadIdx.x;
+  const int lane = tid & 63;
+  const int wave = __builtin_amdgcn_readfirstlane(tid >> 6);
+  const int l31 = lane & 31, g = lane >> 5;
+  char* const slab = smem + KEYS * 256 + wave * (ATT_QW * SLAB_LD);
+  const int h = blockIdx.y;
+  const uint16_t* qb = p.q + (size_t)h * ATT_D;
+  const uint16_t* kb = p.k + (size_t)h * ATT_D;
+  uint16_t* pb = p.p + (size_t)h * p.kh;
+
+  for (int id = tid; id < KEYS * 16; id += PROBS_NW * 64) {
+    const int r = id >> 4, c = id & 15;
+    u32x4 v = {0u, 0u, 0u, 0u};
+    if (r < p.Lkv) v = *(const u32x4*)(kb + (int64_t)r * p.k_rs + c * 8);
+    *(u32x4*)(sK + r * 256 + ((c ^ (r & 15)) << 4)) = v;
+  }
+  __syncthreads();
+  const char* k_rd[8];
+#pragma unroll
+  for (int dc = 0; dc < 8; ++dc) k_rd[dc] = sK + l31 * 256 + (((dc * 2 + g) ^ (l31 & 15)) << 4);
+
+  const float c = p.scale_log2e;
+  const int ppr = p.kh >> 3;
+  const int tail0 = p.H * p.kh, tail_pieces = h == p.H - 1 ? (p.p_cols - tail0) >> 3 : 0;
+  const int tile0 = blockIdx.x * p.tiles_per_wg;
+  for (int ti = 0; ti < p.tiles_per_wg; ++ti) {
+    const int row0 = (tile0 + ti) * PROBS_ROWS + wave * ATT_QW;
+    if (row0 >= p.Lq) break;
+    const int q_row_c = min(row0 + l31, p.Lq - 1);
+    u32x4 qf[8];
+    {
+      const uint16_t* qp = qb + (size_t)q_row_c * p.q_rs + g * 8;
+#pragma unroll
+      for (int dc = 0; dc < 8; ++dc) qf[dc] = *(const u32x4*)(qp + dc * 16);
+    }
+    f32x16 s[NKB];
+#pragma unroll
+    for (int kbk = 0; kbk < NKB; ++kbk)
+#pragma unroll
+      for (int r = 0; r < 16; ++r) s[kbk][r] = 0.f;
+#pragma unroll
+    for (int dc = 0; dc < 8; ++dc)
+#pragma unroll
+      for (int kbk = 0; kbk < NKB; ++kbk) {
+        const u32x4 kf = *(const u32x4*)(k_rd[dc] + kbk * 32 * 256);
+        s[kbk] = mfma32<false>(kf, qf[dc], s[kbk]);
+      }
+    float mx = -INFINITY;
+#pragma unroll
+    for (int kbk = 0; kbk < NKB; ++kbk)
+#pragma unroll
+      for (int r = 0; r < 16; ++r) {
+        const int key = kbk * 32 + (r & 3) + 8 * (r >> 2) + 4 * g;
+        float x = s[kbk][r] * c;
+        if (key == p.dup_key) x += p.dup_log2;
+        if (key >= p.Lkv) x = -INFINITY;
+        s[kbk][r] = x;
+        mx = fmaxf(mx, x);
+      }
+    mx = fmaxf(mx, __shfl_xor(mx, 32, 64));
+    float l = 0.f;
+#pragma unroll
+    for (int kbk = 0; kbk < NKB; ++kbk)
+#pragma unroll
+      for (int r = 0; r < 16; ++r) {
+        const float e = __builtin_amdgcn_exp2f(s[kbk][r] - mx);
+        s[kbk][r] = e;
+        l += e;
+      }
+    l += __shfl_xor(l, 32, 64);
+    const float inv = 1.0f / l;
+#pragma unroll
+    for (int kbk = 0; kbk < NKB; ++kbk)
+#pragma unroll
+      for (int i = 0; i < 4; ++i) {
+        u32x2 w;
+        w[0] = pack2<false>(s[kbk][4 * i + 0] * inv, s[kbk][4 * i + 1] * inv);
+        w[1] = pack2<false>(s[kbk][4 * i + 2] * inv, s[kbk][4 * i + 3] * inv);
+        *(u32x2*)(slab + l31 * SLAB_LD + (kbk * 32 + 8 * i + 4 * g) * 2) = w;
+      }
+    __builtin_amdgcn_fence(__ATOMIC_RELEASE, "workgroup");
+    __builtin_amdgcn_wave_barrier();
+    const int rows_here = min(ATT_QW, p.Lq - row0);
+    for (int id = lane; id < rows_here * ppr; id += 64) {
+      const int r = id / ppr, pc = id - r * ppr;
+      const u32x4 v = *(const u32x4*)(slab + r * SLAB_LD + pc * 16);
+      *(u32x4*)(pb + (int64_t)(row0 + r) * p.p_rs + pc * 8) = v;
+    }
+    for (int id = lane; id < rows_here * tail_pieces; id += 64) {
+      const int r = id / tail_pieces, pc = id - r * tail_pieces;
+      *(u32x4*)(p.p + (int64_t)(row0 + r) * p.p_rs + tail0 + pc * 8) = u32x4{0u, 0u, 0u, 0u};
+    }
+    __builtin_amdgcn_fence(__ATOMIC_ACQUIRE, "workgroup");
+    __builtin_amdgcn_wave_barrier();
+  }
+}
+
 }
 
 using namespace rtv;
@@ -676,6 +794,60 @@
   return attn_fwd_impl(q, k, v, o, B, Lq, Lkv, 0, 0, H, D, q_batch_stride, q_row_stride, k_batch_stride, k_row_stride,
                        v_batch_stride, v_row_stride, o_batch_stride, o_row_stride, scale, 0, 0, dtype, stream,
                        dup_count > 1 ? dup_key : -1, dup_count);
+}
+
+template <int NKB>
+static int launch_attn_probs(const ProbsParams& p, dim3 grid, hipStream_t stream) {
+  static LdsAttr lds_attr;
+  const int lds = NKB * 32 * 256 + PROBS_NW * ATT_QW * (NKB * 64 + 16);
+  if (int st = ensure_dynamic_lds((const void*)attn_probs_kernel<NKB>, lds, &lds_attr, "attn_probs")) return st;
+  hipLaunchKernelGGL((attn_probs_kernel<NKB>), grid, dim3(PROBS_NW * 64), lds, stream, p);
+  return check_launch("attn_probs");
+}
+
+extern "C" int rtv_attn_probs_dup(const void* q, const void* k, void* p, int Lq, int Lkv, int H, int D, int64_t q_row_stride,
+                                  int64_t k_row_stride, int64_t p_row_stride, int kh, int p_cols, float scale, int dup_key,
+                                  int dup_count, rtv_stream_t stream) {
+  if (D != ATT_D) return set_error(-1, "attn_probs: head_dim must be 128");
+  if (H <= 0 || Lq <= 0) return 0;
+  if (Lkv <= 0 || Lkv > 128) return set_error(-1, "attn_probs: the key window must hold 1..128 keys");
+  if (kh <= 0 || (kh & 7) || kh < Lkv || kh > 128) return set_error(-1, "attn_probs: kh must be a multiple of 8 in [Lkv, 128]");
+  if ((p_cols & 7) || (int64_t)H * kh > p_cols || p_cols > p_row_stride)
+    return set_error(-1, "attn_probs: need H * kh <= p_cols <= p_row_stride, p_cols a multiple of 8");
+  if ((q_row_stride | k_row_stride | p_row_stride) & 7 || q_row_stride < (int64_t)H * ATT_D || k_row_stride < (int64_t)H * ATT_D)
+    return set_error(-1, "attn_probs: strides must be multiples of 8 elements (16-byte rows) and hold H heads");
+  if (((uintptr_t)q | (uintptr_t)k | (uintptr_t)p) & 15) return set_error(-1, "attn_probs: base pointers must be 16-byte aligned");
+  if (dup_key < 0 || dup_key >= Lkv || dup_count < 1) return set_error(-1, "attn_probs: dup_key must be a key of the window, dup_count >= 1");
+  ProbsParams pp;
+  pp.q = (const uint16_t*)q;
+  pp.k = (const uint16_t*)k;
+  pp.p = (uint16_t*)p;
+  pp.Lq = Lq;
+  pp.Lkv = Lkv;
+  pp.H = H;
+  pp.q_rs = q_row_stride;
+  pp.k_rs = k_row_stride;
+  pp.p_rs = p_row_stride;
+  pp.kh = kh;
+  pp.p_cols = p_cols;
+  pp.scale_log2e = scale * 1.4426950408889634f;
+  pp.dup_key = dup_count > 1 ? dup_key : -1;
+  pp.dup_log2 = dup_count > 1 ? log2f((float)dup_count) : 0.f;
+  const int cus = device_num_cus() > 0 ? device_num_cus() : 256;
+  const int n_tiles = (Lq + PROBS_ROWS - 1) / PROBS_ROWS;
+  int tpw = (int)(((int64_t)n_tiles * H) / (2 * (int64_t)cus));
+  tpw = tpw < 1 ? 1 : (tpw > 8 ? 8 : tpw);
+  pp.tiles_per_wg = tpw;
+  const dim3 grid((n_tiles + tpw - 1) / tpw, H);
+  ProfScope prof(PROF_ATTN, (hipStream_t)stream, 2.0 * H * (double)Lq * Lkv * ATT_D);
+  note_kernel(DK_ATTN_PROBS);
+  const int nkb = (kh + 31) / 32;
+  switch (nkb) {
+    case 1: return launch_attn_probs<1>(pp, grid, (hipStream_t)stream);
+    case 2: return launch_attn_probs<2>(pp, grid, (hipStream_t)stream);
+    case 3: return launch_attn_probs<3>(pp, grid, (hipStream_t)stream);
+    default: return launch_attn_probs<4>(pp, grid, (hipStream_t)stream);
+  }
 }
 
 extern "C" size_t rtv_attn_split_workspace_bytes(int B, int Lq, int H, int kv_splits) {
diff --git a/realtime_video_amd/csrc/dit_forward.hip b/realtime_video_amd/csrc/dit_forward.hip
--- a/realtime_video_amd/csrc/dit_forward.hip
+++ b/realtime_video_amd/csrc/dit_forward.hip
@@ -8,6 +8,55 @@
 __global__ void silu_kernel(const bf16_t* __restrict__ x, bf16_t* __restrict__ out, int64_t n) {
   for (int64_t i = (int64_t)blockIdx.x * blockDim.x + threadIdx.x; i < n; i += (int64_t)gridDim.x * blockDim.x)
     out[i] = f32_to_bf16(silu(bf16_to_f32(x[i])));
+}
+
+constexpr int FOLD_ROWS = 64, FOLD_LD = 130;
+__global__ __launch_bounds__(256) void cross_fold_weight_kernel(const bf16_t* __restrict__ w, int64_t ldw, const bf16_t* __restrict__ v,
+                                                               int64_t ldv, bf16_t* __restrict__ vo, int64_t ldvo, int H, int rows, int kh,
+                                                               int k_fold) {
+  __shared__ __attribute__((aligned(16))) bf16_t sW[FOLD_ROWS * FOLD_LD];
+  __shared__ __attribute__((aligned(16))) bf16_t sV[128 * FOLD_LD];
+  const int tid = threadIdx.x, lane = tid & 63, wave = tid >> 6;
+  const int n0 = blockIdx.x * FOLD_ROWS, h = blockIdx.y;
+  for (int id = tid; id < FOLD_ROWS * 64; id += 256) {
+    const int r = id >> 6, c = (id & 63) * 2;
+    *(uint32_t*)(sW + r * FOLD_LD + c) = *(const uint32_t*)(w + (int64_t)(n0 + r) * ldw + h * 128 + c);
+  }
+  for (int id = tid; id < rows * 64; id += 256) {
+    const int r = id >> 6, c = (id & 63) * 2;
+    *(uint32_t*)(sV + r * FOLD_LD + c) = *(const uint32_t*)(v + (int64_t)r * ldv + h * 128 + c);
+  }
+  __syncthreads();
+  for (int ts = 0; ts < kh; ts += 64) {
+    const int t = ts + lane;
+    float acc[16];
+#pragma unroll
+    for (int i = 0; i < 16; ++i) acc[i] = 0.f;
+    if (t < rows) {
+      const bf16_t* vr = sV + t * FOLD_LD;
+      const bf16_t* wr = sW + wave * 16 * FOLD_LD;
+      for (int dd = 0; dd < 128; dd += 2) {
+        const uint32_t v2 = *(const uint32_t*)(vr + dd);
+        const float v0 = __uint_as_float(v2 << 16), v1 = __uint_as_float(v2 & 0xffff0000u);
+#pragma unroll
+        for (int i = 0; i < 16; ++i) {
+          const uint32_t w2 = *(const uint32_t*)(wr + i * FOLD_LD + dd);
+          acc[i] = fmaf(__uint_as_float(w2 << 16), v0, acc[i]);
+          acc[i] = fmaf(__uint_as_float(w2 & 0xffff0000u), v1, acc[i]);
+        }
+      }
+    }
+    if (t < kh) {
+#pragma unroll
+      for (int i = 0; i < 16; ++i) vo[(int64_t)(n0 + wave * 16 + i) * ldvo + h * kh + t] = f32_to_bf16(acc[i]);
+    }
+  }
+  if (h == H - 1) {
+    const int tail0 = H * kh;
+    for (int t = tail0 + lane; t < k_fold; t += 64)
+#pragma unroll
+      for (int i = 0; i < 16; ++i) vo[(int64_t)(n0 + wave * 16 + i) * ldvo + t] = 0;
+  }
 }
 
 struct Workspace {
@@ -76,6 +125,7 @@
   DitBuffers b;
   rtv_stream_t stream;
   int d, H, L, ffn, hd, F, gh, gw, fs, M, r0, rc, tc;
+  int fold_kh, fold_k;
 };
 
 static int make_ctx(const rtv_dit_config* cfg, const rtv_dit_weights* w, const rtv_dit_step* st, void* workspace,
@@ -113,6 +163,15 @@
   carve(cfg, c->F, c->gh, c->gw, (char*)workspace, workspace_bytes, &c->b, &ok);
   if (!ok) return set_error(-1, "dit: workspace too small (see rtv_dit_workspace_bytes)");
   c->tc = st->gemm_tile_cfg;
+  c->fold_kh = c->fold_k = 0;
+  if (st->ca_vo_ld > 0 && st->ca_v && !cfg->use_fp8 && st->text_rows > 0 && st->text_rows + 1 < cfg->text_len) {
+    int kh = 0, kf = 0;
+    if (rtv_cross_fold_dims(c->H, st->text_rows, &kh, &kf) && kf <= c->d) {
+      if (st->ca_vo_ld < kf || (st->ca_vo_ld & 7)) return set_error(-1, "dit: ca_vo_ld must be a multiple of 8 and >= k_fold (rtv_cross_fold_dims)");
+      c->fold_kh = kh;
+      c->fold_k = kf;
+    }
+  }
   return 0;
 }
 
@@ -133,6 +192,28 @@
   hipLaunchKernelGGL(silu_kernel, dim3(blocks), dim3(256), 0, (hipStream_t)stream, (const bf16_t*)x,
                      (bf16_t*)out, n);
   return check_launch("silu");
+}
+
+extern "C" int rtv_cross_fold_dims(int num_heads, int text_rows, int* kh, int* k_fold) {
+  const int khv = text_rows >= 0 ? (text_rows + 1 + 7) & ~7 : 0;
+  const int64_t kf = ((int64_t)num_heads * khv + 63) & ~(int64_t)63;
+  if (kh) *kh = khv;
+  if (k_fold) *k_fold = kf > 0x7fffffff ? 0 : (int)kf;
+  return num_heads > 0 && text_rows > 0 && khv <= RTV_CROSS_FOLD_KH_MAX && kf <= 0x7fffffff;
+}
+
+extern "C" int rtv_cross_fold_weight(const void* co_w, int64_t ldw, const void* v, int64_t ldv, void* vo, int64_t ldvo, int num_heads,
+                                     int rows, int kh, int k_fold, rtv_stream_t stream) {
+  if (!co_w || !v || !vo) return set_error(-1, "cross_fold_weight: null argument");
+  if (num_heads <= 0 || rows <= 0 || rows > kh || kh > 128 || (kh & 7)) return set_error(-1, "cross_fold_weight: need 0 < rows <= kh <= 128, kh % 8 == 0");
+  const int64_t d = (int64_t)num_heads * 128;
+  if ((int64_t)num_heads * kh > k_fold || k_fold > ldvo || ldw < d || ldv < d || ((ldw | ldv) & 1))
+    return set_error(-1, "cross_fold_weight: need num_heads * kh <= k_fold <= ldvo and rows of num_heads * 128 elements");
+  if (((uintptr_t)co_w | (uintptr_t)v) & 3) return set_error(-1, "cross_fold_weight: operands must be 4-byte aligned");
+  ProfScope prof(PROF_MISC, (hipStream_t)stream, 2.0 * d * (double)num_heads * rows * 128);
+  hipLaunchKernelGGL(cross_fold_weight_kernel, dim3((unsigned)(d / FOLD_ROWS), num_heads), dim3(256), 0, (hipStream_t)stream,
+                     (const bf16_t*)co_w, ldw, (const bf16_t*)v, ldv, (bf16_t*)vo, ldvo, num_heads, rows, kh, k_fold);
+  return check_launch("cross_fold_weight");
 }
 
 extern "C" size_t rtv_dit_workspace_bytes(const rtv_dit_config* cfg, int F, int gh, int gw) {
@@ -179,6 +260,9 @@
       RTV_TRY(linear(c, S_LAYER0 + S_PER_LAYER * l + S_CK, b.ctx, d, lw.ck_w, lw.ck_b, b.ktmp, T, d, 0, nullptr, 0, 0, 0, nullptr, tc, stream));
       RTV_TRY(rtv_rmsnorm(b.ktmp, d, st->ca_k[l], d, T, d, cfg->eps, lw.cnorm_k_w, stream));
       RTV_TRY(linear(c, S_LAYER0 + S_PER_LAYER * l + S_CV, b.ctx, d, lw.cv_w, lw.cv_b, st->ca_v[l], T, d, 0, nullptr, 0, 0, 0, nullptr, tc, stream));
+      if (c.fold_k)
+        RTV_TRY(rtv_cross_fold_weight(lw.co_w, d, st->ca_v[l], d, st->ca_v[c.L + l], st->ca_vo_ld, c.H, st->text_rows + 1, c.fold_kh, c.fold_k,
+                                      stream));
     }
   }
   return 0;
@@ -353,13 +437,20 @@
   RTV_TRY(rtv_layernorm_modulate(b.x, b.xn, rc, d, eps, nullptr, nullptr, 0, 0, 0, lw.norm3_w, lw.norm3_b, stream));
   RTV_TRY(linear(c, S_LAYER0 + S_PER_LAYER * l + S_CQ, b.xn, d, lw.cq_w, lw.cq_b, b.qkv, rc, d, 0, nullptr, 0, 0, 0, nullptr, tc, stream));
   RTV_TRY(rtv_rmsnorm(b.qkv, d, b.q, d, rc, d, eps, lw.cnorm_q_w, stream));
-  if (st->text_rows > 0 && st->text_rows + 1 < c.cfg->text_len)
-    RTV_TRY(rtv_attn_fwd_dup(b.q, st->ca_k[l], st->ca_v[l], b.ao, 1, rc, st->text_rows + 1, H, hd, 0, d, 0, d, 0, d, 0, d, scale,
-                             st->text_rows, c.cfg->text_len - st->text_rows, RTV_DTYPE_BF16, stream));
-  else
-    RTV_TRY(rtv_attn_fwd(b.q, st->ca_k[l], st->ca_v[l], b.ao, 1, rc, c.cfg->text_len, H, hd, 0, d, 0, d, 0, d, 0, d,
-                         scale, 0, 0, RTV_DTYPE_BF16, stream));
-  RTV_TRY(linear(c, S_LAYER0 + S_PER_LAYER * l + S_CO, b.ao, d, lw.co_w, lw.co_b, b.x, rc, d, 0, nullptr, 0, 0, 0, b.x, tc, stream));
+  if (c.fold_k) {
+    RTV_TRY(rtv_attn_probs_dup(b.q, st->ca_k[l], b.ao, rc, st->text_rows + 1, H, hd, d, d, c.fold_k, c.fold_kh, c.fold_k, scale,
+                               st->text_rows, c.cfg->text_len - st->text_rows, stream));
+    RTV_TRY(rtv_gemm(b.ao, c.fold_k, st->ca_v[c.L + l], st->ca_vo_ld, b.x, d, rc, d, c.fold_k, lw.co_b, 0, nullptr, 0, 0, 0, b.x, d,
+                     RTV_DTYPE_BF16, tc, stream));
+  } else {
+    if (st->text_rows > 0 && st->text_rows + 1 < c.cfg->text_len)
+      RTV_TRY(rtv_attn_fwd_dup(b.q, st->ca_k[l], st->ca_v[l], b.ao, 1, rc, st->text_rows + 1, H, hd, 0, d, 0, d, 0, d, 0, d, scale,
+                               st->text_rows, c.cfg->text_len - st->text_rows, RTV_DTYPE_BF16, stream));
+    else
+      RTV_TRY(rtv_attn_fwd(b.q, st->ca_k[l], st->ca_v[l], b.ao, 1, rc, c.cfg->text_len, H, hd, 0, d, 0, d, 0, d, 0, d,
+                           scale, 0, 0, RTV_DTYPE_BF16, stream));
+    RTV_TRY(linear(c, S_LAYER0 + S_PER_LAYER * l + S_CO, b.ao, d, lw.co_w, lw.co_b, b.x, rc, d, 0, nullptr, 0, 0, 0, b.x, tc, stream));
+  }
   RTV_TRY(rtv_layernorm_modulate(b.x, b.xn, rc, d, eps, em + 3 * d, em + 4 * d, 6 * d, fs, r0, nullptr, nullptr, stream));
   RTV_TRY(linear(c, S_LAYER0 + S_PER_LAYER * l + S_FFN0, b.xn, d, lw.ffn0_w, lw.ffn0_b, b.h, rc, c.ffn, RTV_ACT_GELU_TANH, nullptr, 0, 0, 0, nullptr, tc, stream));
   RTV_TRY(linear(c, S_LAYER0 + S_PER_LAYER * l + S_FFN2, b.h, c.ffn, lw.ffn2_w, lw.ffn2_b, b.x, rc, d, 0, em + 5 * d, 6 * d, fs, r0, b.x, tc, stream));
diff --git a/realtime_video_amd/csrc/rtv_internal.h b/realtime_video_amd/csrc/rtv_internal.h
--- a/realtime_video_amd/csrc/rtv_internal.h
+++ b/realtime_video_amd/csrc/rtv_internal.h
@@ -4,6 +4,7 @@
 #include <atomic>
 
 #include "../../include/rtv_hip.h"
+#include "../../include/rtv_hip_cross_fold.h"
 #include "../../include/rtv_hip_lab.h"
 
 namespace rtv {
@@ -30,7 +31,7 @@
 enum DispatchKernel {
   DK_GEMM_128x128 = 0, DK_GEMM_OTHER_CFG, DK_GEMM8_256x256, DK_GEMM8M_128x256, DK_GEMM5_160x256, DK_GEMM_FP8_256x256,
   DK_ATTN_W4, DK_ATTN_FOUR_PHASE, DK_ATTN_LOCKSTEP_256ROW, DK_ATTN_LOCKSTEP_128ROW, DK_ATTN_SPLIT_COMBINE,
-  DK_CONV_HALO4P, DK_CONV_HALO4, DK_CONV_HALO, DK_CONV_IGEMM, DK_COUNT
+  DK_CONV_HALO4P, DK_CONV_HALO4, DK_CONV_HALO, DK_CONV_IGEMM, DK_ATTN_PROBS, DK_COUNT
 };
 void note_kernel(int id);
 
diff --git a/realtime_video_amd/csrc/runtime.hip b/realtime_video_amd/csrc/runtime.hip
--- a/realtime_video_amd/csrc/runtime.hip
+++ b/realtime_video_amd/csrc/runtime.hip
@@ -49,7 +49,8 @@
     "gemm5_kernel<160x256 one wave per SIMD>", "gemm_fp8_kernel<256x256>",
     "attn_fwd_w4_kernel<one wave per SIMD>", "attn_fwd_pp_kernel<four-phase>", "attn_fwd_kernel<lockstep, 256 rows>",
     "attn_fwd_kernel<lockstep, 128 rows>", "attn_combine_kernel<kv split>",
-    "conv_halo4p_kernel<persistent>", "conv_halo4_kernel", "conv_halo_kernel", "conv_igemm_kernel"};
+    "conv_halo4p_kernel<persistent>", "conv_halo4_kernel", "conv_halo_kernel", "conv_igemm_kernel",
+    "attn_probs_kernel<short window, probabilities>"};
 void note_kernel(int id) {
   if (id >= 0 && id < DK_COUNT) g_dispatch[id].fetch_add(1, std::memory_order_relaxed);
 }
diff --git a/realtime_video_amd/ops.py b/realtime_video_amd/ops.py
--- a/realtime_video_amd/ops.py
+++ b/realtime_video_amd/ops.py
@@ -116,6 +116,40 @@
     _lib.call("rtv_attn_fwd_dup", _ptr(q), _ptr(k), _ptr(v), _ptr(out), B, Lq, Lkv, H, D,
               q.stride(0), q.stride(1), k.stride(0), k.stride(1), v.stride(0), v.stride(1),
               out.stride(0), out.stride(1), float(scale), int(dup_key), int(dup_count), _dt(q), _stream())
+    return out
+
+
+def cross_fold_dims(num_heads, text_rows):
+    kh, kf = ctypes.c_int(0), ctypes.c_int(0)
+    ok = _lib.load().rtv_cross_fold_dims(int(num_heads), int(text_rows), ctypes.byref(kh), ctypes.byref(kf))
+    return bool(ok), kh.value, kf.value
+
+
+def attn_probs_dup(q, k, dup_key, dup_count, kh, p_cols, out=None, scale=None):
+    _gpu(q, k)
+    Lq, H, D = q.shape
+    Lkv = k.shape[0]
+    if q.dtype != torch.bfloat16 or k.dtype != torch.bfloat16:
+        raise TypeError("attn_probs_dup is bf16 only")
+    for t in (q, k):
+        if t.stride(2) != 1 or t.stride(1) != D:
+            raise ValueError("attention operands need dense [H, D] inner dims")
+    if out is None:
+        out = torch.empty((Lq, p_cols), dtype=q.dtype, device=q.device)
+    if scale is None:
+        scale = 1.0 / math.sqrt(D)
+    _lib.call("rtv_attn_probs_dup", _ptr(q), _ptr(k), _ptr(out), Lq, Lkv, H, D, q.stride(0), k.stride(0), out.stride(0),
+              int(kh), int(p_cols), float(scale), int(dup_key), int(dup_count), _stream())
+    return out
+
+
+def cross_fold_weight(co_w, v, rows, kh, k_fold, out=None):
+    _gpu(co_w, v)
+    d = co_w.shape[0]
+    if out is None:
+        out = torch.empty((d, k_fold), dtype=torch.bfloat16, device=co_w.device)
+    _lib.call("rtv_cross_fold_weight", _ptr(co_w), co_w.stride(0), _ptr(v), v.stride(0), _ptr(out), out.stride(0), d // 128,
+              int(rows), int(kh), int(k_fold), _stream())
     return out
 
 
```

Result: faster. 19.28, median of 6 (+2.9%).
